# Yash-10/beta-sgp

Measured on AMD Instinct MI355X. Metric: SGP iterations/sec (fp64) on batched 256x256 images, higher is better.
Workload: dtype f64; 1 GPU; C3: 1024 independent 256x256 stamps per GPU, 25x25 PSF, linear A, beta-SGP (beta=1.05), proj_type=1, MAXIT=100, stop_criterion=1; images_per_gpu=1024, images_total=1024, maxit=100, parallelism=1 independent shards, one process per GPU (no collective on the data path), ls_spec=2, streams=1, team=1, proj_cache=1, gn_compact=1, storage=f64, persistent=1, stop_criterion=1

## Files before the change

### beta-sgp_amd/_bsgp.py

```python
import ctypes
import os
import threading

import numpy as np

try:
    import torch
except ImportError:
    torch = None

_HERE = os.path.dirname(os.path.abspath(__file__))
LIB_PATH = os.environ.get("BSGP_LIB", os.path.join(_HERE, "libbsgp.so"))

BSGP_CONV_CIRCULAR = 0
BSGP_CONV_LINEAR_FILL = 1
BSGP_VARIANT_KL = 0
BSGP_VARIANT_BETA = 1
BSGP_STORAGE_F64 = 0
BSGP_STORAGE_F32 = 1
ABI_VERSION = 3
BSGP_ERR_ARG = -1
BSGP_ERR_HIP = -2
BSGP_ERR_UNSUPPORTED = -3
BSGP_ERR_PSF = -4
# ... 35 lines not shown

class Inputs(ctypes.Structure):
    _fields_ = [("gn", _P), ("bkg", _P), ("flux", _P), ("x0", _P), ("beta0", _P), ("obj", _P)]


class Outputs(ctypes.Structure):
    _fields_ = [("x", _P), ("iters", _P), ("discr", _P), ("times", _P), ("crit", _P),
                ("flags", _P), ("beta_final", _P), ("counters", _P), ("err", _P),
                ("x_iter", _P)]


class PsfModel(ctypes.Structure):
    _fields_ = [("hw", ctypes.c_int32), ("ngauss", ctypes.c_int32), ("ldeg", ctypes.c_int32),
                ("sdeg", ctypes.c_int32), ("cos", ctypes.c_double), ("sin", ctypes.c_double),
                ("ax", ctypes.c_double), ("ay", ctypes.c_double), ("sigma_inc", ctypes.c_double),
                ("x_orig", ctypes.c_double), ("y_orig", ctypes.c_double), ("coeffs", _P),
                ("ncoef", ctypes.c_int32)]


BSGP_STATE_MAGIC = 0x53475342
BSGP_STATE_VERSION = 1
BSGP_STATE_HEADER_BYTES = 1024


class StateHeader(ctypes.Structure):
    _fields_ = [
        ("magic", ctypes.c_uint32), ("version", ctypes.c_uint32),
        ("H", ctypes.c_int32), ("W", ctypes.c_int32), ("storage", ctypes.c_int32),
        ("conv_mode", ctypes.c_int32), ("hist_cap", ctypes.c_int32), ("T", ctypes.c_int32),
        ("iters_done", ctypes.c_int32), ("stopped", ctypes.c_int32), ("Xones", ctypes.c_int32),
        ("epoch", ctypes.c_int32), ("g32", ctypes.c_int32), ("beta0_given", ctypes.c_int32),
        ("record_bytes", ctypes.c_int64), ("counters", ctypes.c_int64 * 7),
        ("scaling", ctypes.c_double), ("flux", ctypes.c_double), ("bkg_scalar", ctypes.c_double),
        ("x_low", ctypes.c_double), ("x_upp", ctypes.c_double), ("Dcoeff", ctypes.c_double),
        ("tol", ctypes.c_double), ("elapsed", ctypes.c_double), ("fv", ctypes.c_double),
        ("alpha", ctypes.c_double), ("tau", ctypes.c_double), ("lr", ctypes.c_double),
        ("init_lr", ctypes.c_double), ("beta", ctypes.c_double), ("lam_p", ctypes.c_double),
        ("lam_ratio", ctypes.c_double), ("kappa", ctypes.c_double), ("konst", ctypes.c_double),
        ("gfill", ctypes.c_double), ("Valpha", ctypes.c_double * 32),
        ("Fold", ctypes.c_double * 32), ("prm", Params),
    ]


assert ctypes.sizeof(StateHeader) <= BSGP_STATE_HEADER_BYTES
STATE_HEADER_DTYPE = np.dtype(StateHeader)
STATE_SECTIONS = ("discr", "crit", "times", "flags", "x", "g", "x_tf", "pw", "gn", "bkg")

_lib = None
_lib_lock = threading.Lock()


def lib():
    global _lib
    if _lib is not None:
        return _lib
    with _lib_lock:
        if _lib is None:
            if not os.path.exists(LIB_PATH):
                raise BsgpError(-3, f"{LIB_PATH} not built — run __graft_entry__.build()")
            L = ctypes.CDLL(LIB_PATH)
            i32, i64, dbl, vp = ctypes.c_int32, ctypes.c_int64, ctypes.c_double, ctypes.c_void_p
            L.bsgp_last_error.restype = ctypes.c_char_p
            L.bsgp_abi_version.restype = i32
            L.bsgp_plan_create.argtypes = [i32, i32, vp, i32, i32, i32, i32, i32,
                                           ctypes.POINTER(vp)]
            L.bsgp_plan_create_checked.argtypes = [i32, i32, vp, i32, i32, i32, i32, i32, i32,
                                                   ctypes.POINTER(vp)]
            L.bsgp_plan_destroy.argtypes = [vp]
            L.bsgp_plan_info.argtypes = [vp, vp, vp, vp, vp]
            L.bsgp_solve_device.argtypes = [vp, i32, vp, vp, vp, vp]
            L.bsgp_solve_host.argtypes = [vp, i32, vp, vp, vp]
            L.bsgp_solve_profiled.argtypes = [vp, i32, vp, vp, vp, vp, vp, vp]
            L.bsgp_apply_operator.argtypes = [vp, i32, i32, vp, vp, vp]
            L.bsgp_project_df.argtypes = [i64, dbl, vp, vp, dbl, i32, dbl, dbl, dbl, dbl, i32,
                                          i32, i32, vp, vp, vp]
            L.bsgp_beta_div.argtypes = [i64, vp, vp, dbl, vp, vp]
            L.bsgp_beta_div_deriv.argtypes = [i64, vp, vp, dbl, vp, vp]
            L.bsgp_beta_div_grad_parts.argtypes = [i64, vp, vp, dbl, vp, vp, vp]
            L.bsgp_extract_tiles.argtypes = [vp, i32, i32, vp, i32, i32, i32, vp, vp]
            L.bsgp_coadd_tiles.argtypes = [vp, i32, i32, i32, vp, i32, i32, vp, vp, vp]
            L.bsgp_fits_to_f64.argtypes = [vp, i64, i32, dbl, dbl, vp, vp]
            L.bsgp_psf_stamps.argtypes = [ctypes.POINTER(PsfModel), vp, i32, i32, i32, vp, vp]
            L.bsgp_plan_set_psfs.argtypes = [vp, vp, i32, vp]
            L.bsgp_state_layout.argtypes = [i32, i32, i32, i32, i32, vp]
            L.bsgp_state_bytes.argtypes = [vp, i32, i32, ctypes.POINTER(i64)]
            L.bsgp_state_save.argtypes = [vp, i32, vp, i64, vp]
            L.bsgp_solve_resume.argtypes = [vp, i32, vp, vp, i32, i64, vp, vp, vp]
            L.bsgp_background2d.argtypes = [vp, i32, i32, i32, i32, i32, i32, i32, i32, dbl, i32,
                                            dbl, i32, vp, vp, vp, vp, vp, vp, vp, vp]
            L.bsgp_convolve2d.argtypes = [vp, i32, i32, i32, i32, vp, i32, i32, vp, vp]
            L.bsgp_detect_sources.argtypes = [vp, i32, i32, i32, i32, vp, dbl, i32, i32, vp, vp,
                                              vp, vp]
            L.bsgp_segment_catalog.argtypes = [vp, vp, vp, i32, i32, i32, i32, vp, vp, vp, vp, vp]
            for name in ["bsgp_plan_create", "bsgp_plan_create_checked", "bsgp_plan_destroy", "bsgp_plan_info",
                         "bsgp_solve_device", "bsgp_solve_host", "bsgp_solve_profiled",
                         "bsgp_apply_operator",
                         "bsgp_project_df", "bsgp_beta_div", "bsgp_beta_div_deriv",
                         "bsgp_beta_div_grad_parts", "bsgp_device_synchronize",
                         "bsgp_extract_tiles", "bsgp_coadd_tiles", "bsgp_fits_to_f64",
                         "bsgp_psf_stamps", "bsgp_plan_set_psfs", "bsgp_state_layout",
                         "bsgp_state_bytes", "bsgp_state_save", "bsgp_solve_resume",
                         "bsgp_background2d", "bsgp_convolve2d", "bsgp_detect_sources",
                         "bsgp_segment_catalog"]:
                getattr(L, name).restype = ctypes.c_int
            if L.bsgp_abi_version() != ABI_VERSION:
                raise BsgpError(-3, f"{LIB_PATH} has ABI {L.bsgp_abi_version()}, this binding "
                                    f"needs {ABI_VERSION}: rebuild with __graft_entry__.build()")
            _lib = L
    return _lib


EXPORTED = ["bsgp_plan_create", "bsgp_plan_create_checked", "bsgp_plan_destroy", "bsgp_plan_info", "bsgp_solve_device",
            "bsgp_solve_host", "bsgp_solve_profiled", "bsgp_apply_operator", "bsgp_project_df", "bsgp_beta_div",
            "bsgp_beta_div_deriv", "bsgp_beta_div_grad_parts", "bsgp_device_synchronize",
            "bsgp_last_error", "bsgp_abi_version", "bsgp_extract_tiles", "bsgp_coadd_tiles",
            "bsgp_fits_to_f64", "bsgp_psf_stamps", "bsgp_plan_set_psfs", "bsgp_state_layout",
            "bsgp_state_bytes", "bsgp_state_save", "bsgp_solve_resume", "bsgp_background2d",
            "bsgp_convolve2d", "bsgp_detect_sources", "bsgp_segment_catalog"]


def check(rc):
    if rc != 0:
        raise BsgpError(rc, lib().bsgp_last_error().decode(errors="replace"))


def require_gpu():
    if torch is None or not torch.cuda.is_available():
        raise BsgpError(-2, "no HIP device visible: the beta-SGP engine has no CPU fallback")


def _ptr(t):
    return ctypes.c_void_p(t.data_ptr()) if t is not None else None


def current_stream():
    return ctypes.c_void_p(torch.cuda.current_stream().cuda_stream)


class Plan:

    _leased = False
    _done = None

    def __init__(self, H, W, psf, conv_mode, device=None, storage=BSGP_STORAGE_F64,
                 psf_checked=False):
        require_gpu()
        if device is None:
            device = torch.cuda.current_device()
        psf = np.ascontiguousarray(psf, dtype="<f8")
        self.H, self.W = int(H), int(W)
        self.kh, self.kw = psf.shape
        self.conv_mode = conv_mode
        self.device = device
        self.storage = storage
        h = ctypes.c_void_p()
        rc = lib().bsgp_plan_create_checked(self.H, self.W, psf.ctypes.data, self.kh, self.kw,
                                            conv_mode, storage, device, int(bool(psf_checked)),
                                            ctypes.byref(h))
        if rc != 0:
            raise BsgpError(rc, lib().bsgp_last_error().decode(errors="replace"))
        self.h = h
        P, Q, wave = ctypes.c_int32(), ctypes.c_int32(), ctypes.c_int32()
        sb = ctypes.c_int64()
        check(lib().bsgp_plan_info(h, ctypes.byref(P), ctypes.byref(Q), ctypes.byref(sb),
                                   ctypes.byref(wave)))
        self.P, self.Q, self.slot_bytes, self.fft_waves = P.value, Q.value, sb.value, wave.value

    def __del__(self):
        h = getattr(self, "h", None)
        if h is not None and _lib is not None:
            try:
                _lib.bsgp_plan_destroy(h)
            except Exception:
                pass
            self.h = None

    def set_psfs(self, psfs):
        psfs = psfs.to(dtype=torch.float64).contiguous()
        if psfs.dim() != 3 or tuple(psfs.shape[1:]) != (self.kh, self.kw):
            raise ValueError(f"psfs must be [n, {self.kh}, {self.kw}]")
        check(lib().bsgp_plan_set_psfs(self.h, _ptr(psfs), psfs.shape[0], current_stream()))
        self.n_psf = psfs.shape[0]
        return self

    def apply(self, x, transpose=False):
        x = x.contiguous()
        out = torch.empty_like(x)
        B = 1 if x.dim() == 2 else x.shape[0]
        check(lib().bsgp_apply_operator(self.h, B, int(transpose), _ptr(x), _ptr(out),
                                        current_stream()))
        return out

    def solve(self, gn, bkg, params, flux=None, x0=None, beta0=None, want_times=True, obj=None,
              want_iterates=False, profile=False):
        B = gn.shape[0]
        M1 = params.MAXIT + 1
        dev = gn.device
        f64 = dict(dtype=torch.float64, device=dev)
        if want_iterates:
            need = B * params.MAXIT * self.H * self.W * 8
            free = torch.cuda.mem_get_info(dev)[0]
            if need > 0.8 * free:
                raise BsgpError(
                    f"save=True keeps {params.MAXIT} iterates of {self.H}x{self.W} on the device "
                    f"({need / 2**30:.1f} GiB, {free / 2**30:.1f} GiB free): lower MAXIT")
        nd = B * M1 * (2 + bool(want_times) + (obj is not None)) + B
        d64 = torch.zeros(nd, **f64)
        i32 = torch.zeros(B * (M1 + 1) + 2 * 8 * B, dtype=torch.int32, device=dev)
        parts = iter(torch.split(d64, [B * M1] * (2 + bool(want_times) + (obj is not None)) + [B]))
        discr, crit = next(parts).view(B, M1), next(parts).view(B, M1)
        times = next(parts).view(B, M1) if want_times else None
        err = next(parts).view(B, M1) if obj is not None else None
        beta_final = next(parts)
        cnt, iters, flags = torch.split(i32, [2 * 8 * B, B, B * M1])
        out = {
            "x": torch.empty_like(gn),
            "iters": iters,
            "discr": discr,
            "times": times,
            "crit": crit,
            "flags": flags.view(B, M1),
            "beta_final": beta_final,
            "counters": cnt.view(torch.int64).view(B, 8),
            "err": err,
            "x_iter": (torch.zeros(B, params.MAXIT, self.H, self.W, **f64) if want_iterates
                       else None),
        }
        ins = Inputs(_ptr(gn), _ptr(bkg), _ptr(flux), _ptr(x0), _ptr(beta0), _ptr(obj))
        outs = Outputs(*[_ptr(out[k]) for k in ["x", "iters", "discr", "times", "crit", "flags",
                                                 "beta_final", "counters", "err", "x_iter"]])
        self._keep = (gn, bkg, flux, x0, beta0, obj)
        self._last = (B, int(params.MAXIT), int(params.bkg_is_map), out)
        if profile:
            kms = np.zeros(6, np.float64)
            nl = np.zeros(6, np.int64)
            check(lib().bsgp_solve_profiled(self.h, B, ctypes.byref(params), ctypes.byref(ins),
                                            ctypes.byref(outs), current_stream(),
                                            kms.ctypes.data, nl.ctypes.data))
            out["kernel_ms"], out["launches"] = kms, nl
            return out
        check(lib().bsgp_solve_device(self.h, B, ctypes.byref(params), ctypes.byref(ins),
                                      ctypes.byref(outs), current_stream()))
        return out

    def save_state(self, B):
        last = getattr(self, "_last", None)
        if last is None or last[0] != B:
            raise BsgpError(BSGP_ERR_ARG, "save_state: no solve of this batch size ran on the plan")
        _, maxit, bmap, _ = last
        nb = ctypes.c_int64()
        check(lib().bsgp_state_bytes(self.h, bmap, maxit, ctypes.byref(nb)))
        rec = torch.empty((B, nb.value), dtype=torch.uint8, device="cuda")
        check(lib().bsgp_state_save(self.h, B, _ptr(rec), nb.value, current_stream()))
        return rec

    def resume(self, state, params, index=None, want_times=True):
        n = state.shape[0]
        B = n if index is None else int(index.numel())
        M1 = params.MAXIT + 1
        dev = state.device
        f64 = dict(dtype=torch.float64, device=dev)
        d64 = torch.zeros(B * M1 * (2 + bool(want_times)) + B, **f64)
        i32 = torch.zeros(B * (M1 + 1) + 2 * 8 * B, dtype=torch.int32, device=dev)
        parts = iter(torch.split(d64, [B * M1] * (2 + bool(want_times)) + [B]))
        discr, crit = next(parts).view(B, M1), next(parts).view(B, M1)
        times = next(parts).view(B, M1) if want_times else None
# ... 427 lines not shown
```

### beta-sgp_amd/csrc/bsgp_api.hip

```cpp
#include <hip/hip_runtime.h>

#include <algorithm>
#include <atomic>
#include <cerrno>
#include <cstdlib>
#include <cmath>
#include <cstdio>
#include <cstring>
#include <string>
#include <vector>

#include "bsgp_internal.hpp"
#include "bsgp_psf.hpp"

using namespace bsgp;

namespace {

thread_local std::string g_err;

int fail(int code, const std::string& msg) {
  g_err = msg;
  return code;
}
// ... 71 lines not shown
  for (int h = 1; h <= maxh; ++h) {
    lev_off[h - 1] = (int)order.size();
    for (int k = 0; k < M; ++k)
      if (b.heights[k] == h) order.push_back(k);
  }
  lev_off[maxh] = (int)order.size();
  for (int i = 0; i < M; ++i) newid[order[i]] = L + i;
  auto val = [&](int t) { return t >= 0 ? t : newid[-t - 1]; };
  std::vector<int> prog(b.leaves);
  for (int i = 0; i < M; ++i) {
    prog.push_back(val(b.nodes_tmp[2 * order[i]]));
    prog.push_back(val(b.nodes_tmp[2 * order[i] + 1]));
  }
  for (int v : lev_off) prog.push_back(v);
  for (int t : root_tmp) prog.push_back(val(t));
  pp->nleaf = L;
  pp->nnode = M;
  pp->nlev = maxh;
  pp->nchunk = (int)root_tmp.size();
  return prog;
}

std::vector<cd> twiddles(int n) {
  std::vector<cd> t(n);
  const long double pi = 3.141592653589793238462643383279502884L;
  for (int k = 0; k < n; ++k) {
    const long double a = -2.0L * pi * (long double)k / (long double)n;
    t[k] = cmk((double)cosl(a), (double)sinl(a));
  }
  return t;
}

}

struct bsgp_plan_s {
  int device = 0;
  int conv_mode = 0;
  Geo g{};
  cd* tw = nullptr;
  cd* tf = nullptr;
  int n_tf = 1;
  int kh = 0, kw = 0;
  size_t lds_fft_bytes = 0;
  size_t lds_bytes = 0;
  int wg_per_cu = 1;
  int resident_per_cu = 1;
  int ncu = 256;
  double* ws = nullptr;
  size_t ws_slots = 0;
  size_t slot_stride = 0;
  size_t vec_stride = 0;
  size_t spec_off = 0;
  ImgState* st = nullptr;
  size_t st_n = 0;
  int* active = nullptr;
  int* active_h = nullptr;
  int* done_h = nullptr;
  int* done_d = nullptr;
  int seq = 0;
  static constexpr int kPollRing = 8;
  hipEvent_t ev_it[kPollRing] = {};
  static constexpr int kMaxStreams = 16;
  hipStream_t sub[kMaxStreams] = {};
  hipEvent_t ev_fork = nullptr;
  hipEvent_t ev_join[kMaxStreams] = {};
  int nsub = 0;
  double* tpart = nullptr;
  size_t tpart_n = 0;
  unsigned int* tctr = nullptr;
  size_t tctr_bytes = 0;
  double* plist = nullptr;
  size_t plist_n = 0;
  cd* opws = nullptr;
  size_t opws_slots = 0;
  int storage = BSGP_STORAGE_F64;
  int* pwprog = nullptr;
  PwProg pw{};
  unsigned* pq = nullptr;
  size_t pq_n = 0;
  bool last_valid = false;
  bsgp_params last_prm{};
  bsgp_outputs last_out{};
  int last_B = 0, last_T = 0, last_beta0 = 0;
};

static int proj_list_cap(const Geo& g, int T) {
  const long npair = ((long)g.H * g.W + 1) / 2;
  const int nb = plan_block(g);
  if (T == 1) return (int)(2 * ((npair + nb - 1) / nb));
  const long cp = (long)g.nfw * g.W;
  const long nch = (npair + cp - 1) / cp;
  return (int)(2 * ((nch + T - 1) / T) * ((cp + nb - 1) / nb));
}

static int ensure_plist(bsgp_plan p, size_t n) {
  if (n > p->plist_n) {
    if (p->plist) HIP_TRY(hipFree(p->plist));
    p->plist = nullptr;
    p->plist_n = 0;
    HIP_TRY(hipMalloc(&p->plist, n * sizeof(double)));
    p->plist_n = n;
  }
  return BSGP_OK;
}

static int ensure_ws(bsgp_plan p, size_t slots) {
  if (slots > p->ws_slots) {
    if (p->ws) HIP_TRY(hipFree(p->ws));
    p->ws = nullptr;
    p->ws_slots = 0;
    HIP_TRY(hipMalloc(&p->ws, slots * p->slot_stride * sizeof(double)));
    p->ws_slots = slots;
  }
  if (slots > p->st_n) {
    if (p->st) HIP_TRY(hipFree(p->st));
    p->st = nullptr;
    p->st_n = 0;
    HIP_TRY(hipMalloc(&p->st, slots * sizeof(ImgState)));
    p->st_n = slots;
  }
  return BSGP_OK;
}

static std::atomic<int> g_solve_seq{0};

static int choose_team(const bsgp_plan_s* p, int B, int req) {
  if (req == 1) return 1;
  const Geo& g = p->g;
  const int rows2 = (g.H + 1) / 2;
  int tgeo = rows2 / g.nfw;
  if (g.Qh / g.nfw < tgeo) tgeo = g.Qh / g.nfw;
  const int res = p->ncu * p->resident_per_cu / B;
  int T = std::min(p->ncu / B, tgeo);
  if (req > 1) T = std::min(req, tgeo);
  T = std::min(T, res);
  T = std::min(T, kMaxTeam);
  return T < 1 ? 1 : T;
}

static int ensure_team(bsgp_plan p, size_t B, int T) {
  const size_t np = B * kPartBufs * (size_t)(T + 8) * kMaxRed;
  if (T > 1 && np > p->tpart_n) {
    if (p->tpart) HIP_TRY(hipFree(p->tpart));
    p->tpart = nullptr;
    p->tpart_n = 0;
    HIP_TRY(hipMalloc(&p->tpart, np * sizeof(double)));
    p->tpart_n = np;
  }
  const size_t cb = round_up((B * kTeamWords + kTeamLine) * sizeof(unsigned int), 128);
  if (cb > p->tctr_bytes) {
    if (p->tctr) HIP_TRY(hipFree(p->tctr));
    p->tctr = nullptr;
    p->tctr_bytes = 0;
    HIP_TRY(hipMalloc(&p->tctr, cb));
    p->tctr_bytes = cb;
  }
  return BSGP_OK;
}

extern "C" {

int32_t bsgp_abi_version(void) { return 3; }

int bsgp_phase_prof(uint64_t* out, int32_t n, int32_t reset) {
  hipError_t e = phase_prof(reinterpret_cast<unsigned long long*>(out), n, reset);
  if (e == hipErrorNotSupported) return fail(BSGP_ERR_UNSUPPORTED, "built without BSGP_PHASE_PROF");
// ... 291 lines not shown
    if (p->sub[i]) (void)hipStreamDestroy(p->sub[i]);
    if (p->ev_join[i]) (void)hipEventDestroy(p->ev_join[i]);
  }
  if (p->ev_fork) (void)hipEventDestroy(p->ev_fork);
  if (p->st) (void)hipFree(p->st);
  if (p->active) (void)hipFree(p->active);
  if (p->active_h) (void)hipHostFree(p->active_h);
  if (p->done_h) (void)hipHostFree(p->done_h);
  for (hipEvent_t e : p->ev_it)
    if (e) (void)hipEventDestroy(e);
  if (p->opws) (void)hipFree(p->opws);
  if (p->tpart) (void)hipFree(p->tpart);
  if (p->tctr) (void)hipFree(p->tctr);
  if (p->plist) (void)hipFree(p->plist);
  if (p->pwprog) (void)hipFree(p->pwprog);
  if (p->pq) (void)hipFree(p->pq);
  delete p;
  return BSGP_OK;
}

int bsgp_plan_set_psfs(bsgp_plan p, const double* psfs, int32_t n, void* stream) {
  if (!p || !psfs || n < 1) return fail(BSGP_ERR_ARG, "bad arguments");
  Geo& g = p->g;
  const bool circ = p->conv_mode == BSGP_CONV_CIRCULAR;
  if (!circ && (p->kh > g.P || p->kw > g.Q || p->kw > g.P || p->kh > g.Q))
    return fail(BSGP_ERR_ARG, "per-image PSFs need a kernel no larger than the FFT grid");
  DEVICE_SCOPE(p->device);
  hipStream_t s = (hipStream_t)stream;
  const size_t PQ = (size_t)g.P * g.Q, tfn = (size_t)g.Qh * g.P, specn = (size_t)g.P * g.Qh;
  const size_t per = 2 * PQ * sizeof(double) + specn * sizeof(cd);
  const int chunk = (int)std::max<size_t>(1, std::min<size_t>((size_t)n, (256u << 20) / per));
  cd* tf = nullptr;
  double* kc = nullptr;
  cd* spec = nullptr;
  double* sums = nullptr;
  int rc = BSGP_OK;
  if (hipMalloc(&tf, (size_t)n * 2 * tfn * sizeof(cd)) != hipSuccess ||
      hipMalloc(&kc, (size_t)chunk * 2 * PQ * sizeof(double)) != hipSuccess ||
      hipMalloc(&spec, (size_t)chunk * specn * sizeof(cd)) != hipSuccess ||
      hipMalloc(&sums, (size_t)n * sizeof(double)) != hipSuccess)
    rc = fail(BSGP_ERR_HIP, "per-image PSF allocation failed");
  const double scale = 1.0 / ((double)g.P * (double)g.Q);
  Geo gb = g;
  gb.tf_stride = 0;
  for (int c0 = 0; rc == BSGP_OK && c0 < n; c0 += chunk) {
    const int m = std::min(chunk, n - c0);
    cd* t = tf + (size_t)c0 * 2 * tfn;
    if (hipMemsetAsync(kc, 0, (size_t)m * 2 * PQ * sizeof(double), s) != hipSuccess ||
        launch_place_psfs(gb, m, psfs + (size_t)c0 * p->kh * p->kw, p->kh, p->kw, circ ? 1 : 0,
                          kc, sums + c0, s) != hipSuccess ||
        launch_build_tfs(gb, m, kc, 2 * PQ, spec, specn, t, 2 * tfn, scale, 0, p->lds_bytes,
                         s) != hipSuccess ||
        launch_build_tfs(gb, m, circ ? kc : kc + PQ, 2 * PQ, spec, specn, t + tfn, 2 * tfn,
                         scale, circ ? 1 : 0, p->lds_bytes, s) != hipSuccess)
      rc = fail(BSGP_ERR_HIP, "per-image TF launch failed");
  }
  std::vector<double> hs(n);
  if (rc == BSGP_OK && (hipMemcpyAsync(hs.data(), sums, (size_t)n * sizeof(double),
                                       hipMemcpyDeviceToHost, s) != hipSuccess ||
                        hipStreamSynchronize(s) != hipSuccess))
    rc = fail(BSGP_ERR_HIP, "per-image TF build failed");
  for (int i = 0; rc == BSGP_OK && i < n; ++i)
    if (!(std::fabs(hs[i] - 1.0) <= 1e4 * 2.220446049250313e-16)) {
      char b[160];
      snprintf(b, sizeof b, "PSF %d is not normalized! sum(psf) - 1. = %.17g", i, hs[i] - 1.0);
      rc = fail(BSGP_ERR_PSF, b);
    }
  if (kc) (void)hipFree(kc);
  if (spec) (void)hipFree(spec);
  if (sums) (void)hipFree(sums);
  if (rc != BSGP_OK) {
    if (tf) (void)hipFree(tf);
    return rc;
  }
  if (p->tf) (void)hipFree(p->tf);
  p->tf = tf;
  p->n_tf = n;
  g.tfA = tf;
  g.tfAT = tf + tfn;
  g.tf_stride = n > 1 ? 2 * tfn : 0;
  return BSGP_OK;
}

int bsgp_plan_info(bsgp_plan p, int32_t* P, int32_t* Q, int64_t* slot_bytes,
                   int32_t* fft_waves) {
  if (!p) return fail(BSGP_ERR_ARG, "plan is NULL");
  if (P) *P = p->g.P;
  if (Q) *Q = p->g.Q;
  if (slot_bytes) *slot_bytes = (int64_t)(p->slot_stride * sizeof(double));
  if (fft_waves) *fft_waves = p->g.nfw;
  return BSGP_OK;
}

static int check_params(const bsgp_params* q) {
  if (!q) return fail(BSGP_ERR_ARG, "params is NULL");
  if (q->variant != BSGP_VARIANT_KL && q->variant != BSGP_VARIANT_BETA)
    return fail(BSGP_ERR_ARG, "bad variant");
  if (q->MAXIT < 1) return fail(BSGP_ERR_ARG, "MAXIT must be >= 1");
  if (q->M_alpha < 1 || q->M_alpha > 32) return fail(BSGP_ERR_ARG, "M_alpha must be in [1, 32]");
  if (q->M < 1 || q->M > 32) return fail(BSGP_ERR_ARG, "M must be in [1, 32]");
  if (q->ls_spec < 1 || q->ls_spec > 8) return fail(BSGP_ERR_ARG, "ls_spec must be in [1, 8]");
  if (q->init_recon < 0 || q->init_recon > 3) return fail(BSGP_ERR_ARG, "bad init_recon");
  if (q->proj_type != 0 && q->proj_type != 1) return fail(BSGP_ERR_ARG, "bad proj_type");
  if (q->scale_data < 0 || q->scale_data > 2) return fail(BSGP_ERR_ARG, "bad scale_data");
  if (q->flux_f32 && !(q->gn_f32 && q->scale_data != 2))
    return fail(BSGP_ERR_ARG, "flux_f32 needs gn_f32 with scale_data 0 or 1");
  return BSGP_OK;
}

struct SolveProf {
  std::vector<hipEvent_t> ev;
  double* kernel_ms;
  int64_t* launches;
};

struct ResumeCtx {
  StateArgs sa;
  int T;
  int it0;
  bool uniform;
  int done_it;
  int beta0_given;
};

static int solve_impl(bsgp_plan p, int32_t B, const bsgp_params* prm, const bsgp_inputs* in,
                      const bsgp_outputs* out, void* stream, SolveProf* prof,
                      const ResumeCtx* rs = nullptr);

int bsgp_solve_device(bsgp_plan p, int32_t B, const bsgp_params* prm, const bsgp_inputs* in,
                      const bsgp_outputs* out, void* stream) {
  return solve_impl(p, B, prm, in, out, stream, nullptr);
}

int bsgp_solve_profiled(bsgp_plan p, int32_t B, const bsgp_params* prm, const bsgp_inputs* in,
                        const bsgp_outputs* out, void* stream, double* kernel_ms,
                        int64_t* launches) {
  if (!kernel_ms || !launches) return fail(BSGP_ERR_ARG, "kernel_ms / launches missing");
  if (!prm) return fail(BSGP_ERR_ARG, "params is NULL");
  if (!p) return fail(BSGP_ERR_ARG, "plan is NULL");
  DEVICE_SCOPE(p->device);
  SolveProf prof;
  prof.kernel_ms = kernel_ms;
  prof.launches = launches;
  const size_t nev = 6 * (size_t)(prm->MAXIT > 0 ? prm->MAXIT : 0) + 2;
  prof.ev.resize(nev, nullptr);
  int rc = BSGP_OK;
  for (size_t i = 0; i < nev && rc == BSGP_OK; ++i)
    if (hipEventCreate(&prof.ev[i]) != hipSuccess) rc = fail(BSGP_ERR_HIP, "event create failed");
  if (rc == BSGP_OK) {
    bsgp_params q = *prm;
    q.streams = 1;
    rc = solve_impl(p, B, &q, in, out, stream, &prof);
  }
  for (hipEvent_t e : prof.ev)
    if (e) (void)hipEventDestroy(e);
  return rc;
}

static int solve_impl(bsgp_plan p, int32_t B, const bsgp_params* prm, const bsgp_inputs* in,
                      const bsgp_outputs* out, void* stream, SolveProf* prof,
                      const ResumeCtx* rs) {
  if (!p) return fail(BSGP_ERR_ARG, "plan is NULL");
  int rc = check_params(prm);
  if (rc) return rc;
  if (B < 1) return fail(BSGP_ERR_ARG, "B must be >= 1");
  if (!rs) {
    if (!in || !in->gn || !in->bkg) return fail(BSGP_ERR_ARG, "inputs gn/bkg missing");
    if ((prm->init_recon == 1 || prm->scale_data == 2) && !in->x0)
      return fail(BSGP_ERR_ARG, "init_recon=1 and scale_data=2 need x0");
  }
  if (!out || !out->x || !out->iters || !out->discr) return fail(BSGP_ERR_ARG, "outputs missing");
  if (out->err && (!in || !in->obj)) return fail(BSGP_ERR_ARG, "err needs the ground truth obj");
  if (p->n_tf > 1 && B != p->n_tf)
    return fail(BSGP_ERR_ARG, "the plan holds one PSF per image: B must equal its PSF count");
  DEVICE_SCOPE(p->device);
  rc = ensure_ws(p, (size_t)B);
  if (rc) return rc;
  const int T = rs ? rs->T : choose_team(p, B, prm->team);
  rc = ensure_team(p, (size_t)B, T);
  if (rc) return rc;
  SolveArgs a;
  a.g = p->g;
  a.prm = *prm;
  if (rs) {
    a.in = bsgp_inputs{};
    if (rs->beta0_given) a.in.beta0 = reinterpret_cast<const double*>(p->st);
  } else {
    a.in = *in;
  }
  a.out = *out;
  a.B = B;
  a.img0 = 0;
  a.nimg = B;
  a.st = p->st;
  a.active = p->active;
  a.ws = p->ws;
  a.slot_stride = p->slot_stride;
  a.vec_stride = p->vec_stride;
  a.lds_fft_bytes = p->lds_fft_bytes;
  a.T = T;
  a.Tc = T;
  if (T > 1) {
    const int ncol = (p->g.coop && p->g.nfc == 1 && p->g.Q % 2 == 0)
                         ? p->g.Qh - 1
                         : p->g.Qh;
    const int nc = (ncol + p->g.nfc - 1) / p->g.nfc;
    const int want = 4 * p->ncu / B;
    a.Tc = std::max(T, std::min(nc, want));
  }
  a.fuse_col = T == 1 ? 2 : 0;
  a.tpart = T > 1 ? p->tpart : nullptr;
  a.tctr = p->tctr;
  a.tfail = reinterpret_cast<int*>(p->tctr + (size_t)B * kTeamWords);
  a.plist = nullptr;
  a.plist_stride = 0;
  a.lcap = 0;
  a.list_lds = 0;
  a.pw = p->pw;
  a.storage = p->storage;
  a.spec_off = p->spec_off;
  a.spin_limit = (unsigned)env_knob("BSGP_SPIN_LIMIT", 1ll << 26, 0, 0xffffffffll);
  a.ls_predict = (int)env_knob("BSGP_LS_PREDICT", 1, 0, 5);
  a.ls_cap = (prm->beta > 0.0 && prm->beta < 1.0)
                 ? (int)std::ceil(std::log(1e-12) / std::log(prm->beta)) + 2
                 : 4096;
  if (prm->proj_cache && prm->proj_type == 1) {
    a.lcap = proj_list_cap(p->g, T);
    const size_t half = round_up((size_t)a.lcap * T * plan_block(p->g), 32);
    a.plist_stride = 2 * half;
    rc = ensure_plist(p, (size_t)B * a.plist_stride);
    if (rc) return rc;
    a.plist = p->plist;
    if (T > 1) {
      const size_t fit = p->lds_fft_bytes / ((size_t)plan_block(p->g) * 2 * sizeof(double));
      a.list_lds = (int)std::min<size_t>((size_t)a.lcap, fit);
    }
  }
  hipStream_t s = (hipStream_t)stream;
  const int K = (prm->adapt_beta && prm->variant == BSGP_VARIANT_BETA)
                    ? 1
                    : (prm->ls_spec <= 1 ? 1 : prm->ls_spec <= 2 ? 2 : prm->ls_spec <= 4 ? 4 : 8);
  int S = prm->streams < 1 ? 1 : prm->streams;
  if (S > bsgp_plan_s::kMaxStreams) S = bsgp_plan_s::kMaxStreams;
  if (S > B) S = B;
  const bool track = out->err != nullptr || out->x_iter != nullptr;
  const bool ring_rule = prm->stop_criterion >= 2 && prm->stop_criterion <= 4;
  const bool persist =
      prm->persistent && T == 1 && !track && (!rs || ring_rule || rs->uniform);
  if (persist) S = 1;
  const bool ring = prm->stop_criterion >= 2 && prm->stop_criterion <= 4;
  a.fold_setup = (persist && !ring && !rs && env_knob("BSGP_FOLD_SETUP", 1, 0, 1)) ? 1 : 0;
  if (S > 1 && p->nsub < S) {
    if (!p->ev_fork) HIP_TRY(hipEventCreateWithFlags(&p->ev_fork, hipEventDisableTiming));
    for (int i = (p->nsub > 1 ? p->nsub : 1); i < S; ++i) {
      HIP_TRY(hipStreamCreateWithFlags(&p->sub[i], hipStreamNonBlocking));
      HIP_TRY(hipEventCreateWithFlags(&p->ev_join[i], hipEventDisableTiming));
    }
    p->nsub = S;
  }
  HIP_TRY(hipMemsetD32Async((hipDeviceptr_t)p->active, rs ? 0 : B, 1, s));
  a.seq = g_solve_seq.fetch_add(1, std::memory_order_relaxed) + 1;
  p->seq = a.seq;
  a.done_host = p->done_d;
  HIP_TRY(hipMemsetAsync(p->tctr, 0, p->tctr_bytes, s));
  if (T > 1 && (T <= kTeamFlags || T >= 8))
    HIP_TRY(hipMemsetD32Async((hipDeviceptr_t)p->tpart, kPartEmptyWord,
                              B * kPartBufs * (size_t)(T + 8) * kMaxRed * 2, s));
  p->last_valid = true;
  p->last_prm = *prm;
  p->last_out = *out;
  p->last_B = B;
  p->last_T = T;
  p->last_beta0 = a.in.beta0 != nullptr;
  StateArgs ld{};
  if (rs) {
    ld = rs->sa;
    ld.ws = p->ws;
    ld.slot_stride = p->slot_stride;
    ld.vec_stride = p->vec_stride;
    ld.st = p->st;
    ld.T = T;
    ld.M1 = prm->MAXIT + 1;
    ld.out = *out;
    ld.prm = *prm;
    ld.active = p->active;
    HIP_TRY(launch_state_load(ld, B, s));
    if (!(persist && !ring))
      HIP_TRY(launch_state_post(ld, B, nullptr, nullptr, 0, p->done_d, a.seq, s));
  }
  hipStream_t ss[bsgp_plan_s::kMaxStreams];
  SolveArgs sa[bsgp_plan_s::kMaxStreams];
  if (S > 1) HIP_TRY(hipEventRecord(p->ev_fork, s));
  for (int j = 0; j < S; ++j) {
    ss[j] = j > 0 ? p->sub[j] : s;
    if (j > 0) HIP_TRY(hipStreamWaitEvent(ss[j], p->ev_fork, 0));
    sa[j] = a;
    sa[j].img0 = (int)((int64_t)B * j / S);
    sa[j].nimg = (int)((int64_t)B * (j + 1) / S) - sa[j].img0;
    if (prof) HIP_TRY(hipEventRecord(prof->ev[0], ss[j]));
    if (!a.fold_setup && !rs) HIP_TRY(launch_setup(sa[j], p->lds_bytes, ss[j]));
    if (prof) HIP_TRY(hipEventRecord(prof->ev[1], ss[j]));
    if (track) HIP_TRY(launch_track(sa[j], 0, ss[j]));
  }
  if (persist) {
    const size_t need = (size_t)2 * B + 4;
    if (need > p->pq_n) {
      if (p->pq) HIP_TRY(hipFree(p->pq));
      p->pq = nullptr;
      p->pq_n = 0;
      HIP_TRY(hipMalloc(&p->pq, need * sizeof(unsigned)));
      p->pq_n = need;
    }
    HIP_TRY(hipMemsetAsync(p->pq, 0, need * sizeof(unsigned), s));
    if (rs && !ring)
      HIP_TRY(launch_state_post(ld, B, p->pq, p->pq + 1, rs->done_it, p->done_d, a.seq, s));
    int per_cu = 0;
    HIP_TRY(persist_resident_per_cu(sa[0], K, p->lds_bytes, &per_cu));
    if (per_cu < 1) return fail(BSGP_ERR_HIP, "persistent solver does not fit a CU");
    const int grid = (int)std::min<long>(B, (long)p->ncu * per_cu);
    if (prof) HIP_TRY(hipEventRecord(prof->ev[2], s));
    HIP_TRY(launch_persist(sa[0], K, p->lds_bytes, s, p->pq, p->pq + 1, grid));
    if (prof) {
      HIP_TRY(hipEventRecord(prof->ev[3], s));
      HIP_TRY(hipStreamSynchronize(s));
      for (int k = 0; k < 6; ++k) {
        prof->kernel_ms[k] = 0.0;
        prof->launches[k] = 0;
      }
      float ms = 0.f;
      HIP_TRY(hipEventElapsedTime(&ms, prof->ev[0], prof->ev[1]));
      prof->kernel_ms[0] = a.fold_setup ? 0.0 : ms;
      prof->launches[0] = a.fold_setup ? 0 : 1;
// ... 118 lines not shown
  }
  auto d2h = [&](void* h, const void* d, size_t bytes) {
    return !h || hipMemcpy(h, d, bytes, hipMemcpyDeviceToHost) == hipSuccess;
  };
  ok = hipDeviceSynchronize() == hipSuccess && d2h(out->x, dout.x, B * N * 8) &&
       d2h(out->iters, dout.iters, B * 4) && d2h(out->discr, dout.discr, B * M1 * 8) &&
       (!out->times || d2h(out->times, dout.times, B * M1 * 8)) &&
       (!out->crit || d2h(out->crit, dout.crit, B * M1 * 8)) &&
       (!out->flags || d2h(out->flags, dout.flags, B * M1 * 4)) &&
       (!out->beta_final || d2h(out->beta_final, dout.beta_final, B * 8)) &&
       (!out->counters || d2h(out->counters, dout.counters, B * 64)) &&
       (!out->err || d2h(out->err, dout.err, B * M1 * 8)) &&
       (!out->x_iter || d2h(out->x_iter, dout.x_iter, B * (M1 - 1) * N * 8));
  cleanup();
  if (!ok) return fail(BSGP_ERR_HIP, "solve or device to host copy failed");
  return BSGP_OK;
}


int bsgp_state_layout(int32_t H, int32_t W, int32_t storage, int32_t bkg_is_map,
                      int32_t hist_cap, int64_t* offs) {
  if (!offs) return fail(BSGP_ERR_ARG, "offs is NULL");
  if (H < 1 || W < 1 || hist_cap < 1) return fail(BSGP_ERR_ARG, "bad shape or hist_cap");
  if (storage != BSGP_STORAGE_F64 && storage != BSGP_STORAGE_F32)
    return fail(BSGP_ERR_ARG, "bad storage");
  const StateLayout L = state_layout((size_t)H * W, storage, bkg_is_map != 0, hist_cap);
  const size_t v[11] = {L.bytes, L.discr, L.crit, L.times, L.flags, L.x,
                        L.g,     L.xtf,   L.pw,   L.gn,    L.bkg};
  for (int i = 0; i < 11; ++i) offs[i] = (int64_t)v[i];
  return BSGP_OK;
}

int bsgp_state_bytes(bsgp_plan p, int32_t bkg_is_map, int32_t MAXIT_done_max,
                     int64_t* bytes_per_image) {
  if (!p) return fail(BSGP_ERR_ARG, "plan is NULL");
  if (!bytes_per_image || MAXIT_done_max < 0) return fail(BSGP_ERR_ARG, "bad arguments");
  *bytes_per_image = (int64_t)state_layout((size_t)p->g.H * p->g.W, p->storage, bkg_is_map != 0,
                                           MAXIT_done_max + 1)
                         .bytes;
  return BSGP_OK;
}

int bsgp_state_save(bsgp_plan p, int32_t B, void* state_dev, int64_t bytes_per_image,
                    void* stream) {
  if (!p) return fail(BSGP_ERR_ARG, "plan is NULL");
  if (!state_dev) return fail(BSGP_ERR_ARG, "state_dev is NULL");
  if (!p->last_valid) return fail(BSGP_ERR_ARG, "no solve has run on this plan");
  if (B != p->last_B || B > 65535)
    return fail(BSGP_ERR_ARG, "B must be the last solve's batch size (at most 65535)");
  const bsgp_params& q = p->last_prm;
  if (q.stop_criterion == 2 && !p->last_out.crit)
    return fail(BSGP_ERR_ARG, "saving a stop_criterion 2 solve needs its out->crit");
  StateArgs a{};
  a.N = p->g.H * p->g.W;
  a.H = p->g.H;
  a.W = p->g.W;
  a.storage = p->storage;
  a.conv_mode = p->conv_mode;
  a.bmap = q.bkg_is_map != 0;
  a.hist_cap = q.MAXIT + 1;
  a.L = state_layout((size_t)a.N, a.storage, a.bmap != 0, a.hist_cap);
  if ((int64_t)a.L.bytes != bytes_per_image)
    return fail(BSGP_ERR_ARG, "bytes_per_image is not bsgp_state_bytes(plan, bkg_is_map, MAXIT)");
  a.rec = static_cast<unsigned char*>(state_dev);
  a.rec_bytes = a.L.bytes;
  a.ws = p->ws;
  a.slot_stride = p->slot_stride;
  a.vec_stride = p->vec_stride;
  a.st = p->st;
  a.T = p->last_T;
  a.beta0_given = p->last_beta0;
  a.M1 = q.MAXIT + 1;
  a.out = p->last_out;
  a.prm = q;
  DEVICE_SCOPE(p->device);
  HIP_TRY(launch_state_save(a, B, (hipStream_t)stream));
  return BSGP_OK;
}

int bsgp_solve_resume(bsgp_plan p, int32_t B, const bsgp_params* prm, const void* state_dev,
                      int32_t n_state, int64_t bytes_per_image, const int32_t* index,
                      const bsgp_outputs* out, void* stream) {
  if (!p) return fail(BSGP_ERR_ARG, "plan is NULL");
  int rc = check_params(prm);
  if (rc) return rc;
  if (!state_dev || n_state < 1) return fail(BSGP_ERR_ARG, "state_dev missing");
  if (B < 1 || B > 65535 || (!index && B > n_state))
    return fail(BSGP_ERR_ARG, "B must be in [1, 65535] and, without an index, at most n_state");
  if (!out || !out->x || !out->iters || !out->discr) return fail(BSGP_ERR_ARG, "outputs missing");
  if (out->err || out->x_iter)
    return fail(BSGP_ERR_UNSUPPORTED, "err / x_iter are not available on a resumed solve");
  if (p->n_tf > 1 && B != p->n_tf)
    return fail(BSGP_ERR_ARG, "the plan holds one PSF per image: B must equal its PSF count");
  if (bytes_per_image < BSGP_STATE_HEADER_BYTES || bytes_per_image % 16)
    return fail(BSGP_ERR_ARG, "bad bytes_per_image");
  DEVICE_SCOPE(p->device);
  hipStream_t s = (hipStream_t)stream;
  std::vector<bsgp_state_header> hs((size_t)n_state);
  std::vector<int32_t> idx((size_t)B);
  HIP_TRY(hipMemcpy2DAsync(hs.data(), sizeof(bsgp_state_header), state_dev,
                           (size_t)bytes_per_image, sizeof(bsgp_state_header), (size_t)n_state,
                           hipMemcpyDeviceToHost, s));
  if (index)
    HIP_TRY(hipMemcpyAsync(idx.data(), index, (size_t)B * sizeof(int32_t), hipMemcpyDeviceToHost,
                           s));
  HIP_TRY(hipStreamSynchronize(s));
  if (!index)
    for (int i = 0; i < B; ++i) idx[i] = i;
  const size_t N = (size_t)p->g.H * p->g.W;
  ResumeCtx rs{};
  int min_done = -1, max_done = -1;
  char msg[200];
  for (int i = 0; i < B; ++i) {
    if (idx[i] < 0 || idx[i] >= n_state) {
      snprintf(msg, sizeof msg, "index[%d] = %d is outside the %d records", i, idx[i], n_state);
      return fail(BSGP_ERR_ARG, msg);
    }
    const bsgp_state_header& h = hs[(size_t)idx[i]];
    const bsgp_params& q = h.prm;
    const char* bad = nullptr;
    auto same = [](const void* a, const void* b, size_t n) { return memcmp(a, b, n) == 0; };
#define BSGP_SAME(f) \
  if (!bad && !same(&q.f, &prm->f, sizeof q.f)) bad = #f
    if (h.magic != BSGP_STATE_MAGIC) bad = "magic";
    if (!bad && h.version != BSGP_STATE_VERSION) bad = "version";
    if (!bad && (h.H != p->g.H || h.W != p->g.W)) bad = "shape (H, W)";
    if (!bad && h.storage != p->storage) bad = "storage";
    if (!bad && h.conv_mode != p->conv_mode) bad = "conv_mode";
    BSGP_SAME(variant);
    BSGP_SAME(init_recon);
    BSGP_SAME(proj_type);
    BSGP_SAME(stop_criterion);
    BSGP_SAME(M_alpha);
    BSGP_SAME(M);
    BSGP_SAME(max_projs);
    BSGP_SAME(gamma);
    BSGP_SAME(beta);
    BSGP_SAME(alpha);
    BSGP_SAME(alpha_min);
    BSGP_SAME(alpha_max);
    BSGP_SAME(tau);
    BSGP_SAME(ccd_sat_level);
    BSGP_SAME(betaParam);
    BSGP_SAME(lr);
    BSGP_SAME(lr_exp_param);
    BSGP_SAME(tol_convergence);
    BSGP_SAME(prescaled_scaling);
    BSGP_SAME(prescaled_tol4);
    BSGP_SAME(has_sat);
    BSGP_SAME(scale_data);
    BSGP_SAME(verbose);
    BSGP_SAME(adapt_beta);
    BSGP_SAME(schedule_lr);
    BSGP_SAME(bkg_is_map);
    BSGP_SAME(ls_series);
    BSGP_SAME(gn_compact);
    BSGP_SAME(gn_f32);
    BSGP_SAME(beta0_general);
    BSGP_SAME(flux_f32);
#undef BSGP_SAME
    if (!bad && (h.hist_cap < 1 || h.iters_done < 0 || h.iters_done >= h.hist_cap ||
                 h.record_bytes != bytes_per_image ||
                 (int64_t)state_layout(N, p->storage, q.bkg_is_map != 0, h.hist_cap).bytes !=
                     bytes_per_image))
      bad = "record_bytes / hist_cap";
    if (!bad && i > 0 && (h.hist_cap != rs.sa.hist_cap || h.T != rs.T ||
// ... 315 lines not shown
```

### beta-sgp_amd/csrc/bsgp_device.hpp

```cpp
#pragma once

#include <hip/hip_runtime.h>
#include <stdint.h>

#include <type_traits>

#include "bsgp_fft.hpp"
#include "bsgp_lanesplit.hpp"
#include "bsgp_math.hpp"

namespace bsgp {

#ifndef BSGP_BLOCK
#define BSGP_BLOCK 256
#endif
constexpr int kBlock = BSGP_BLOCK;
constexpr int kWaves = kBlock / 64;
constexpr int kMaxRed = 24;

constexpr int kTeamFlags = 64;
constexpr int kPartBufs = 3;
constexpr unsigned long long kPartEmpty = 0xFFF75EE0FFF75EE0ull;
constexpr unsigned int kPartEmptyWord = 0xFFF75EE0u;
constexpr int kSharedBytes = 512;

constexpr int kPhaseSlots = 40;
#ifdef BSGP_PHASE_PROF
static __device__ unsigned long long g_phase[kPhaseSlots];
#define PH_T(v) const unsigned long long v = __builtin_amdgcn_s_memtime()
#define PH_ADD(slot, t0)                                                                 \
  do {                                                                                   \
    if (threadIdx.x == 0) atomicAdd(&g_phase[slot], __builtin_amdgcn_s_memtime() - (t0)); \
  } while (0)
#define PH_SUB(slot, t)                                                                 \
  do {                                                                                  \
    if (PHS >= 0) {                                                                     \
      const unsigned long long t_ = __builtin_amdgcn_s_memtime();                        \
      if (threadIdx.x == 0) atomicAdd(&g_phase[(slot) < 0 ? 0 : (slot)], t_ - (t));       \
      t = t_;                                                                           \
    }                                                                                   \
  } while (0)
#define PH_SUB_T(v) unsigned long long v = __builtin_amdgcn_s_memtime()
#else
#define PH_T(v)
#define PH_ADD(slot, t0)
#define PH_SUB(slot, t)
#define PH_SUB_T(v)
#endif

struct Geo {
  int H, W;
  int P, Q;
  int Qh;
  int nfw;
  int nfc;
  int coop;
  int lpad;
  int sld;
  int tw2;
  int twmix;
  FftPlan fp;
  FftPlan fq;
  const cd* tfA;
  const cd* tfAT;
  size_t tf_stride;
};

__device__ __forceinline__ const cd* tf_of(const Geo& G, int img, int transpose) {
  return (transpose ? G.tfAT : G.tfA) + (size_t)img * G.tf_stride;
}

__device__ __forceinline__ void copy_tw(const FftPlan& f) {
  if (f.lds_tw < 0) return;
  extern __shared__ __attribute__((aligned(16))) char bsgp_dyn_lds[];
  cd* d = reinterpret_cast<cd*>(bsgp_dyn_lds + f.lds_tw);
  for (int i = threadIdx.x; i < f.n; i += kBlock) d[i] = f.tw[i];
}
__device__ __forceinline__ void copy_tw2(const FftPlan& f) {
  if (f.lds_tw2 < 0) return;
  extern __shared__ __attribute__((aligned(16))) char bsgp_dyn_lds[];
  cd* d = reinterpret_cast<cd*>(bsgp_dyn_lds + f.lds_tw2);
  const int m = 64 + f.n / 64;
  for (int i = threadIdx.x; i < m; i += blockDim.x) d[i] = f.tw[i < 64 ? i : 64 * (i - 64)];
}
__device__ __forceinline__ void load_tw_lds(const Geo& G) {
  if (G.twmix >= 0) {
    extern __shared__ __attribute__((aligned(16))) char bsgp_dyn_lds[];
    cd* d = reinterpret_cast<cd*>(bsgp_dyn_lds + G.twmix);
    for (int i = threadIdx.x; i < 64 + 512; i += blockDim.x)
      d[i] = G.fp.tw[i < 64 ? 32 * i : 4 * (i - 64)];
  }
  copy_tw(G.fp);
  if (G.fq.lds_tw != G.fp.lds_tw) copy_tw(G.fq);
  copy_tw2(G.fp);
  if (G.fq.lds_tw2 != G.fp.lds_tw2) copy_tw2(G.fq);
  __syncthreads();
}

__device__ __forceinline__ void wave_sync() {
  __builtin_amdgcn_fence(__ATOMIC_RELEASE, "wavefront");
  __builtin_amdgcn_s_waitcnt(0xC07F);
  __builtin_amdgcn_wave_barrier();
  __builtin_amdgcn_fence(__ATOMIC_ACQUIRE, "wavefront");
}

struct WaveSync {
  __device__ __forceinline__ void operator()() const { wave_sync(); }
};

template <int O>
__device__ __forceinline__ double xor_lanes(double v) {
  if constexpr (O == 1 || O == 2) {
    constexpr int ctrl = O == 1 ? 0xB1 : 0x4E;
    const int lo = __builtin_amdgcn_update_dpp(0, __double2loint(v), ctrl, 0xF, 0xF, false);
    const int hi = __builtin_amdgcn_update_dpp(0, __double2hiint(v), ctrl, 0xF, 0xF, false);
    return __hiloint2double(hi, lo);
  } else if constexpr (O < 32) {
    constexpr int pat = (O << 10) | 0x1F;
    const int lo = __builtin_amdgcn_ds_swizzle(__double2loint(v), pat);
    const int hi = __builtin_amdgcn_ds_swizzle(__double2hiint(v), pat);
    return __hiloint2double(hi, lo);
  } else {
    return __shfl_xor(v, O, 64);
  }
}
__device__ __forceinline__ double wave_sum(double v) {
  v += xor_lanes<32>(v);
  v += xor_lanes<16>(v);
  v += xor_lanes<8>(v);
  v += xor_lanes<4>(v);
  v += xor_lanes<2>(v);
  v += xor_lanes<1>(v);
  return v;
}
template <bool MAX>
__device__ __forceinline__ double wave_ext_step(double v, double u) {
  return MAX ? ((u > v || u != u) ? u : v) : ((u < v || u != u) ? u : v);
}
template <bool MAX>
__device__ __forceinline__ double wave_ext(double v) {
  v = wave_ext_step<MAX>(v, xor_lanes<32>(v));
  v = wave_ext_step<MAX>(v, xor_lanes<16>(v));
  v = wave_ext_step<MAX>(v, xor_lanes<8>(v));
  v = wave_ext_step<MAX>(v, xor_lanes<4>(v));
  v = wave_ext_step<MAX>(v, xor_lanes<2>(v));
  v = wave_ext_step<MAX>(v, xor_lanes<1>(v));
  return v;
}
__device__ __forceinline__ double wave_max(double v) { return wave_ext<true>(v); }
__device__ __forceinline__ double wave_min(double v) { return wave_ext<false>(v); }

template <int NV>
// ... 600 lines not shown
    typename Rep::val r[sizeof(T) / B];
#pragma unroll
    for (int n = 0; n < (int)(sizeof(T) / B); ++n)
      r[n] = __builtin_nontemporal_load(reinterpret_cast<const R*>(p) + n);
    T v;
    __builtin_memcpy(&v, r, sizeof(T));
    return v;
  }
}
template <bool NT, class T, int ALIGN = (alignof(T) < 16 ? (int)alignof(T) : 16)>
__device__ __forceinline__ void stp(T* p, const T& v) {
  if constexpr (!NT) {
    *p = v;
  } else {
    constexpr int B = sizeof(T) <= 16 ? (int)sizeof(T) : 16;
    static_assert(sizeof(T) % B == 0, "4, 8 or whole 16-byte pieces");
    typedef NtRep<B, (B < ALIGN ? B : ALIGN)> Rep;
    typedef typename Rep::ptr R;
    typename Rep::val r[sizeof(T) / B];
    __builtin_memcpy(r, &v, sizeof(T));
#pragma unroll
    for (int n = 0; n < (int)(sizeof(T) / B); ++n)
      __builtin_nontemporal_store(r[n], reinterpret_cast<R*>(p) + n);
  }
}

struct alignas(32) CPair {
  cd a, b;
};

template <unsigned POL = 0>
__device__ __forceinline__ void store_pair(cd* col, bool two, bool pair_ok, cd ak, cd bk) {
  constexpr bool NT = (POL & kNtSR) != 0;
  if (two && pair_ok) {
    CPair v;
    v.a = ak;
    v.b = bk;
    stp<NT>(reinterpret_cast<CPair*>(col), v);
  } else {
    stp<NT>(col, ak);
    if (two) stp<NT>(col + 1, bk);
  }
}

constexpr int kJCH = 4;
constexpr int kGCH = 3;
constexpr int kPCH = 5;

template <int JCH, class LD, class V>
__device__ __forceinline__ void load_rows(LD& ld, int r, bool two, int j0, int lane, int ncols,
                                          V (&v0)[JCH], V (&v1)[JCH]) {
  const int r1 = two ? r + 1 : r;
#pragma unroll
  for (int u = 0; u < JCH; ++u) {
    const int j = min(j0 + lane + 64 * u, ncols - 1);
    v0[u] = ld(r, j);
    v1[u] = ld(r1, j);
  }
}

template <class V>
struct Two {
  V a, b;
};
struct NoWide {};

template <class T>
__device__ __forceinline__ void half_swap(T& a, T& b) {
  static_assert(sizeof(T) % 4 == 0, "whole dwords");
  constexpr int N = sizeof(T) / 4;
  unsigned int x[N], y[N];
  __builtin_memcpy(x, &a, sizeof(T));
  __builtin_memcpy(y, &b, sizeof(T));
#pragma unroll
  for (int n = 0; n < N; ++n) {
    const auto s = __builtin_amdgcn_permlane32_swap(x[n], y[n], false, false);
    x[n] = s[0];
    y[n] = s[1];
  }
  __builtin_memcpy(&a, x, sizeof(T));
  __builtin_memcpy(&b, y, sizeof(T));
}

template <bool COOP>
__device__ __forceinline__ bool row_wide(const Geo& G) {
  return !COOP && (G.W & 1) == 0;
}

__device__ __forceinline__ double split_undo(double v) {
  return __shfl(v, split_lane((int)(threadIdx.x & 63u)), 64);
}

template <int JCH, class LD2, class V>
__device__ __forceinline__ void load_rows2(LD2& ld2, int r, bool two, int j0, int lane, int ncols,
                                           V (&v0)[JCH], V (&v1)[JCH]) {
  const int rr = (two && split_half(lane)) ? r + 1 : r;
#pragma unroll
  for (int u = 0; u < JCH; ++u) {
    const Two<V> q = ld2(rr, split_pair_clamped(j0 + 64 * u, lane, ncols));
    v0[u] = q.a;
    v1[u] = q.b;
  }
}

struct BlockSync {
  __device__ __forceinline__ void operator()() const { __syncthreads(); }
};
constexpr int kCCH = 4;


template <class LD, class MK>
__device__ __forceinline__ void coop_row_fwd_1(const Geo& G, const Part& D, int nrows, int ncols,
                                             int ldim, cd* spec, cd* lds, LD& ld, MK& mk) {
  using V = decltype(ld(0, 0));
  const int t = threadIdx.x;
  const bool pair_ok = (ldim & 1) == 0;
  cd* a = lds;
  cd* b = lds + G.lpad;
  for (int r = 2 * D.gw0; r < nrows; r += 2 * D.gws) {
    const bool two = (r + 1) < nrows;
    for (int j0 = 0; j0 < G.Q; j0 += kBlock * kCCH) {
      V v0[kCCH], v1[kCCH];
#pragma unroll
      for (int u = 0; u < kCCH; ++u) {
        const int j = min(j0 + t + kBlock * u, ncols - 1);
        v0[u] = ld(r, j);
        v1[u] = ld(two ? r + 1 : r, j);
      }
#pragma unroll
      for (int u = 0; u < kCCH; ++u) {
        const int j = j0 + t + kBlock * u;
        if (j < G.Q) {
          double va = 0.0, vb = 0.0;
          if (j < ncols) {
            va = mk(r, j, v0[u]);
            if (two) vb = mk(r + 1, j, v1[u]);
          }
          a[j] = cmk(va, vb);
        }
      }
    }
    __syncthreads();
    cd* Z = fft_wide(a, b, G.fq, false, t, kBlock, BlockSync());
    for (int k = t; k < G.Qh; k += kBlock) {
      cd ak, bk;
      r2c_split(Z, G.Q, k, &ak, &bk);
      store_pair(spec + (size_t)k * ldim + r, two, pair_ok, ak, bk);
    }
    __syncthreads();
  }
}

__device__ __forceinline__ void coop_gather_1(const Geo& G, const cd* spec, int r, bool two, cd* a) {
  const int t = threadIdx.x;
  for (int k0 = 0; k0 < G.Qh; k0 += kBlock * kCCH) {
    cd A[kCCH], B[kCCH];
#pragma unroll
    for (int u = 0; u < kCCH; ++u) {
      const int k = min(k0 + t + kBlock * u, G.Qh - 1);
      const cd* col = spec + (size_t)k * G.sld + r;
      A[u] = col[0];
      const cd b = col[two ? 1 : 0];
      B[u] = two ? b : cmk(0.0, 0.0);
    }
#pragma unroll
    for (int u = 0; u < kCCH; ++u) {
      const int k = k0 + t + kBlock * u;
      if (k < G.Qh) {
// ... 346 lines not shown
  const CGrp c = coop_grp(D.nf);
  const int t = c.t;
  cd* a = lds + c.g * 2 * G.lpad;
  cd* b = a + G.lpad;
  for (int k0 = D.gw0; k0 < G.Qh; k0 += D.gws) {
    const int k = k0 + c.g;
    const bool act = k < G.Qh;
    cd* col = spec + (size_t)k * G.sld;
    const cd* tk = tf + (size_t)k * G.P;
    PH_T(tq0);
    if (act) {
      for (int p0 = 0; p0 < G.P; p0 += c.nt * kCCH) {
        cd cv[kCCH];
#pragma unroll
        for (int u = 0; u < kCCH; ++u) {
          const int p = p0 + t + c.nt * u;
          const cd v = col[min(p, G.H - 1)];
          cv[u] = (p < G.H) ? v : cmk(0.0, 0.0);
        }
#pragma unroll
        for (int u = 0; u < kCCH; ++u) {
          const int p = p0 + t + c.nt * u;
          if (p < G.P) a[p] = cv[u];
        }
      }
    }
    __syncthreads();
    PH_ADD(29, tq0);
    PH_T(tq1);
    cd* Z = fft_wide<false>(a, b, G.fp, false, t, c.nt, BlockSync());
    if (act) {
      for (int p0 = 0; p0 < G.P; p0 += c.nt * kCCH) {
        cd tv[kCCH];
#pragma unroll
        for (int u = 0; u < kCCH; ++u) tv[u] = tk[min(p0 + t + c.nt * u, G.P - 1)];
#pragma unroll
        for (int u = 0; u < kCCH; ++u) {
          const int p = p0 + t + c.nt * u;
          if (p < G.P) Z[p] = cmul(Z[p], tv[u]);
        }
      }
    }
    __syncthreads();
    cd* Y = fft_wide<false>(Z, (Z == a) ? b : a, G.fp, true, t, c.nt, BlockSync());
    if (act)
      for (int p = t; p < G.H; p += c.nt) col[p] = Y[p];
    __syncthreads();
    PH_ADD(30, tq1);
  }
}

template <class LD, class MK>
__device__ __forceinline__ void coop_row_fwd(const Geo& G, const Part& D, int nrows, int ncols,
                                             int ldim, cd* spec, cd* lds, LD& ld, MK& mk) {
  if (D.nf == 1)
    coop_row_fwd_1(G, D, nrows, ncols, ldim, spec, lds, ld, mk);
  else
    coop_row_fwd_g(G, D, nrows, ncols, ldim, spec, lds, ld, mk);
}
template <class LD, class USE>
__device__ __forceinline__ void coop_row_inv(const Geo& G, const Part& D, const cd* spec, cd* lds,
                                             LD& ld, USE& use) {
  if (D.nf == 1)
    coop_row_inv_1(G, D, spec, lds, ld, use);
  else
    coop_row_inv_g(G, D, spec, lds, ld, use);
}
template <class CP>
__device__ __forceinline__ void coop_row_inv_fwd(const Geo& G, const Part& D, cd* spec, cd* lds,
                                                 CP& cp) {
  if (D.nf == 1)
    coop_row_inv_fwd_1(G, D, spec, lds, cp);
  else
    coop_row_inv_fwd_g(G, D, spec, lds, cp);
}
__device__ __forceinline__ void coop_col_conv(const Geo& G, const Part& D, cd* spec, const cd* tf,
                                              cd* lds) {
  if (D.nf == 1)
    coop_col_conv_1(G, D, spec, tf, lds);
  else
    coop_col_conv_g(G, D, spec, tf, lds);
}

template <int JCH = kJCH, bool PF = false, bool COMP = true, bool COOP = false,
          bool PIPE = false, int PHS = -1, unsigned POL = 0, class LD, class MK,
          class LD2 = NoWide>
__device__ __forceinline__ void row_fwd2(const Geo& G, const Part& D, int nrows, int ncols,
                                         int ldim, cd* spec, cd* lds, LD&& ld, MK&& mk,
                                         LD2&& ld2 = LD2{}) {
  if constexpr (COOP) {
    coop_row_fwd(G, D, nrows, ncols, ldim, spec, lds, ld, mk);
    return;
  }
  using V = decltype(ld(0, 0));
  const int w = threadIdx.x >> 6, lane = threadIdx.x & 63;
  const bool pair_ok = (ldim & 1) == 0;
  constexpr bool kHasWide =
      !std::is_same<typename std::decay<LD2>::type, NoWide>::value;
  if (w < G.nfw) {
    auto run = [&](auto wide_c, auto& ldw) __attribute__((always_inline)) {
    constexpr bool WIDE = decltype(wide_c)::value;
    auto load = [&](int rr, bool two_r, int j0, V (&w0)[JCH], V (&w1)[JCH]) __attribute__((always_inline)) {
      if constexpr (WIDE)
        load_rows2<JCH>(ldw, rr, two_r, j0, lane, ncols, w0, w1);
      else
        load_rows<JCH>(ld, rr, two_r, j0, lane, ncols, w0, w1);
    };
    cd* a = lds + w * 2 * G.lpad;
    cd* b = a + G.lpad;
    int r = 2 * (D.gw0 + w);
    V v0[JCH], v1[JCH];
    if (PF && r < nrows) load(r, (r + 1) < nrows, 0, v0, v1);
    PH_SUB_T(tph);
    for (; r < nrows; r += 2 * D.gws) {
      const bool two = (r + 1) < nrows;
      auto put = [&](int j0, const V (&w0)[JCH], const V (&w1)[JCH]) __attribute__((always_inline)) {
#pragma unroll
        for (int u = 0; u < JCH; ++u) {
          V q0 = w0[u], q1 = w1[u];
          if constexpr (WIDE) half_swap(q0, q1);
          const int j = j0 + 64 * u + (WIDE ? split_col(lane) : lane);
          if (j < G.Q) {
            double va = 0.0, vb = 0.0;
            if (j < ncols) {
              va = mk(r, j, q0);
              if (two) vb = mk(r + 1, j, q1);
            }
            a[j] = cmk(va, vb);
          }
        }
      };
      if constexpr (PIPE) {
        constexpr int S = 64 * JCH;
        V u0[JCH], u1[JCH];
        if (!PF) load(r, two, 0, v0, v1);
        for (int j0 = 0; j0 < G.Q; j0 += 2 * S) {
          if (j0 + S < ncols) load(r, two, j0 + S, u0, u1);
          put(j0, v0, v1);
          if (j0 + S < G.Q) {
            if (j0 + 2 * S < ncols) load(r, two, j0 + 2 * S, v0, v1);
            put(j0 + S, u0, u1);
          }
        }
      } else {
        for (int j0 = 0; j0 < G.Q; j0 += 64 * JCH) {
          if ((!PF || j0 > 0) && j0 < ncols) load(r, two, j0, v0, v1);
          put(j0, v0, v1);
        }
      }
      const int rn = r + 2 * D.gws;
      if (PF && rn < nrows) load(rn, (rn + 1) < nrows, 0, v0, v1);
      wave_sync();
      PH_SUB(PHS, tph);
      cd* Z = fft_any<COMP>(a, b, G.fq, false, lane, 64, WaveSync());
      PH_SUB(PHS + 1, tph);
      for (int k = lane; k < G.Qh; k += 64) {
        cd ak, bk;
        r2c_split(Z, G.Q, k, &ak, &bk);
        store_pair<POL>(spec + (size_t)k * ldim + r, two, pair_ok, ak, bk);
      }
      wave_sync();
      PH_SUB(PHS + 2, tph);
    }
    };
    if constexpr (kHasWide) {
      if ((ncols & 1) == 0)
        run(std::true_type{}, ld2);
      else
        run(std::false_type{}, ld2);
    } else {
      run(std::false_type{}, ld2);
    }
  }
}

template <bool COOP = false, class Prod>
__device__ __forceinline__ void row_fwd(const Geo& G, const Part& D, int nrows, int ncols, int ldim,
                                        cd* spec, cd* lds, Prod&& prod) {
  row_fwd2<kJCH, false, true, COOP>(G, D, nrows, ncols, ldim, spec, lds, prod,
                                                  [](int, int, double v) { return v; });
}

template <unsigned POL = 0>
__device__ __forceinline__ void gather_pair(const Geo& G, const cd* spec, int ld, int r, bool two,
                                            cd* a, int lane) {
  constexpr bool NT = (POL & kNtSR) != 0;
  for (int k0 = lane; k0 < G.Qh; k0 += 64 * kGCH) {
    cd A[kGCH], B[kGCH];
#pragma unroll
    for (int u = 0; u < kGCH; ++u) {
      const int k = min(k0 + 64 * u, G.Qh - 1);
      const cd* col = spec + (size_t)k * ld + r;
      A[u] = ldp<NT>(col);
      const cd bk = ldp<NT>(col + (two ? 1 : 0));
      B[u] = two ? bk : cmk(0.0, 0.0);
    }
#pragma unroll
    for (int u = 0; u < kGCH; ++u) {
      const int k = k0 + 64 * u;
      if (k < G.Qh) {
        a[k] = cmk(A[u].x - B[u].y, A[u].y + B[u].x);
        if (k > 0 && G.Q - k >= G.Qh) a[G.Q - k] = cmk(A[u].x + B[u].y, B[u].x - A[u].y);
      }
    }
  }
}

typedef __attribute__((address_space(3))) void lds_void_t;
typedef __attribute__((address_space(1))) void gbl_void_t;
template <unsigned POL = 0>
__device__ __forceinline__ void stage_pair(const Geo& G, const cd* spec, int ld, int r, bool two,
                                           cd* F, int lane) {
  constexpr int kAux = (POL & kNtSR) ? 2 : 0;
  for (int k0 = 0; k0 < G.Qh; k0 += 32) {
    const int k = k0 + (lane >> 1);
    if (k < G.Qh) {
      const cd* col = spec + (size_t)k * ld + r + (two ? (lane & 1) : 0);
      __builtin_amdgcn_global_load_lds((gbl_void_t*)col, (lds_void_t*)(F + 2 * k0), 16, 0, kAux);
    }
  }
}
__device__ __forceinline__ void unpack_pair(const Geo& G, const cd* F, bool two, cd* a, int lane) {
  for (int k = lane; k < G.Qh; k += 64) {
    const cd A = F[2 * k];
    const cd B = two ? F[2 * k + 1] : cmk(0.0, 0.0);
    a[k] = cmk(A.x - B.y, A.y + B.x);
    if (k > 0 && G.Q - k >= G.Qh) a[G.Q - k] = cmk(A.x + B.y, B.x - A.y);
  }
}

template <bool PRE, int JCH = kJCH, bool COMP = true, bool COOP = false,
          bool PIPE = false, int PHS = -1, unsigned POL = 0, class LD, class USE,
          class LD2 = NoWide>
__device__ __forceinline__ void row_inv2(const Geo& G, const Part& D, const cd* spec, cd* lds,
                                         LD&& ld, USE&& use, LD2&& ld2 = LD2{}) {
  if constexpr (COOP) {
    coop_row_inv(G, D, spec, lds, ld, use);
    return;
  }
  using V = decltype(ld(0, 0));
  const int w = threadIdx.x >> 6, lane = threadIdx.x & 63;
  constexpr bool kHasWide =
      !std::is_same<typename std::decay<LD2>::type, NoWide>::value;
  if (w < G.nfw) {
    auto run = [&](auto wide_c, auto& ldw) __attribute__((always_inline)) {
    constexpr bool WIDE = decltype(wide_c)::value;
    auto load = [&](int rr, bool two_r, int j0, V (&w0)[JCH], V (&w1)[JCH]) __attribute__((always_inline)) {
      if constexpr (WIDE)
        load_rows2<JCH>(ldw, rr, two_r, j0, lane, G.W, w0, w1);
      else
        load_rows<JCH>(ld, rr, two_r, j0, lane, G.W, w0, w1);
    };
    cd* in = lds + w * 2 * G.lpad;
    cd* other = in + G.lpad;
    int r = 2 * (D.gw0 + w);
    PH_SUB_T(tph);
    if (r < G.H) gather_pair<POL>(G, spec, G.sld, r, (r + 1) < G.H, in, lane);
    for (; r < G.H; r += 2 * D.gws) {
      const bool two = (r + 1) < G.H;
      V v0[JCH], v1[JCH];
      if (PRE) load(r, two, 0, v0, v1);
      wave_sync();
      PH_SUB(PHS + 2, tph);
      cd* Z = fft_any<COMP>(in, other, G.fq, true, lane, 64, WaveSync());
      PH_SUB(PHS + 1, tph);
      cd* F = (Z == in) ? other : in;
      const int rn = r + 2 * D.gws;
      const bool next = rn < G.H, two_n = (rn + 1) < G.H;
      if (next) stage_pair<POL>(G, spec, G.sld, rn, two_n, F, lane);
      auto eat = [&](int j0, const V (&w0)[JCH], const V (&w1)[JCH]) __attribute__((always_inline)) {
#pragma unroll
        for (int u = 0; u < JCH; ++u) {
          V q0 = w0[u], q1 = w1[u];
          if constexpr (WIDE) half_swap(q0, q1);
          const int j = j0 + 64 * u + (WIDE ? split_col(lane) : lane);
          if (j < G.W) {
            const cd z = Z[j];
            use(r, j, z.x, q0);
            if (two) use(r + 1, j, z.y, q1);
          }
        }
      };
      if constexpr (PIPE) {
        constexpr int S = 64 * JCH;
        V u0[JCH], u1[JCH];
        if (!PRE) load(r, two, 0, v0, v1);
        for (int j0 = 0; j0 < G.W; j0 += 2 * S) {
          load(r, two, j0 + S, u0, u1);
          eat(j0, v0, v1);
          if (j0 + S < G.W) {
            load(r, two, j0 + 2 * S, v0, v1);
            eat(j0 + S, u0, u1);
          }
        }
      } else {
        for (int j0 = 0; j0 < G.W; j0 += 64 * JCH) {
          if (!PRE || j0 > 0) load(r, two, j0, v0, v1);
          eat(j0, v0, v1);
        }
      }
      PH_SUB(PHS, tph);
      if (next) {
        asm volatile("s_waitcnt vmcnt(0)" ::: "memory");
        wave_sync();
        unpack_pair(G, F, two_n, Z, lane);
        in = Z;
        other = F;
      }
    }
    wave_sync();
    };
    if constexpr (kHasWide) {
      if ((G.W & 1) == 0)
        run(std::true_type{}, ld2);
      else
        run(std::false_type{}, ld2);
    } else {
      run(std::false_type{}, ld2);
    }
  }
}

template <bool COOP = false, class Cons>
__device__ __forceinline__ void row_inv(const Geo& G, const Part& D, const cd* spec, cd* lds,
                                        Cons&& cons) {
  row_inv2<false, kJCH, true, COOP>(
      G, D, spec, lds, [](int, int) { return 0; },
      [&](int r, int j, double v, int) { cons(r, j, v); });
}

template <bool COOP = false, class CP>
__device__ __forceinline__ void row_inv_fwd(const Geo& G, const Part& D, cd* spec, cd* lds,
                                            CP&& cp) {
  if constexpr (COOP) {
    coop_row_inv_fwd(G, D, spec, lds, cp);
    return;
  }
  const int w = threadIdx.x >> 6, lane = threadIdx.x & 63;
  const bool pair_ok = (G.sld & 1) == 0;
  if (w < G.nfw) {
    cd* a = lds + w * 2 * G.lpad;
    cd* b = a + G.lpad;
    for (int r = 2 * (D.gw0 + w); r < G.H; r += 2 * D.gws) {
      const bool two = (r + 1) < G.H;
      gather_pair(G, spec, G.sld, r, two, a, lane);
      wave_sync();
      cd* Z = fft_any(a, b, G.fq, true, lane, 64, WaveSync());
      cd* in2 = (Z == a) ? b : a;
      for (int j = lane; j < G.Q; j += 64) {
        double va = 0.0, vb = 0.0;
        if (j < G.W) {
          const cd z = Z[j];
          va = cp(r, j, z.x);
          if (two) vb = cp(r + 1, j, z.y);
        }
        in2[j] = cmk(va, vb);
      }
      wave_sync();
      cd* Y = fft_any(in2, Z, G.fq, false, lane, 64, WaveSync());
      for (int k = lane; k < G.Qh; k += 64) {
        cd ak, bk;
        r2c_split(Y, G.Q, k, &ak, &bk);
        store_pair(spec + (size_t)k * G.sld + r, two, pair_ok, ak, bk);
      }
      wave_sync();
    }
  }
}

template <int JCH = kJCH, bool COMP = true, unsigned POL = 0, class LD, class CP>
__device__ __forceinline__ void row_inv_fwd2(const Geo& G, const Part& D, cd* spec, cd* lds,
                                             LD&& ld, CP&& cp) {
  using V = decltype(ld(0, 0));
  const int w = threadIdx.x >> 6, lane = threadIdx.x & 63;
  const bool pair_ok = (G.sld & 1) == 0;
  if (w < G.nfw) {
    cd* a = lds + w * 2 * G.lpad;
    cd* b = a + G.lpad;
    for (int r = 2 * (D.gw0 + w); r < G.H; r += 2 * D.gws) {
      const bool two = (r + 1) < G.H;
      gather_pair<POL>(G, spec, G.sld, r, two, a, lane);
      V v0[JCH], v1[JCH];
      load_rows<JCH>(ld, r, two, 0, lane, G.W, v0, v1);
      wave_sync();
      cd* Z = fft_any<COMP>(a, b, G.fq, true, lane, 64, WaveSync());
      cd* in2 = (Z == a) ? b : a;
      for (int j0 = 0; j0 < G.Q; j0 += 64 * JCH) {
        if (j0 > 0 && j0 < G.W) load_rows<JCH>(ld, r, two, j0, lane, G.W, v0, v1);
#pragma unroll
        for (int u = 0; u < JCH; ++u) {
          const int j = j0 + 64 * u + lane;
          if (j < G.Q) {
            double va = 0.0, vb = 0.0;
            if (j < G.W) {
              const cd z = Z[j];
              va = cp(r, j, z.x, v0[u]);
              if (two) vb = cp(r + 1, j, z.y, v1[u]);
            }
            in2[j] = cmk(va, vb);
          }
        }
      }
      wave_sync();
      cd* Y = fft_any<COMP>(in2, Z, G.fq, false, lane, 64, WaveSync());
      for (int k = lane; k < G.Qh; k += 64) {
        cd ak, bk;
        r2c_split(Y, G.Q, k, &ak, &bk);
        store_pair<POL>(spec + (size_t)k * G.sld + r, two, pair_ok, ak, bk);
      }
      wave_sync();
    }
  }
}

template <bool COOP = false, unsigned POL = 0>
__device__ __forceinline__ void col_conv(const Geo& G, const Part& D, cd* spec, const cd* tf,
                                         cd* lds) {
  constexpr bool NT = (POL & kNtSC) != 0;
  if constexpr (COOP) {
    coop_col_conv(G, D, spec, tf, lds);
    return;
  }
  const int w = threadIdx.x >> 6, lane = threadIdx.x & 63;
  if (w < G.nfw) {
    cd* a = lds + w * 2 * G.lpad;
    cd* b = a + G.lpad;
    for (int k = D.gw0 + w; k < G.Qh; k += D.gws) {
      cd* col = spec + (size_t)k * G.sld;
#ifdef BSGP_TF_ONECOL
      const cd* t = tf;
#else
      const cd* t = tf + (size_t)k * G.P;
#endif
      for (int p0 = 0; p0 < G.P; p0 += 64 * kPCH) {
        cd cv[kPCH];
#pragma unroll
        for (int u = 0; u < kPCH; ++u) {
          const int p = p0 + lane + 64 * u;
          const cd c = ldp<NT>(col + min(p, G.H - 1));
          cv[u] = p < G.H ? c : cmk(0.0, 0.0);
        }
#pragma unroll
        for (int u = 0; u < kPCH; ++u) {
          const int p = p0 + lane + 64 * u;
          if (p < G.P) a[p] = cv[u];
        }
      }
      wave_sync();
      cd* Z = fft_any(a, b, G.fp, false, lane, 64, WaveSync());
      if (G.P <= 64 * kPCH) {
        cd tv[kPCH];
#pragma unroll
        for (int u = 0; u < kPCH; ++u) tv[u] = t[min(lane + 64 * u, G.P - 1)];
#pragma unroll
        for (int u = 0; u < kPCH; ++u) {
          const int p = lane + 64 * u;
          if (p < G.P) Z[p] = cmul(Z[p], tv[u]);
        }
      } else {
        for (int p = lane; p < G.P; p += 64) Z[p] = cmul(Z[p], t[p]);
      }
      wave_sync();
      cd* Y = fft_any(Z, (Z == a) ? b : a, G.fp, true, lane, 64, WaveSync());
      for (int p = lane; p < G.H; p += 64) stp<NT>(col + p, Y[p]);
      wave_sync();
    }
  }
  __syncthreads();
}

struct ProjOut {
  double lam;
  int evals;
  int biter;
  int siter;
};

struct ProjClip {
  bool has_sat;
  double satv;
  __device__ __forceinline__ double operator()(double c, double dia, double lam) const {
    double v = (c + lam) / dia;
    v = (0.0 > v) ? 0.0 : v;
    if (has_sat) v = (satv < v) ? satv : v;
    return v;
  }
};

template <class CDF>
__device__ __forceinline__ double proj_sum(int N, CDF& cdf, const ProjClip& clip, double lam, double* red) {
  double s[1] = {0.0};
  for (int i = threadIdx.x; i < N; i += kBlock) {
    double c, dia;
    cdf(i, c, dia);
    s[0] += clip(c, dia, lam);
  }
  block_sum<1>(s, red);
  return s[0];
}
// ... 277 lines not shown
```

### beta-sgp_amd/csrc/bsgp_internal.hpp

```cpp
#pragma once

#include <hip/hip_runtime.h>

#include <vector>

#include "../../include/bsgp.h"
#include "bsgp_device.hpp"

namespace bsgp {

struct ImgState {
  int par, Xones, stop, iter, epoch;
  int bar_base;
  int64_t E_p, E_ls, ls_passes, status, ls_series;
  int64_t proj_passes, proj_list;
  double sc, flux, bks_scalar, lo, hi, Dcoeff, tol, t0;
  double fv, alpha, tau, lr, init_lr, beta, lam_p, gd, lam;
  double lam_ratio, kappa;
  double konst;
  int g32;
  int par_tf;
  double gfill;
  double Valpha[32];
  double Fold[32];
};


struct PwProg {
  const int* prog;
  int nleaf, nnode, nlev, nchunk;
};

struct SolveArgs {
  Geo g;
  bsgp_params prm;
  bsgp_inputs in;
  bsgp_outputs out;
  int B;
  int img0, nimg;
  ImgState* st;
  int* active;
  int* done_host;
  int seq;
  double* ws;
  size_t slot_stride;
  size_t vec_stride;
  size_t lds_fft_bytes;
  int T;
  int Tc;
  int fuse_col;
  double* tpart;
  unsigned int* tctr;
  int* tfail;
  double* plist;
  size_t plist_stride;
  int lcap;
  int list_lds;
  PwProg pw;
  int storage;
  size_t spec_off;
  int ls_cap;
  unsigned spin_limit;
  int fold_setup;
  int ls_predict;
};

hipError_t launch_setup(const SolveArgs& a, size_t lds, hipStream_t s);
hipError_t launch_iteration(const SolveArgs& a, int K, size_t lds, hipStream_t s,
                            hipEvent_t* ev = nullptr);
hipError_t launch_track(const SolveArgs& a, int it, hipStream_t s);
hipError_t launch_build_tf(const Geo& g, const double* kc, cd* spec, cd* tf, double scale,
                           int conj, size_t lds, hipStream_t s);
hipError_t launch_build_tfs(const Geo& g, int n, const double* kc, size_t kc_stride, cd* spec,
                            size_t spec_stride, cd* tf, size_t tf_stride, double scale, int conj,
                            size_t lds, hipStream_t s);
hipError_t launch_place_psfs(const Geo& g, int n, const double* psfs, int kh, int kw, int circ,
                             double* kc, double* sums, hipStream_t s);
hipError_t launch_apply_op(const Geo& g, int B, int transpose, const double* x, double* out,
                           cd* specws, size_t spec_stride, int grid, size_t lds, hipStream_t s);
hipError_t launch_apply_op_split(const Geo& g, int B, int transpose, const double* x,
                                 double* out, cd* specws, size_t spec_stride, int per, size_t lds,
                                 hipStream_t s);
hipError_t launch_project_df(int n, double b, const double* c, const double* dia, ProjClip clip,
                             double lam0, double dlam0, double tol_lam, int biter, int siter,
                             int max_projs, double* x, double* info, hipStream_t s);
hipError_t launch_beta_div(int n, const double* y, const double* x, double beta, double* out,
                           hipStream_t s);
hipError_t launch_beta_div_deriv(int64_t n, const double* y, const double* x, double beta,
                                 double* out, hipStream_t s);
hipError_t launch_grad_parts(int64_t n, const double* den, const double* gn, double beta,
                             double* pow1, double* w, hipStream_t s);
hipError_t set_solver_lds_limit(size_t bytes);
hipError_t team_resident_per_cu(bool coop, int storage, size_t lds, int* per_cu);
hipError_t launch_extract_tiles(const double* img, int W, const int* boxes, int n, int th, int tw,
                                double* out, hipStream_t s);
hipError_t launch_coadd_tiles(const double* tiles, int n, int th, int tw, const int* boxes, int H,
                              int W, double* mean, double* footprint, hipStream_t s);
hipError_t launch_fits_to_f64(const void* raw, int64_t n, int bitpix, double bscale, double bzero,
                              double* out, hipStream_t s);
constexpr int kBkgMaxBox = 4096;
constexpr int kBkgMaxCells = 4096;
constexpr int kBkgMaxFilter = 7;
constexpr int kBkgZoomLine = 520;
struct BkgArgs {
  const void* data;
  const unsigned char* mask;
  int B, H, W, bh, bw, fh, fw, ny, nx, maxiters, clip;
  double sigma;
  double excl_count;
  double* ws;
  size_t ws_stride;
  int* wsi;
  double *bkg, *rms, *mesh, *rms_mesh, *medians;
  int* status;
};
hipError_t launch_bkg_boxstats(const BkgArgs& a, int f32, hipStream_t s);
hipError_t launch_bkg_mesh(const BkgArgs& a, hipStream_t s);
hipError_t launch_bkg_zoom(const BkgArgs& a, hipStream_t s);
constexpr int kSegMaxKernel = 7;
constexpr int kSegChunk = 2048;
struct SegConvArgs {
  const void* data;
  const double* kernel;
  double* out;
  int B, H, W, kh, kw;
};
struct SegArgs {
  const void* data;
  const double* thr_map;
  const unsigned char* mask;
  double thr;
  int B, H, W, npixels, conn, nblk;
  int* lab;
  int* area;
  int* blk;
  int* labels_out;
  int* nlabels_out;
};
struct SegCatArgs {
  const double* data;
  const double* conv;
  const int* labels;
  const int* nlabels;
  int B, H, W, cap;
  int* icols;
  double* fcols;
  int* status;
};
hipError_t launch_seg_convolve(const SegConvArgs& a, int f32, hipStream_t s);
hipError_t launch_seg_detect(const SegArgs& a, int f32, hipStream_t s);
hipError_t launch_seg_catalog(const SegCatArgs& a, hipStream_t s);
struct PsfModel;
hipError_t launch_psf_stamps(const PsfModel& m, const double* xy, int n, int spatial,
                             int normalize, double* out, hipStream_t s);
hipError_t phase_prof(unsigned long long* out, int n, int reset);
hipError_t launch_persist(const SolveArgs& a, int K, size_t lds, hipStream_t s, unsigned* queue,
                          unsigned* done, int grid);
hipError_t persist_resident_per_cu(const SolveArgs& a, int K, size_t lds, int* per_cu);
hipError_t persist_phase_prof(unsigned long long* out, int n, int reset);
void persist_kernels_all(std::vector<const void*>& f);

static_assert(sizeof(bsgp_state_header) <= BSGP_STATE_HEADER_BYTES, "state header overflows");

struct StateLayout {
  size_t bytes, discr, crit, times, flags, x, g, xtf, pw, gn, bkg;
};
inline size_t state_pad16(size_t v) { return (v + 15) / 16 * 16; }
inline StateLayout state_layout(size_t N, int storage, bool bmap, int hist_cap) {
  const size_t vb = storage == BSGP_STORAGE_F32 ? 4 : 8;
  StateLayout L{};
  size_t o = BSGP_STATE_HEADER_BYTES;
  auto take = [&](size_t n) {
    const size_t at = o;
    o += state_pad16(n);
    return at;
  };
  L.discr = take((size_t)hist_cap * 8);
  L.crit = take((size_t)hist_cap * 8);
  L.times = take((size_t)hist_cap * 8);
  L.flags = take((size_t)hist_cap * 4);
  L.x = take(N * vb);
  L.g = take(N * vb);
  L.xtf = take(N * vb);
  L.pw = take(N * vb);
  L.gn = take(N * 8);
  L.bkg = bmap ? take(N * 8) : 0;
  L.bytes = o;
  return L;
}

struct StateArgs {
  unsigned char* rec;
  size_t rec_bytes;
  const int* index;
  StateLayout L;
  double* ws;
  size_t slot_stride, vec_stride;
  ImgState* st;
  int N, storage, bmap, hist_cap, T, conv_mode, H, W, beta0_given;
  int M1;
  bsgp_outputs out;
  bsgp_params prm;
  int* active;
};
hipError_t launch_state_save(const StateArgs& a, int B, hipStream_t s);
hipError_t launch_state_load(const StateArgs& a, int B, hipStream_t s);
hipError_t launch_state_post(const StateArgs& a, int B, unsigned* queue, unsigned* done,
                             int done_it, int* done_host, int seq, hipStream_t s);

constexpr int kCoopGroups = 4;
constexpr int kCoopBlock = 512;
__host__ __device__ inline int plan_block(const Geo& g) { return g.coop ? kCoopBlock : kBlock; }
inline bool app_static_plan(const Geo& g, int storage) {
  const bool app_n = g.fp.n == 400 || g.fp.n == 480 || g.fq.n == 400 || g.fq.n == 480;
  return !g.coop && storage == BSGP_STORAGE_F64 && app_n;
}

}

extern "C" {
size_t bsgp_c512_args_size(void);
int bsgp_c512_block(void);
int bsgp_c512_waves(void);
hipError_t bsgp_c512_launch_setup(const void* a, size_t lds, hipStream_t s);
hipError_t bsgp_c512_launch_iteration(const void* a, int K, size_t lds, hipStream_t s,
                                      hipEvent_t* ev);
hipError_t bsgp_c512_team_resident(int storage, size_t lds, int* per_cu);
hipError_t bsgp_c512_set_lds_limit(size_t bytes);
hipError_t bsgp_c512_launch_persist(const void* a, int K, size_t lds, hipStream_t s,
                                    unsigned* queue, unsigned* done, int grid);
hipError_t bsgp_c512_persist_resident(const void* a, int K, size_t lds, int* per_cu);
hipError_t bsgp_c512_persist_set_lds_limit(size_t bytes);
size_t bsgp_app_args_size(void);
hipError_t bsgp_app_launch_persist(const void* a, int K, size_t lds, hipStream_t s,
                                   unsigned* queue, unsigned* done, int grid);
hipError_t bsgp_app_persist_resident(const void* a, int K, size_t lds, int* per_cu);
hipError_t bsgp_app_persist_set_lds_limit(size_t bytes);
hipError_t bsgp_app_phase_prof(unsigned long long* out, int n, int reset);
hipError_t bsgp_c512_phase_prof(unsigned long long* out, int n, int reset);
}
```

### beta-sgp_amd/csrc/bsgp_kernels.hpp

```cpp
#pragma once

#include <hip/hip_runtime.h>

#include <type_traits>
#include <vector>

#include "bsgp_device.hpp"
#include "bsgp_internal.hpp"

namespace bsgp {


#ifndef BSGP_LS1_PRE
#define BSGP_LS1_PRE false
#endif
constexpr int kLs1Jch = 1;
#ifndef BSGP_COL_ATTR
#define BSGP_COL_ATTR
#endif
#ifndef BSGP_LS_ATTR
#define BSGP_LS_ATTR __attribute__((amdgpu_waves_per_eu(COOP ? 1 : ((K <= 2 && !ADAPT) ? 3 : 2))))
#endif
#ifndef BSGP_LS1_K2
#define BSGP_LS1_K2 0
#endif
#ifndef BSGP_STREAM_NT
#define BSGP_STREAM_NT 0
#endif
constexpr int kLsLanes = 32;
#ifndef BSGP_ACC_SERIES
#define BSGP_ACC_SERIES 0
#endif
constexpr int kLsAccJch = 1;
constexpr bool kLsAccPf = true;
#ifndef BSGP_LS1_PIPE
#define BSGP_LS1_PIPE false
#endif
#ifndef BSGP_LSACC_PIPE
#define BSGP_LSACC_PIPE false
#endif
#ifndef BSGP_BB_PIPE
#define BSGP_BB_PIPE false
#endif
constexpr int kProjU = 4;
constexpr int kDirJch = 4;
constexpr bool kDirPf = true;
constexpr bool kDirComp = true;
constexpr bool kLsComp = false;
constexpr bool kBbComp = false;
#ifndef BSGP_BB_PRE
#define BSGP_BB_PRE false
#endif
constexpr int kBbJch = 1;

__device__ __forceinline__ double clipX(double x, double lo, double hi) {
  double X = (x < lo) ? lo : x;
  return (X > hi) ? hi : X;
}

__device__ __forceinline__ double realtime_s() {
  return (double)__builtin_amdgcn_s_memrealtime() * 1e-8;
}

template <int U, class LD, class CP>
__device__ __forceinline__ void stream_range(int p0, int p1, LD&& ld, CP&& cp) {
  using T = decltype(ld(0));
  for (int b = p0 + threadIdx.x; b < p1; b += kBlock * U) {
    T v[U];
#pragma unroll
    for (int u = 0; u < U; ++u) v[u] = ld(min(b + u * kBlock, p1 - 1));
#pragma unroll
    for (int u = 0; u < U; ++u) {
      const int p = b + u * kBlock;
      if (p < p1) cp(p, v[u]);
    }
  }
}
template <int U, class LD, class CP>
__device__ __forceinline__ void stream2(const Part& D, int npair, LD&& ld, CP&& cp) {
  if (D.T == 1) {
    stream_range<U>(0, npair, ld, cp);
    return;
  }
  for (int p0 = D.m * D.cp; p0 < npair; p0 += D.T * D.cp)
    stream_range<U>(p0, p0 + D.cp < npair ? p0 + D.cp : npair, ld, cp);
}

template <bool NT = false>
__device__ __forceinline__ double2 ld2(const double* a, int p) {
  return ldp<NT>(reinterpret_cast<const double2*>(a) + p);
}
template <bool NT = false>
__device__ __forceinline__ double2 ld2(const float* a, int p) {
  const float2 f = ldp<NT>(reinterpret_cast<const float2*>(a) + p);
  return double2{(double)f.x, (double)f.y};
}

template <bool NT = false, class T>
__device__ __forceinline__ double opt_ld(bool on, const T* a, int i, double off) {
  const double v = (double)ldp<NT>(a + (on ? i : 0));
  return on ? v : off;
}
template <bool NT = false, class T>
__device__ __forceinline__ double2 opt_ld2(bool on, const T* a, int p, double off) {
  const double2 v = ld2<NT>(a, on ? p : 0);
  return on ? v : double2{off, off};
}
template <bool NT = false>
__device__ __forceinline__ double g_raw(bool g32, const double* gns, int i) {
  const unsigned int* w = reinterpret_cast<const unsigned int*>(gns) + (g32 ? i : 2 * i);
// ... 51 lines not shown
  double alpha, lo, hi, lam_p;
  ProjClip clip;
  __device__ __forceinline__ void cd_of(double x, double g, double& c, double& dia) const {
    const double X = Xones ? 1.0 : clipX(x, lo, hi);
    const double D = 1 / X;
    const double y = x - alpha * (X * g);
    c = y * D;
    dia = D;
  }
  __device__ __forceinline__ void yx(double x, double g, double& y, double& X) const {
    X = Xones ? 1.0 : clipX(x, lo, hi);
    y = x - alpha * (X * g);
  }
  __device__ __forceinline__ double pv(double y, double X, double lam) const {
    double v = fma(lam, X, y);
    v = (0.0 > v) ? 0.0 : v;
    if (clip.has_sat) v = (clip.satv < v) ? clip.satv : v;
    return v;
  }
  __device__ __forceinline__ double d(double x, double g) const {
    double y;
    if (proj) {
      double c, dia;
      cd_of(x, g, c, dia);
      y = clip(c, dia, lam_p);
    } else {
      const double X = Xones ? 1.0 : clipX(x, lo, hi);
      y = x - alpha * (X * g);
      if (y < 0) y = 0;
    }
    return y - x;
  }
};

__device__ __forceinline__ Dir make_dir(const SolveArgs& A, const ImgState& st) {
  Dir D;
  D.Xones = st.Xones != 0;
  D.proj = A.prm.proj_type == 1;
  D.alpha = st.alpha;
  D.lo = st.lo;
  D.hi = st.hi;
  D.lam_p = st.lam_p;
  D.clip = ProjClip{A.prm.has_sat != 0, A.prm.ccd_sat_level / st.sc - 2.220446049250313e-16};
  if (A.prm.gn_f32 && A.prm.proj_type == 0 && st.iter == 1) {
    D.lo = (double)(float)st.lo;
    D.hi = (double)(float)st.hi;
  }
  return D;
}

__device__ __forceinline__ Objective make_obj(const SolveArgs& A, double beta) {
  Objective o;
  o.variant = A.prm.variant;
  o.f32g = A.prm.gn_f32 != 0;
  o.set_beta(beta);
  return o;
}

__device__ __forceinline__ Team make_team(const SolveArgs& A, int img, const ImgState& st) {
  Team t;
  t.T = A.T;
  t.m = A.T == 1 ? 0 : (int)(blockIdx.x % (unsigned)A.T);
  t.part = A.tpart ? A.tpart + (size_t)img * kPartBufs * (A.T + 8) * kMaxRed : nullptr;
  t.flags = A.T <= 1 ? 0 : A.T <= kTeamFlags ? 1 : A.T >= 8 ? 2 : 0;
  t.ctr = A.tctr ? A.tctr + (size_t)img * kTeamWords : nullptr;
  t.base = (unsigned int)st.bar_base;
  t.nb = 0;
  t.fail = A.tfail;
  t.grp = (int)(blockIdx.x & 7u);
  const unsigned first = blockIdx.x - (unsigned)t.m;
  const int r = (int)(((unsigned)t.grp - (first & 7u)) & 7u);
  t.ng = t.T / 8 + (r < (t.T & 7) ? 1 : 0);
  t.G = t.T < 8 ? t.T : 8;
  return t;
}
__device__ __forceinline__ int team_img(const SolveArgs& A) {
  return A.img0 + (A.T == 1 ? (int)blockIdx.x : (int)(blockIdx.x / (unsigned)A.T));
}
__device__ __forceinline__ void team_end(ImgState& st, const Team& t) {
  if (t.T > 1 && t.m == 0 && threadIdx.x == 0 && t.nb > 0)
    st.bar_base = (int)(t.base + (unsigned int)t.nb);
}
__device__ __forceinline__ bool leader(const Team& t) { return t.m == 0 && threadIdx.x == 0; }

#define BSGP_LDS_VIEWS(A)                                                           \
  extern __shared__ __attribute__((aligned(16))) char smem[];                      \
  cd* lds = reinterpret_cast<cd*>(smem + (A).g.tw2);                               \
  double* red = reinterpret_cast<double*>(smem + (A).g.tw2 + (A).lds_fft_bytes)

template <class TERM>
__device__ __forceinline__ float np_f32_sum(const PwProg& pw, TERM&& term, float* vals, const Part& D, Team& tm) {
  const int* lv = pw.prog;
  const int* nd = lv + 2 * pw.nleaf;
  const int* off = nd + 2 * pw.nnode;
  const int* roots = off + pw.nlev + 1;
  const int q = D.gt0 + (int)threadIdx.x;
  const int j = q & 7;
  const int lstride = D.gts >> 3;
  const int nrounds = (pw.nleaf + lstride - 1) / lstride;
  for (int it = 0; it < nrounds; ++it) {
    const int l = (q >> 3) + it * lstride;
    const bool act = l < pw.nleaf;
    const int s0 = act ? lv[2 * l] : 0, n = act ? lv[2 * l + 1] : 0;
    float r = 0.0f;
    if (n >= 8) {
      const int m8 = n - (n % 8);
      r = term(s0 + j);
      for (int i = 8 + j; i < m8; i += 8) r += term(s0 + i);
    }
    float s = r + __shfl_xor(r, 1);
    s = s + __shfl_xor(s, 2);
    s = s + __shfl_xor(s, 4);
    if (act && j == 0) {
      float res;
      int i;
      if (n < 8) {
        res = 0.0f;
        i = 0;
      } else {
        res = s;
        i = n - (n % 8);
      }
      for (; i < n; ++i) res += term(s0 + i);
      vals[l] = res;
    }
  }
  team_sync(tm);
  for (int h = 0; h < pw.nlev; ++h) {
    for (int k = off[h] + D.gt0 + (int)threadIdx.x; k < off[h + 1]; k += D.gts)
      vals[pw.nleaf + k] = vals[nd[2 * k]] + vals[nd[2 * k + 1]];
    team_sync(tm);
  }
  float res = 0.0f;
  for (int c = 0; c < pw.nchunk; ++c) res = res + vals[roots[c]];
  return res;
}

__device__ __forceinline__ void write_counters(const SolveArgs& A, const ImgState& st, int img,
                                               int T) {
  if (!A.out.counters) return;
  int64_t* c = A.out.counters + (size_t)img * 8;
  c[0] = st.E_p;
  c[1] = st.E_ls;
  c[2] = st.ls_passes;
  c[3] = st.status |
         ((A.tfail && __hip_atomic_load(A.tfail, __ATOMIC_RELAXED, __HIP_MEMORY_SCOPE_AGENT)) ? 4
                                                                                              : 0);
  c[4] = st.ls_series;
  c[5] = T;
  c[6] = st.proj_passes;
  c[7] = st.proj_list;
}

__device__ __forceinline__ void count_stopped(const SolveArgs& A) {
  if (atomicSub(A.active, 1) == 1 && A.done_host)
    __hip_atomic_store(A.done_host, A.seq, __ATOMIC_RELAXED, __HIP_MEMORY_SCOPE_SYSTEM);
}

template <bool COOP, class V>
__device__ __forceinline__ void setup_phase(const SolveArgs& A, int img) {
  BSGP_LDS_VIEWS(A);
  const Geo& G = A.g;
  const bsgp_params& P = A.prm;
  const int N = G.H * G.W;
  const int tid = threadIdx.x;
  const bool bmap = P.bkg_is_map != 0;
// ... 344 lines not shown
      const int kl = cnt < nl ? cnt : nl;
      for (; k < kl; ++k) t[0] += D.pv(qy[k * kBlock + tl], qX[k * kBlock + tl], lam);
    }
    for (; k + 4 <= cnt; k += 4) {
      double yv[4], Xv[4];
#pragma unroll
      for (int u = 0; u < 4; ++u) {
        yv[u] = ly[(size_t)(k + u) * LS + gt];
        Xv[u] = lX[(size_t)(k + u) * LS + gt];
      }
#pragma unroll
      for (int u = 0; u < 4; ++u) t[0] += D.pv(yv[u], Xv[u], lam);
    }
    for (; k < cnt; ++k) t[0] += D.pv(ly[(size_t)k * LS + gt], lX[(size_t)k * LS + gt], lam);
    team_sum<1>(t, red, tm);
    PH_ADD(11, tl0);
    const double lin = SA + lam * SB;
    return (hs ? lin + nsat * satv : lin) + t[0];
  };
  auto sumf = [&](double lam) {
    double S;
    if (calls == 0) {
      const double lams[3] = {lam, lam - 1.0, lam + 1.0};
      double Sv[3];
      const bool wide = tm.T > 1 && (long)N <= (long)kProjWidePx * LS;
      bool guess = wide || (isfinite(lam_prev) && lam_prev != 0.0);
      const double w = kProjGuessW * fabs(lam_prev);
      double gL = wide ? lams[1] : lam_prev - w, gU = wide ? lams[2] : lam_prev + w;
      const double lh = D.alpha * lam_ratio;
      if (!wide && isfinite(lh) && lh != 0.0) {
        gL = lh - kProjW1 * fabs(lh);
        gU = lh + kProjW1 * fabs(lh);
        const double pk = kappa * lh;
        if (isfinite(pk) && pk != 0.0) {
          gL = fmin(gL, pk - kProjW2 * fabs(pk));
          gU = fmax(gU, pk + kProjW2 * fabs(pk));
        }
        guess = true;
      }
      const double slope = pass(std::integral_constant<int, 3>{}, lams, Sv, guess, gL, gU);
      S = Sv[0];
      xl0 = lams[1];
      xs0 = Sv[1];
      xl1 = lams[2];
      xs1 = Sv[2];
      note(lams[1], Sv[1]);
      note(lams[2], Sv[2]);
      lamN = slope > 0.0 ? lam - (S - flux) / slope : NAN;
    } else if (lam == xl0) {
      S = xs0;
    } else if (lam == xl1) {
      S = xs1;
    } else {
      if (!isfinite(first_lam)) first_lam = lam;
      if (have && lam >= cL && lam <= cU) {
        S = leval(lam);
        list_reads += (int64_t)nstr;
      } else {
        bool split = false;
        double qL = 0.0, qU = 0.0;
        if (first_miss && isfinite(lamN)) {
          qL = fmin(lam, lamN);
          qU = fmax(lam, lamN);
          split = true;
        } else if (isfinite(Lk) && isfinite(Uk)) {
          qL = fmin(Lk, Uk);
          qU = fmax(Lk, Uk);
          split = true;
        }
        first_miss = false;
        const double lams[1] = {lam};
        double Sv[1];
        (void)pass(std::integral_constant<int, 1>{}, lams, Sv, split, qL, qU);
        S = Sv[0];
      }
    }
    ++calls;
    note(lam, S);
    return S;
  };
  return project_df_fn(sumf, flux, 0.0, 1.0, 1e-11, 0, 0, A.prm.max_projs);
}

template <bool COOP, class V, bool LL = true, unsigned POL = 0>
__device__ __forceinline__ void dir_phase(const SolveArgs& A, int img) {
  constexpr bool kO16 = (POL & kNtO16) != 0, kO8 = (POL & kNtO8) != 0;
  BSGP_LDS_VIEWS(A);
  ImgState& st = A.st[img];
  PH_T(tk0);
  Team tm = make_team(A, img, st);
  const Geo& G = A.g;
  const Part Pt = make_part(tm, G.nfw, G.W);
  const bsgp_params& P = A.prm;
  const int N = G.H * G.W;
  const int npair = (N + 1) / 2;
  const bool odd = (N & 1) != 0;
  Bufs<V> B = slot_bufs<V>(A, img, st.par, st.par_tf);
  Dir D = make_dir(A, st);
  const double flux = st.flux;
  int evals = 0;
  int64_t ppass = 0, plist_reads = 0;
  double lam_ratio = 0.0, kappa = 0.0;
  if (P.proj_type == 1 && A.plist != nullptr) {
    double first_lam = NAN;
    ProjOut po = cached_projection<V, LL, POL>(A, img, Pt, tm, D, B, red, lds, st.lam_p, flux, npair,
                                          odd, N, ppass, plist_reads, st.lam_ratio, st.kappa,
                                          first_lam);
    D.lam_p = po.lam;
    evals = po.evals;
    lam_ratio = D.alpha != 0.0 ? po.lam / D.alpha : 0.0;
    kappa = (isfinite(first_lam) && po.lam != 0.0) ? first_lam / po.lam : 0.0;
  } else if (P.proj_type == 1) {
    const V* xa = B.xa;
    const V* ga = B.ga;
    auto psum = [&](double lam) {
      double s[1] = {0.0};
      stream2<4>(
          Pt, npair,
          [&](int p) {
            struct Ld {
              double2 x, g;
            } v;
            v.x = ld2<(POL & kNtPJ) != 0>(xa, p);
            v.g = ld2<(POL & kNtPJ) != 0>(ga, p);
            return v;
          },
          [&](int p, const auto& v) {
            double c, d;
            D.cd_of(v.x.x, v.g.x, c, d);
            s[0] += D.clip(c, d, lam);
            if (!odd || 2 * p + 1 < N) {
              D.cd_of(v.x.y, v.g.y, c, d);
              s[0] += D.clip(c, d, lam);
            }
          });
      team_sum<1>(s, red, tm);
      return s[0];
    };
    ProjOut po = project_df_fn(psum, flux, 0.0, 1.0, 1e-11, 0, 0, P.max_projs);
    D.lam_p = po.lam;
    evals = po.evals;
    ppass = po.evals;
  }
  PH_ADD(0, tk0);
  PH_T(tk1);
  double gd[1] = {0.0};
  row_fwd2<kDirJch, kDirPf, kDirComp, COOP, false, 22, POL>(
      G, Pt, G.H, G.W, G.sld, B.spec, lds,
      [&](int r, int j) {
        const int i = r * G.W + j;
        return double2{(double)ldp<kO8>(B.xa + i), (double)ldp<kO8>(B.ga + i)};
      },
      [&](int, int, const double2& v) {
        const double d = D.d(v.x, v.y);
        gd[0] += d * v.y;
        return d;
      },
      [&](int r, int j) {
        const int p = (r * G.W + j) >> 1;
        const double2 x = ld2<kO16>(B.xa, p), g = ld2<kO16>(B.ga, p);
        return Two<double2>{double2{x.x, g.x}, double2{x.y, g.y}};
      });
  if (row_wide<COOP>(G)) gd[0] = split_undo(gd[0]);
  team_sum<1>(gd, red, tm);
  PH_ADD(1, tk1);
  PH_ADD(2, tk0);
  team_end(st, tm);
  if (leader(tm)) {
    for (int k = 0; k < P.M_alpha - 1; ++k) st.Valpha[k] = st.Valpha[k + 1];
    for (int k = 0; k < P.M - 1; ++k) st.Fold[k] = st.Fold[k + 1];
    st.Fold[P.M - 1] = st.fv;
    st.epoch += 1;
    st.lam_p = D.lam_p;
    st.lam_ratio = isfinite(lam_ratio) ? lam_ratio : 0.0;
    st.kappa = isfinite(kappa) ? kappa : 0.0;
    st.E_p += evals;
    st.proj_passes += ppass;
    st.proj_list += plist_reads;
    st.gd = gd[0];
  }
}

template <bool COOP, class V>
__global__ void __launch_bounds__(kBlock) k_dir(SolveArgs A) {
  const int img = team_img(A);
  if (A.st[img].stop) return;
  load_tw_lds(A.g);
  dir_phase<COOP, V>(A, img);
}

template <bool COOP>
__global__ void __launch_bounds__(kBlock) BSGP_COL_ATTR k_col(SolveArgs A, int transpose) {
  BSGP_LDS_VIEWS(A);
  const int img = A.img0 + (A.Tc == 1 ? (int)blockIdx.x : (int)(blockIdx.x / (unsigned)A.Tc));
  const ImgState& st = A.st[img];
  if (st.stop) return;
  PH_T(tc0);
  Team tm{};
  tm.T = A.Tc;
  tm.m = A.Tc == 1 ? 0 : (int)(blockIdx.x % (unsigned)A.Tc);
  const Bufs<double> B = slot_bufs<double>(A, img, 0);
  load_tw_lds(A.g);
  col_conv<COOP>(A.g, make_part(tm, A.g.nfc, A.g.W), B.spec, tf_of(A.g, img, transpose), lds);
  PH_ADD(3, tc0);
}

template <int K, int MODE, bool ADAPT, bool COOP, class V, bool SB = false, bool PRED = false,
          unsigned POL = 0>
__device__ __forceinline__ void ls_phase(const SolveArgs& A, int img) {
  constexpr bool kO8 = (POL & kNtO8) != 0, kW = (POL & kNtW) != 0;
  BSGP_LDS_VIEWS(A);
  ImgState& st = A.st[img];
  PH_T(tk0);
  Team tm = make_team(A, img, st);
  const Geo& G = A.g;
  const Part Pt = make_part(tm, G.nfw, G.W);
  const bsgp_params& P = A.prm;
  const int N = G.H * G.W;
  const int npair = (N + 1) / 2;
  const bool odd = (N & 1) != 0;
  const bool bmap = SB ? false : P.bkg_is_map != 0;
  const double lr_st = st.lr;
  constexpr bool adapt = ADAPT;
  Bufs<V> B = slot_bufs<V>(A, img, st.par, st.par_tf);
  const double bks_scalar = st.bks_scalar;
  const double flux = st.flux;
  const double gd = st.gd;
  const int g32 = st.g32;
  const double gsc = st.sc, grc = 1.0 / st.sc, gfill = st.gfill;
  auto gdec1 = [&](float v) __attribute__((always_inline)) {
    const double g = v;
    return g > 0 ? (g32 == 2 ? div_rn(g, gsc, grc) : g) : gfill;
  };
  auto gdec = [&](double r) __attribute__((always_inline)) {
    return g32 ? gdec1(__int_as_float(__double2loint(r))) : r;
  };
  double fr = st.Fold[0];
  for (int k = 1; k < P.M; ++k) fr = py_max2(fr, st.Fold[k]);
  const int ls_cap = A.ls_cap;
  Objective obj = make_obj(A, st.beta);
  double lam = 1.0;
  double f_acc = 0.0;
  int nls = 0, passes = 0, status = 0, series_evals = 0;
  bool accepted = false;
  bool acc_series = false;
  constexpr int NT = 2 * K + 2;
  double konst = st.konst;
  const bool k32 = ADAPT && P.gn_f32 != 0;
  float* const xbc =
      (k32 && tm.T == 1 && sizeof(V) == 8) ? reinterpret_cast<float*>(B.pw) + N : nullptr;
  auto konst32 = [&](double b) -> double {
    const float sf = (float)(1 / (b * (b - 1)));
    const float bf = (float)b;
    return (double)np_f32_sum(
        A.pw,
        [&](int i) {
          if (xbc) return sf * xbc[i];
          const double g = g32 ? gdec1(reinterpret_cast<const float*>(B.gns)[i]) : B.gns[i];
          return sf * libm_powf((float)g, bf);
        },
        reinterpret_cast<float*>(B.pw), Pt, tm);
  };
  auto bderiv = [&](double den, double g, double b, int i) __attribute__((always_inline)) {
    return k32 ? beta_deriv_px_f32(den, g, b, xbc ? xbc + i : nullptr) : beta_deriv_px(den, g, b);
  };
  constexpr int MS = 6;
  constexpr double kSeriesRho = 0.01;
  constexpr double kSeriesTail = 8.673617379884035e-19;
  const bool tail_bound = obj.beta >= 0.0 && obj.beta <= MS + 2;
  const bool series = (MODE == 3 || MODE == 4) && !adapt && P.ls_series != 0;
  double* ser = red + kWaves * kMaxRed + kMaxRed + 8;
  double rho = INFINITY;
  constexpr bool kPredBuild = PRED && BSGP_LS1_K2 && !COOP && !ADAPT &&
                              (MODE == 3 || MODE == 4) && sizeof(V) == 8;
  constexpr double kLsStagLam = 1e-4;
  int pred = 0;
  if constexpr (kPredBuild) {
    if (series && tm.T == 1 && A.ls_predict != 0) {
      const double ll = st.lam;
      const int lp = A.ls_predict;
      pred = lp == 2 ? 1 : lp == 3 ? 2 : ll == 1.0 ? (lp == 5 ? 0 : 1) : ll < kLsStagLam ? (lp >= 4 ? 2 : 0) : 0;
    }
  }
  const bool k2 = BSGP_LS1_K2 && !COOP && series && pred == 0;
  const double lam2 = lam * P.beta;
  double f2 = NAN;
  bool have2 = false;
  constexpr int O2 = 4 + 2 * (MS + 1);
  constexpr int N1 = O2 + ((BSGP_LS1_K2 && !COOP) ? 2 : 0);
  auto ls_replay = [&](bool with_mom) __attribute__((always_inline)) {
    if constexpr (kPredBuild) {
      PH_T(tr0);
      double t1[N1];
#pragma unroll
      for (int k = 0; k < N1; ++k) t1[k] = 0.0;
      double umax = 0.0;
      const int w = threadIdx.x >> 6, lane = threadIdx.x & 63;
      if (w < G.nfw) {
// ... 63 lines not shown
            return q;
          },
          [&](int r, int j, double v, const SpIn& q) {
            const int i = r * G.W + j;
            stp<kW>(B.dtf + i, (V)v);
            const double g = gdec(q.g);
            const double xt = q.x0 + lam * v;
            const double den = xt + q.bkv;
            const double p = fpow(den, bm1s);
            ts[0] += obj.c1 * (den * p);
            ts[1] += (MODE == 4 ? (double)(obj.c2f * (float)g) : obj.c2 * g) * p;
            stp<kW>(xs + i, (V)xt);
            stp<kW>(ps + i, (V)p);
            return g * (p / den);
          });
      team_sum<2>(ts, red, tm);
      PH_ADD(37, tk0);
      ++passes;
      ++nls;
      const double f1 = obj.combine(konst, ts[0], ts[1], flux, (double)N);
      if (f1 <= fr + P.gamma * lam * gd || lam < 1e-12) {
        f_acc = f1;
        accepted = true;
        spec_acc = true;
      } else {
        lam = lam * P.beta;
      }
    }
  }
  if (pred != 1) {
    double t1[N1];
#pragma unroll
    for (int k = 0; k < N1; ++k) t1[k] = 0.0;
    double umax = 0.0;
    struct LsIn {
      double x0, g, p0, bkv;
    };
    row_inv2<BSGP_LS1_PRE, kLs1Jch, kLsComp, COOP, BSGP_LS1_PIPE, 13, POL>(
        G, Pt, B.spec, lds,
        [&](int r, int j) {
          const int i = r * G.W + j;
          LsIn q;
          q.x0 = ldp<kO8>(B.xtf + i);
          q.g = g_raw<kO8>(g32, B.gns, i);
          q.p0 = opt_ld<kO8>(series, B.pw, i, 0.0);
          q.bkv = opt_ld<kO8>(bmap, B.bks, i, bks_scalar);
          return q;
        },
        [&](int r, int j, double v, const LsIn& q) {
      const int i = r * G.W + j;
      stp<kW>(B.dtf + i, (V)v);
      const double g = gdec(q.g);
      const double x0 = q.x0;
      const double bkv = q.bkv;
      const double xt = x0 + lam * v;
      obj.template terms_m<MODE>(xt, xt + bkv, g, &t1[0]);
      if constexpr (adapt) {
        if (!k32) t1[2] += obj.konst(g);
        t1[3] += bderiv(xt + bkv, g, obj.beta, i);
      }
      if (series) {
        const double a = x0 + bkv;
        const double u = v / a;
        const double p0 = q.p0;
        const double A0 = a * p0, B0 = (MODE == 4 ? (double)(obj.c2f * (float)g) : g) * p0;
        double um = 1.0;
#pragma unroll
        for (int m = 0; m <= MS; ++m) {
          t1[4 + m] += A0 * um;
          t1[4 + MS + 1 + m] += B0 * um;
          um *= u;
        }
        const double au = fabs(u);
        umax = (au > umax || au != au || !(a > 0)) ? (a > 0 ? au : INFINITY) : umax;
        if constexpr (BSGP_LS1_K2 && !COOP) {
          if (k2) {
            const double x2 = x0 + lam2 * v;
            obj.template terms_m<MODE>(x2, x2 + bkv, g, &t1[O2]);
          }
        }
      }
    });
    if (series) {
      team_sum_max<N1>(t1, umax, red, tm, 25);
      rho = umax;
    } else {
      team_sum<N1>(t1, red, tm);
    }
    PH_ADD(4, tk0);
    if (series && threadIdx.x == 0) {
      for (int m = 0; m <= MS; ++m) {
        ser[m] = t1[4 + m];
        ser[MS + 1 + m] = t1[4 + MS + 1 + m];
      }
    }
    if (adapt) konst = k32 ? konst32(obj.beta) : t1[2];
    ++passes;
    ++nls;
    const double f1 = obj.combine(konst, t1[0], t1[1], flux, (double)N);
    if (f1 <= fr + P.gamma * lam * gd || lam < 1e-12) {
      f_acc = f1;
      accepted = true;
    } else {
      lam = lam * P.beta;
      if (adapt) {
        const double bgrad = (obj.beta == 0.0 || obj.beta == 1.0) ? 0.0 : t1[3] / N;
        obj.set_beta(obj.beta - lr_st * bgrad);
      }
      if constexpr (BSGP_LS1_K2 && !COOP) {
        if (k2) {
          f2 = obj.combine(konst, t1[O2], t1[O2 + 1], flux, (double)N);
          have2 = true;
        }
      }
    }
  }
#ifdef BSGP_PHASE_PROF
  if (threadIdx.x == 0 && pred) atomicAdd(&g_phase[pred == 1 ? 32 : 33], 1ull);
#endif
  if (pred == 1 && !accepted) {
    ls_replay(true);
#ifdef BSGP_PHASE_PROF
    if (threadIdx.x == 0) atomicAdd(&g_phase[35], 1ull);
#endif
  }
  const bool have_mom = !spec_acc;
  if (series && have_mom && threadIdx.x == 0) {
    double c0 = 1.0, c1 = 1.0;
    ser[2 * (MS + 1)] = 1.0;
    ser[3 * (MS + 1)] = 1.0;
    for (int m = 1; m <= MS; ++m) {
      c0 = c0 * (obj.beta - (m - 1)) / m;
      c1 = c1 * (obj.beta - 1 - (m - 1)) / m;
      ser[2 * (MS + 1) + m] = c0;
      ser[3 * (MS + 1) + m] = c1;
    }
    const double c7p = fabs(c0 * (obj.beta - MS) / (MS + 1));
    const double c7q = fabs(c1 * (obj.beta - 1 - MS) / (MS + 1));
    const double tp = c7p * ser[MS] / ser[0], tq = c7q * ser[2 * MS + 1] / ser[MS + 1];
    ser[4 * (MS + 1)] = (ser[0] > 0 && ser[MS + 1] > 0 && tp == tp && tq == tq)
                            ? (tp > tq ? tp : tq)
                            : INFINITY;
  }
  __syncthreads();
  const double tail_c = (series && tail_bound) ? ser[4 * (MS + 1)] : INFINITY;
  auto series_ok = [&](double l) __attribute__((always_inline)) {
    const double lu = l * rho;
    if (lu <= kSeriesRho) return true;
    if (!(lu <= 0.5)) return false;
    double l7 = l;
#pragma unroll
    for (int m = 1; m <= MS; ++m) l7 *= l;
    return l7 * rho * tail_c / (1.0 - lu) <= kSeriesTail;
  };
  PH_T(tk1);
  if (pred == 2 && !accepted && !series_ok(lam)) {
    ls_replay(false);
#ifdef BSGP_PHASE_PROF
    if (threadIdx.x == 0) atomicAdd(&g_phase[36], 1ull);
#endif
  }
  while (!accepted) {
    if (have2 && !series_ok(lam)) {
      have2 = false;
      ++nls;
      if (f2 <= fr + P.gamma * lam * gd || lam < 1e-12) {
        f_acc = f2;
// ... 121 lines not shown
      obj.set_beta(obj.beta - lr_st * bgrad);
    }
    if (nls > ls_cap) {
      status = 1;
      break;
    }
  }
  PH_ADD(5, tk1);
  PH_T(tk2);
  const double lam_acc = lam;
  const bool pw_series = BSGP_ACC_SERIES && acc_series && MODE >= 3;
  const double bm1 = obj.beta - 1;
  struct AcIn {
    double x, d, g, bkv, p0;
  };
  if (!spec_acc) {
    row_fwd2<kLsAccJch, kLsAccPf, kLsComp, COOP, BSGP_LSACC_PIPE, 16, POL>(
        G, Pt, G.H, G.W, G.sld, B.spec, lds,
        [&](int r, int j) {
          const int i = r * G.W + j;
          AcIn q;
          q.x = ldp<kO8>(B.xtf + i);
          q.d = ldp<kO8>(B.dtf + i);
          q.g = g_raw<kO8>(g32, B.gns, i);
          q.bkv = opt_ld<kO8>(bmap, B.bks, i, bks_scalar);
          q.p0 = opt_ld<kO8>(pw_series, B.pw, i, 0.0);
          return q;
        },
        [&](int r, int j, const AcIn& q) {
          const int i = r * G.W + j;
          const double xt = q.x + lam_acc * q.d;
          stp<kW>(B.xtf + i, (V)xt);
          const double den = xt + q.bkv;
          const double g = gdec(q.g);
          if (P.variant != BSGP_VARIANT_BETA) return g / den;
          double p;
          if (pw_series) {
            const double t = lam_acc * (q.d / (q.x + q.bkv));
            double h = 1.0;
  #pragma unroll
            for (int m = MS; m >= 1; --m) h = fma(fma(obj.beta, 1.0 / m, -1.0) * t, h, 1.0);
            p = q.p0 * h;
          } else {
            p = fpow(den, bm1);
          }
          stp<kW>(B.pw + i, (V)p);
          return g * (p / den);
        });
  }
  PH_ADD(6, tk2);
  if (A.fuse_col & 2) {
    PH_T(tc0);
    team_sync(tm);
    col_conv<COOP, POL>(G, Pt, B.spec, tf_of(G, img, 1), lds);
    PH_ADD(3, tc0);
  }
  PH_ADD(7, tk0);
  team_end(st, tm);
  if (leader(tm)) {
    if (A.out.flags)
      A.out.flags[(size_t)img * (P.MAXIT + 1) + st.iter] =
          ((f_acc >= fr) ? 1 : 0) | ((nls < 0xffff ? nls : 0xffff) << 8);
    st.fv = f_acc;
    st.beta = obj.beta;
    st.konst = konst;
    st.lam = lam_acc;
    if (spec_acc) st.par_tf ^= 1;
    st.E_ls += nls;
    st.ls_passes += passes;
    st.ls_series += series_evals;
    st.status |= status;
  }
}

template <int K, int MODE, bool ADAPT, bool COOP, class V>
__global__ void __launch_bounds__(kBlock) BSGP_LS_ATTR k_ls(SolveArgs A) {
  const int img = team_img(A);
  if (A.st[img].stop) return;
  load_tw_lds(A.g);
  ls_phase<K, MODE, ADAPT, COOP, V>(A, img);
}


template <bool COOP, class V, unsigned POL = 0>
__device__ __forceinline__ void bb_phase(const SolveArgs& A, int img) {
  constexpr bool kO16 = (POL & kNtO16) != 0, kO8 = (POL & kNtO8) != 0, kW = (POL & kNtW) != 0;
  BSGP_LDS_VIEWS(A);
  ImgState& st = A.st[img];
  PH_T(tk0);
  Team tm = make_team(A, img, st);
  const Geo& G = A.g;
  const Part Pt = make_part(tm, G.nfw, G.W);
  const bsgp_params& P = A.prm;
  const int N = G.H * G.W;
  const int tid = threadIdx.x;
  const bool beta_obj = P.variant == BSGP_VARIANT_BETA;
  Bufs<V> B = slot_bufs<V>(A, img, st.par, st.par_tf);
  Dir D = make_dir(A, st);
  const double lam = st.lam;
  const double lo = st.lo, hi = st.hi;
  const double alpha = st.alpha;
  double vmin_ring = INFINITY;
  for (int k = 0; k < P.M_alpha - 1; ++k) vmin_ring = k ? py_min2(vmin_ring, st.Valpha[k]) : st.Valpha[0];
  const int iter = st.iter;
  const double tau0 = st.tau, init_lr = st.init_lr, lr0 = st.lr;
  const int epoch = st.epoch;
  const double fv = st.fv, Dcoeff = st.Dcoeff, tol = st.tol, fold_last = st.Fold[P.M - 1];
  const double sc = st.sc;
  double bb[6] = {0, 0, 0, 0, 0, 0};
  struct BbIn {
    double p, x, g;
  };
  row_inv2<BSGP_BB_PRE, kBbJch, kBbComp, COOP, BSGP_BB_PIPE, 19, POL>(
      G, Pt, B.spec, lds,
      [&](int r, int j) {
        const int i = r * G.W + j;
        BbIn q;
        q.p = opt_ld<kO8>(beta_obj, B.pw, i, 1.0);
        q.x = ldp<kO8>(B.xa + i);
        q.g = ldp<kO8>(B.ga + i);
        return q;
      },
      [&](int r, int j, double at, const BbIn& q) {
    const int i = r * G.W + j;
    const double gnew = q.p - at;
    const double x = q.x, g = q.g;
    const double d = D.d(x, g);
    const double sk = lam * d;
    const double xn = x + lam * d;
    const double yk = gnew - g;
    const double X = clipX(xn, lo, hi);
    const double Dd = 1 / X;
    const double sk2 = sk * Dd;
    const double yk2 = yk * X;
    bb[0] += sk2 * yk;
    bb[1] += yk2 * sk;
    bb[2] += sk2 * sk2;
    bb[3] += yk2 * yk2;
    bb[4] += sk * sk;
    bb[5] += xn * xn;
    stp<kW>(B.xb + i, (V)xn);
    stp<kW>(B.gb + i, (V)gnew);
  },
      [&](int r, int j) {
        const int p = (r * G.W + j) >> 1;
        const double2 pw = opt_ld2<kO16>(beta_obj, B.pw, p, 1.0), x = ld2<kO16>(B.xa, p),
                      g = ld2<kO16>(B.ga, p);
        return Two<BbIn>{BbIn{pw.x, x.x, g.x}, BbIn{pw.y, x.y, g.y}};
      });
  if (row_wide<COOP>(G)) {
#pragma unroll
    for (int k = 0; k < 6; ++k) bb[k] = split_undo(bb[k]);
  }
  team_sum<6>(bb, red, tm);
  PH_ADD(8, tk0);
  double alpha1, alpha2;
  if (bb[0] <= 0) {
    alpha1 = py_min2(10 * alpha, P.alpha_max);
  } else {
    alpha1 = py_min2(P.alpha_max, py_max2(P.alpha_min, bb[2] / bb[0]));
  }
  if (bb[1] <= 0) {
    alpha2 = py_min2(10 * alpha, P.alpha_max);
  } else {
    alpha2 = py_min2(P.alpha_max, py_max2(P.alpha_min, bb[1] / bb[3]));
  }
  const double vmin = P.M_alpha > 1 ? py_min2(vmin_ring, alpha2) : alpha2;
  double tau = tau0, anew;
  if (iter <= 20) {
    anew = vmin;
  } else if (alpha2 / alpha1 < tau) {
    anew = vmin;
    tau = tau * 0.9;
  } else {
// ... 12 lines not shown
    loop = crit > tol;
  } else if (P.stop_criterion == 3) {
    crit = (fold_last - fv) / fv;
    loop = crit > tol && crit >= 0;
  } else if (P.stop_criterion == 4) {
    crit = dk;
    loop = dk > tol;
  }
  if (it2 > P.MAXIT) loop = false;
  if (!loop) {
    double* xo = A.out.x + (size_t)img * N;
    for (int i = Pt.gt0 + tid; i < N; i += Pt.gts) xo[i] = B.xa[i] * sc;
  }
  team_end(st, tm);
  if (leader(tm)) {
    const size_t M1 = (size_t)P.MAXIT + 1;
    A.out.discr[img * M1 + it2 - 1] = dk;
    if (A.out.times) A.out.times[img * M1 + it2 - 1] = realtime_s() - st.t0;
    if (A.out.crit) A.out.crit[img * M1 + it2 - 1] = crit;
    st.Valpha[P.M_alpha - 1] = alpha2;
    st.alpha = anew;
    st.tau = tau;
    st.lr = lr;
    st.iter = it2;
    if (loop) {
      st.par ^= 1;
      st.Xones = 0;
    } else {
      st.stop = 1;
      A.out.iters[img] = it2 - 1;
      if (A.out.beta_final) A.out.beta_final[img] = st.beta;
      write_counters(A, st, img, tm.T);
      count_stopped(A);
    }
  }
}

template <bool COOP, class V>
__global__ void __launch_bounds__(kBlock) k_bb(SolveArgs A) {
  const int img = team_img(A);
  if (A.st[img].stop) return;
  load_tw_lds(A.g);
  bb_phase<COOP, V>(A, img);
}

static __global__ void k_ring_init(unsigned* queue, int nimg, int img0) {
  unsigned long long* ring = reinterpret_cast<unsigned long long*>(queue + 4);
  const int i = blockIdx.x * blockDim.x + threadIdx.x;
  if (i == 0) {
    queue[0] = 0;
    queue[1] = (unsigned)nimg;
  }
  if (i < nimg) ring[i] = ((unsigned long long)i << 32) | (unsigned)(img0 + i);
}

#ifndef BSGP_PERSIST_ATTR
#define BSGP_PERSIST_ATTR __attribute__((amdgpu_waves_per_eu(COOP ? 2 : 3)))
#endif

__device__ __forceinline__ unsigned long long ld_sc1_u64(const unsigned long long* p) {
  return __hip_atomic_load((gu64*)p, __ATOMIC_RELAXED, __HIP_MEMORY_SCOPE_AGENT);
}

struct ArgRef {
  unsigned lo, hi;
};
__device__ __forceinline__ ArgRef kernarg_ref() {
  const unsigned long long a = (unsigned long long)__builtin_amdgcn_kernarg_segment_ptr();
  return ArgRef{(unsigned)a, (unsigned)(a >> 32)};
}
__device__ __forceinline__ const SolveArgs& args_of(ArgRef r) {
  typedef const __attribute__((address_space(4))) SolveArgs* KP;
  const unsigned lo = (unsigned)__builtin_amdgcn_readfirstlane((int)r.lo);
  const unsigned hi = (unsigned)__builtin_amdgcn_readfirstlane((int)r.hi);
  const unsigned long long a = ((unsigned long long)hi << 32) | (unsigned long long)lo;
  KP p = (KP)a;
  asm volatile("" : "+s"(p));
  return *(const SolveArgs*)p;
}
template <bool COOP, class V>
__device__ __attribute__((noinline)) void persist_setup(ArgRef r, int img) {
  setup_phase<COOP, V>(args_of(r), __builtin_amdgcn_readfirstlane(img));
}
template <bool COOP, class V, unsigned POL>
__device__ __attribute__((noinline)) void persist_dir(ArgRef r, int img) {
  dir_phase<COOP, V, false, POL>(args_of(r), __builtin_amdgcn_readfirstlane(img));
}
template <bool COOP, unsigned POL>
__device__ __attribute__((noinline)) void persist_col_a(ArgRef r, int img) {
  const SolveArgs& A = args_of(r);
  img = __builtin_amdgcn_readfirstlane(img);
  BSGP_LDS_VIEWS(A);
  (void)red;
  Team tm{};
  tm.T = 1;
  const Bufs<double> Bd = slot_bufs<double>(A, img, 0);
  PH_T(tc0);
  col_conv<COOP, POL>(A.g, make_part(tm, COOP ? A.g.nfc : A.g.nfw, A.g.W), Bd.spec,
                      tf_of(A.g, img, 0), lds);
  PH_ADD(3, tc0);
}
template <int K, int MODE, bool ADAPT, bool COOP, class V, bool SB, unsigned POL>
__device__ __attribute__((noinline)) void persist_ls(ArgRef r, int img) {
  ls_phase<K, MODE, ADAPT, COOP, V, SB, true, POL>(args_of(r),
                                                   __builtin_amdgcn_readfirstlane(img));
}
template <bool COOP, class V, unsigned POL>
__device__ __attribute__((noinline)) void persist_bb(ArgRef r, int img) {
  bb_phase<COOP, V, POL>(args_of(r), __builtin_amdgcn_readfirstlane(img));
}

constexpr unsigned kDoneStop = 0x40000000u;
__device__ __forceinline__ unsigned ld_sc1_u32(const unsigned* p) {
  return __hip_atomic_load((gu32*)p, __ATOMIC_RELAXED, __HIP_MEMORY_SCOPE_AGENT);
}

template <bool COOP, int K, int MODE, bool ADAPT, class V, bool SB = false>
__global__ void __launch_bounds__(kBlock) BSGP_PERSIST_ATTR k_persist(SolveArgs A,
                                                                        unsigned* queue,
                                                                        unsigned* done) {
  BSGP_LDS_VIEWS(A);
  (void)red;
  __shared__ int s_img;
  __shared__ unsigned s_k;
  constexpr unsigned kPol = ADAPT ? 0u : (unsigned)(BSGP_STREAM_NT);
  const int tid = threadIdx.x;
  const Geo& G = A.g;
  load_tw_lds(G);
  const unsigned nimg = (unsigned)A.nimg;
  const unsigned fs = A.fold_setup ? 1u : 0u;
  const unsigned total = ((unsigned)A.prm.MAXIT + fs) * nimg;
  const bool use_ring = A.prm.stop_criterion >= 2 && A.prm.stop_criterion <= 4;
  unsigned long long* ring = reinterpret_cast<unsigned long long*>(queue + 4);
  for (;;) {
    PH_T(tq);
    if (tid == 0) {
      int img = -1;
      unsigned k = 0;
      if (use_ring) {
        const unsigned h = atomicAdd(queue, 1u);
        unsigned long long e = ld_sc1_u64(ring + h % nimg);
        unsigned spins = 0;
        while ((unsigned)(e >> 32) != h) {
          __builtin_amdgcn_s_sleep(2);
          if ((++spins & 63u) == 0) {
            if (__hip_atomic_load((gi32*)A.active, __ATOMIC_RELAXED, __HIP_MEMORY_SCOPE_AGENT) <=
                0)
              break;
            if (__hip_atomic_load((gi32*)A.tfail, __ATOMIC_RELAXED, __HIP_MEMORY_SCOPE_AGENT) ||
                spins > A.spin_limit) {
              __hip_atomic_store((gi32*)A.tfail, 1, __ATOMIC_RELAXED, __HIP_MEMORY_SCOPE_AGENT);
              break;
            }
          }
          e = ld_sc1_u64(ring + h % nimg);
        }
        if ((unsigned)(e >> 32) == h) {
          img = (int)(unsigned)e;
          __builtin_amdgcn_fence(__ATOMIC_ACQUIRE, "agent");
          asm volatile("s_waitcnt vmcnt(0)" ::: "memory");
          if (A.st[img].stop) img = -2;
        }
      } else {
        unsigned t = atomicAdd(queue, 1u);
        if (t < total && __hip_atomic_load((gi32*)A.active, __ATOMIC_RELAXED,
                                           __HIP_MEMORY_SCOPE_AGENT) <= 0)
          t = total;
        if (t < total) {
          img = A.img0 + (int)(t % nimg);
          const unsigned need = t / nimg;
          k = need + 1;
          unsigned d = ld_sc1_u32(done + img), spins = 0;
          while (d < need) {
            __builtin_amdgcn_s_sleep(2);
            d = ld_sc1_u32(done + img);
            if (((++spins & 1023u) == 0 || spins > A.spin_limit) &&
                (__hip_atomic_load((gi32*)A.tfail, __ATOMIC_RELAXED, __HIP_MEMORY_SCOPE_AGENT) ||
                 spins > A.spin_limit)) {
              __hip_atomic_store((gi32*)A.tfail, 1, __ATOMIC_RELAXED, __HIP_MEMORY_SCOPE_AGENT);
              img = -1;
              break;
            }
          }
          if (img >= 0) {
            if (d & kDoneStop) {
              img = -2;
            } else {
              __builtin_amdgcn_fence(__ATOMIC_ACQUIRE, "agent");
              asm volatile("s_waitcnt vmcnt(0)" ::: "memory");
              if (!fs && need == 0 && A.st[img].stop) {
                __hip_atomic_store((gu32*)(done + img), kDoneStop, __ATOMIC_RELAXED,
                                   __HIP_MEMORY_SCOPE_AGENT);
                img = -2;
              }
            }
          }
        }
      }
      s_img = img;
      s_k = k;
    }
    __syncthreads();
    const int img = s_img;
    const unsigned k = s_k;
    __syncthreads();
    PH_ADD(31, tq);
    if (img == -1) break;
    if (img < 0) continue;
    const ArgRef ar = kernarg_ref();
    if (fs && k == 1) {
      persist_setup<COOP, V>(ar, img);
    } else {
      persist_dir<COOP, V, kPol>(ar, img);
      __syncthreads();
      persist_col_a<COOP, kPol>(ar, img);
      persist_ls<K, MODE, ADAPT, COOP, V, SB, kPol>(ar, img);
      __syncthreads();
      persist_bb<COOP, V, kPol>(ar, img);
    }
    asm volatile("s_waitcnt vmcnt(0)" ::: "memory");
    __syncthreads();
    if (tid == 0) {
      const bool stopped = A.st[img].stop != 0;
      if (use_ring) {
        if (!stopped) {
          __builtin_amdgcn_fence(__ATOMIC_RELEASE, "agent");
          asm volatile("s_waitcnt vmcnt(0)" ::: "memory");
          const unsigned t = atomicAdd(queue + 1, 1u);
          __hip_atomic_store((gu64*)(ring + t % nimg),
                             ((unsigned long long)t << 32) | (unsigned)img, __ATOMIC_RELAXED,
                             __HIP_MEMORY_SCOPE_AGENT);
        }
      } else {
        __builtin_amdgcn_fence(__ATOMIC_RELEASE, "agent");
        asm volatile("s_waitcnt vmcnt(0)" ::: "memory");
        __hip_atomic_store((gu32*)(done + img), stopped ? (kDoneStop | k) : k, __ATOMIC_RELAXED,
                           __HIP_MEMORY_SCOPE_AGENT);
      }
    }
  }
}

template <class V>
__global__ void __launch_bounds__(kBlock) k_persist_finalize(SolveArgs A) {
  const int img = A.img0 + (int)blockIdx.x;
  ImgState& st = A.st[img];
  if (st.stop) return;
  const int N = A.g.H * A.g.W;
  const Bufs<V> B = slot_bufs<V>(A, img, st.par, st.par_tf);
  double* xo = A.out.x + (size_t)img * N;
  for (int i = threadIdx.x; i < N; i += kBlock) xo[i] = (double)B.xa[i] * st.sc;
  __syncthreads();
  if (threadIdx.x == 0) {
    st.status |= 4;
    st.stop = 1;
    A.out.iters[img] = st.iter - 1;
    if (A.out.beta_final) A.out.beta_final[img] = st.beta;
    write_counters(A, st, img, 1);
  }
}

inline int ls_mode(const SolveArgs& a, bool* adapt) {
  const bsgp_params& P = a.prm;
  *adapt = P.adapt_beta && P.variant == BSGP_VARIANT_BETA;
  const bool special = a.in.beta0 ? !P.beta0_general : (P.betaParam == 0.0 || P.betaParam == 1.0);
  return P.variant == BSGP_VARIANT_KL ? 0 : special ? -1 : P.gn_f32 ? 4 : 3;
}

template <class V, bool COOP = false>
inline const void* persist_kernel(int K, int mode, bool adapt, bool scalar_bkg = false) {
  if (!COOP && scalar_bkg && !adapt && mode == 3 && K >= 2)
    return (const void*)k_persist<COOP, 2, 3, false, V, true>;
  if (adapt) return (const void*)k_persist<COOP, 1, -1, true, V>;
  if (K > 2) K = 2;
  if (mode == -1) return (const void*)k_persist<COOP, 2, -1, false, V>;
  if (mode == 0) return K == 1 ? (const void*)k_persist<COOP, 1, 0, false, V>
                               : (const void*)k_persist<COOP, 2, 0, false, V>;
  if (mode == 4) return K == 1 ? (const void*)k_persist<COOP, 1, 4, false, V>
                               : (const void*)k_persist<COOP, 2, 4, false, V>;
  return K == 1 ? (const void*)k_persist<COOP, 1, 3, false, V>
                : (const void*)k_persist<COOP, 2, 3, false, V>;
}
template <class V, bool COOP = false>
inline void persist_kernels(std::vector<const void*>& f) {
  for (int adapt = 0; adapt < 2; ++adapt)
    for (int mode : {-1, 0, 3, 4})
      for (int K : {1, 2}) f.push_back(persist_kernel<V, COOP>(K, mode, adapt != 0));
  if (!COOP) f.push_back(persist_kernel<V, COOP>(2, 3, false, true));
}
template <class V, bool COOP = false>
inline hipError_t launch_persist_t(const SolveArgs& a, int K, size_t lds, hipStream_t s,
                                   unsigned* queue, unsigned* done, int grid) {
  if (a.prm.stop_criterion >= 2 && a.prm.stop_criterion <= 4)
    hipLaunchKernelGGL(k_ring_init, dim3((a.nimg + 255) / 256), dim3(256), 0, s, queue, a.nimg,
// ... 133 lines not shown
```

### beta-sgp_amd/csrc/bsgp_persist.hip

```cpp
#include <hip/hip_runtime.h>

#include <vector>

#ifndef BSGP_LS1_K2
#define BSGP_LS1_K2 1
#endif
#ifndef BSGP_STREAM_NT
#define BSGP_STREAM_NT 21
#endif
#include "bsgp_kernels.hpp"

namespace bsgp {

hipError_t launch_persist_f32(const SolveArgs& a, int K, size_t lds, hipStream_t s,
                              unsigned* queue, unsigned* done, int grid);
const void* persist_kernel_f32(int K, int mode, bool adapt, bool scalar_bkg);
void persist_kernels_f32(std::vector<const void*>& f);

hipError_t launch_persist(const SolveArgs& a, int K, size_t lds, hipStream_t s, unsigned* queue,
                          unsigned* done, int grid) {
  if (a.g.coop) return bsgp_c512_launch_persist(&a, K, lds, s, queue, done, grid);
  if (app_static_plan(a.g, a.storage))
    return bsgp_app_launch_persist(&a, K, lds, s, queue, done, grid);
  if (a.storage == BSGP_STORAGE_F32) return launch_persist_f32(a, K, lds, s, queue, done, grid);
  return launch_persist_t<double>(a, K, lds, s, queue, done, grid);
}

hipError_t persist_resident_per_cu(const SolveArgs& a, int K, size_t lds, int* per_cu) {
  if (a.g.coop) return bsgp_c512_persist_resident(&a, K, lds, per_cu);
  if (app_static_plan(a.g, a.storage)) return bsgp_app_persist_resident(&a, K, lds, per_cu);
  bool adapt = false;
  const int mode = ls_mode(a, &adapt);
  const bool sb = !a.prm.bkg_is_map;
  const void* f = a.storage == BSGP_STORAGE_F32 ? persist_kernel_f32(K, mode, adapt, sb)
                                                : persist_kernel<double>(K, mode, adapt, sb);
  return hipOccupancyMaxActiveBlocksPerMultiprocessor(per_cu, f, kBlock, lds);
}

hipError_t persist_phase_prof_f32(unsigned long long* out, int n, int reset);
hipError_t persist_phase_prof(unsigned long long* out, int n, int reset) {
#ifdef BSGP_PHASE_PROF
  hipError_t e = hipMemcpyFromSymbol(out, HIP_SYMBOL(g_phase), n * sizeof(unsigned long long));
  if (e == hipSuccess && reset) {
    unsigned long long z[kPhaseSlots] = {};
    e = hipMemcpyToSymbol(HIP_SYMBOL(g_phase), z, sizeof z);
  }
  if (e == hipSuccess) {
    unsigned long long c[kPhaseSlots] = {};
    e = persist_phase_prof_f32(c, n, reset);
    for (int i = 0; i < n; ++i) out[i] += c[i];
  }
  if (e == hipSuccess) {
    unsigned long long c[kPhaseSlots] = {};
    e = bsgp_app_phase_prof(c, n, reset);
    for (int i = 0; i < n; ++i) out[i] += c[i];
  }
  return e;
#else
  for (int i = 0; i < n; ++i) out[i] = 0;
  (void)reset;
  return hipSuccess;
#endif
}

void persist_kernels_all(std::vector<const void*>& f) {
  persist_kernels<double>(f);
  persist_kernels_f32(f);
}

}
```

### beta-sgp_amd/sgp.py

```python
import errno
import logging
import math
import os

import numpy as np

import _bsgp as _B
import fits_io

DEFAULT_PARAMS = (1000, 1e-4, 0.4, 1e-5, 1e5, 1e1, 3, 0.5, 1)
DEFAULT_COLUMNS = ['label', 'xcentroid', 'ycentroid', 'sky_centroid',
                   'bbox_xmin', 'bbox_xmax', 'bbox_ymin', 'bbox_ymax',
                   'area', 'semimajor_sigma', 'semiminor_sigma',
                   'orientation', 'eccentricity', 'min_value', 'max_value',
                   'local_background', 'segment_flux', 'segment_fluxerr', 'ellipticity',
                   'fwhm']

LS_SPEC_DEFAULT = 2
LS_SERIES_DEFAULT = 1
def _hw_queues():
    try:
        return int(os.environ.get("GPU_MAX_HW_QUEUES", "4"))
    except ValueError:
        return 4


STREAMS_DEFAULT = 8 if _hw_queues() >= 8 else 4
TEAM_DEFAULT = 0
PROJ_CACHE_DEFAULT = 1
GN_COMPACT_DEFAULT = 1
PERSIST_DEFAULT = 1


def _check_psf(psf):
    total = np.sum(psf) if isinstance(psf, np.ndarray) and psf.flags.c_contiguous \
        else np.sum(psf.flatten())
    checkPSF = np.abs(total - 1.)
    tolCheckPSF = 1e4 * np.finfo(float).eps
    if checkPSF > tolCheckPSF:
        errmsg = f"\n\tsum(psf) - 1. = {checkPSF}, tolerance = {tolCheckPSF}"
        raise ValueError(f'PSF is not normalized! Provide a normalized PSF! {errmsg}')


def _bkg_kind(bkg, shape):
    b = np.asarray(bkg)
    if b.size == 1:
        return "scalar", b
    if b.size == int(np.prod(shape)):
        return "map", b.reshape(shape)
    raise ValueError(f"bkg of shape {b.shape} does not broadcast to the image shape {shape}")


def _scalar_dtype(v):
    if isinstance(v, (np.generic, np.ndarray)):
        return np.asarray(v).dtype
    return np.dtype(np.float64) if isinstance(v, float) else np.dtype(np.int64)


def _np1_scalar_div(a, b):
    rt = np.promote_types(_scalar_dtype(a), _scalar_dtype(b))
    if rt.kind != "f":
        rt = np.dtype(np.float64)
    return rt.type(np.asarray(a, dtype=rt) / np.asarray(b, dtype=rt))


def _prelude_host(gn, bkg, init_recon, flux, stop_criterion, scale_data):
    gn = np.asarray(gn)
    gn = gn.astype(gn.dtype.newbyteorder("="), copy=True)
    dt = gn.dtype
    bk = np.asarray(bkg)
    bk = bk.astype(bk.dtype.newbyteorder("="))
    if init_recon == 0:
        x = np.zeros_like(gn)
    elif init_recon == 1:
        np.random.seed(42)
        x = np.random.randn(*gn.shape)
    elif init_recon == 2:
        x = gn.copy()
    else:
        if flux is None:
            v = _np1_scalar_div(np.sum(gn - (bk.astype(dt) if bk.ndim == 0 else bk)), gn.size)
        else:
            v = _np1_scalar_div(flux, gn.size)
        x = np.full(gn.shape, v).astype(dt)
    gn = gn.flatten()
    x = x.flatten()
# ... 276 lines not shown
def sgp(gn, psf, bkg, init_recon=0, proj_type=0, stop_criterion=0, MAXIT=500, gamma=1e-4,
        beta=0.4, alpha=1.3, alpha_min=1e-5, alpha_max=1e5, M_alpha=3, tau=0.5, M=1,
        max_projs=1000, save=False, obj=None, verbose=True, flux=None, ccd_sat_level=None,
        scale_data=True, errflag=False, tol_convergence=1e-4, use_original_SGP_Afunction=True):
    x, it, discr, times, extra = _run(_B.BSGP_VARIANT_KL, gn, psf, bkg, init_recon, proj_type,
                                      stop_criterion, MAXIT, gamma, beta, alpha, alpha_min,
                                      alpha_max, M_alpha, tau, M, max_projs, save, obj, verbose,
                                      flux, ccd_sat_level, scale_data, errflag, tol_convergence,
                                      use_original_SGP_Afunction, {})
    return x, it, discr, times, extra["err"]


def sgp_betaDiv(gn, psf, bkg, init_recon=0, proj_type=0, stop_criterion=0, MAXIT=500,
                gamma=1e-4, beta=0.4, alpha=1.3, alpha_min=1e-5, alpha_max=1e5, M_alpha=3,
                tau=0.5, M=1, max_projs=1000, save=False, obj=None, verbose=True, flux=None,
                ccd_sat_level=None, scale_data=True, errflag=False, adapt_beta=True,
                betaParam=1.005, lr=1e-3, lr_exp_param=0.1, schedule_lr=False,
                tol_convergence=1e-4, use_original_SGP_Afunction=True):
    bkw = dict(adapt_beta=adapt_beta, betaParam=betaParam, lr=lr, lr_exp_param=lr_exp_param,
               schedule_lr=schedule_lr)
    x, it, discr, times, extra = _run(_B.BSGP_VARIANT_BETA, gn, psf, bkg, init_recon, proj_type,
                                      stop_criterion, MAXIT, gamma, beta, alpha, alpha_min,
                                      alpha_max, M_alpha, tau, M, max_projs, save, obj, verbose,
                                      flux, ccd_sat_level, scale_data, errflag, tol_convergence,
                                      use_original_SGP_Afunction, bkw)
    print(f'Beta parameter in beta-divergence (final value): {extra["beta"]}')
    print(f'No. of iterations: {it}')
    return x, it, discr, times, None


def _dev1(a):
    return _B.to_dev(np.asarray(a, dtype=np.float64).ravel())


def betaDiv(y, x, betaParam):
    _B.require_gpu()
    out = _B.beta_div_dev(_dev1(y), _dev1(x), float(betaParam))
    return np.float64(out.cpu().numpy()[0])


def betaDivDeriv(y, x, betaParam):
    if betaParam == 0 or betaParam == 1:
        return 0
    _B.require_gpu()
    shape = np.shape(y)
    out = _B.beta_div_deriv_dev(_dev1(y), _dev1(x), float(betaParam))
    return out.cpu().numpy().reshape(shape)


def betaDivDerivwrtY(AT, den_arg, gn_arg, betaParam):
    _B.require_gpu()
    shape = np.shape(den_arg)
    p1, w = _B.grad_parts_dev(_dev1(den_arg), _dev1(gn_arg), float(betaParam))
    return p1.cpu().numpy().reshape(shape) - AT(x=w.cpu().numpy().reshape(shape))


def lr_schedule(init_lr, k, epoch):
    return init_lr * math.exp(-k * epoch)


def _bkg_batch(bkgs, Bn, H, W):
    torch = _B.torch
    t = (bkgs.to(device="cuda", dtype=torch.float64) if torch.is_tensor(bkgs)
         else _B.to_dev(np.asarray(bkgs, dtype=np.float64)))
    shape = tuple(t.shape)
    if t.dim() == 0 or (t.dim() == 1 and shape[0] in (1, Bn)):
        return t.reshape(-1).expand(Bn).contiguous()
    if shape in ((H, W), (1, H, W)):
        return t.reshape(1, H, W).expand(Bn, H, W).contiguous()
    if shape == (Bn, H, W):
        return t.contiguous()
    raise ValueError(f"bkg of shape {shape} fits neither [B]={Bn} scalars nor [B, H, W] maps "
                     f"of {H}x{W} images")


def _solve_batch(variant, gns, psf, bkgs, betaParams=None, flux=None, init_recon=0, proj_type=0,
                 stop_criterion=0, MAXIT=500, gamma=1e-4, beta=0.4, alpha=1.3, alpha_min=1e-5,
                 alpha_max=1e5, M_alpha=3, tau=0.5, M=1, max_projs=1000, verbose=True,
                 ccd_sat_level=None, scale_data=True, tol_convergence=1e-4,
                 use_original_SGP_Afunction=True, adapt_beta=False, betaParam=1.005, lr=1e-3,
                 lr_exp_param=0.1, schedule_lr=False, ls_spec=None, ls_series=None,
                 streams=None, team=None, proj_cache=None, gn_compact=None,
                 device_out=False, profile=False, storage="f64", gn_f32=None, save=False,
                 errflag=False, obj=None, persistent=None, return_state=False):
    torch = _B.torch
    if save or errflag:
        raise ValueError("save / errflag are single-image options: use sgp / sgp_betaDiv")
    per_image = (psf.dim() if torch.is_tensor(psf) else np.ndim(psf)) == 3
    if return_state and per_image:
        raise ValueError("return_state=True needs one shared PSF: a solver state of per-image "
                         "PSFs is not supported")
    _B.require_gpu()
    if not per_image:
        psf = np.asarray(psf.cpu().numpy() if torch.is_tensor(psf) else psf)
        _B.check_psf_once(psf, _check_psf)
    if gn_f32 is None:
        gn_f32 = (gns.dtype == torch.float32) if torch.is_tensor(gns) else \
            np.asarray(gns).dtype.kind == "f" and np.asarray(gns).dtype.itemsize == 4
    if gn_f32:
        f64b = (bkgs.dtype == torch.float64) if torch.is_tensor(bkgs) else \
            (np.asarray(bkgs).dtype.kind == "f" and np.asarray(bkgs).dtype.itemsize == 8)
        bnd = bkgs.dim() if torch.is_tensor(bkgs) else np.ndim(bkgs)
        if not f64b or (init_recon == 3 and flux is None and bnd <= 1):
            raise ValueError("float32 images in a batch need float64 backgrounds, and a flux for "
                             "init_recon=3 with scalar backgrounds (numpy computes those parts "
                             "in float32 from the background; solve such images one at a time "
                             "with sgp_betaDiv / sgp)")
    if torch.is_tensor(gns):
        gns = gns.to(device="cuda", dtype=torch.float64).contiguous()
    else:
        gns = _B.to_dev(np.asarray(gns, dtype=np.float64))
    if gns.dim() != 3:
        raise ValueError("gns must be a batch [B, H, W]")
    Bn, H, W = gns.shape
    mode = _B.BSGP_CONV_CIRCULAR if use_original_SGP_Afunction else _B.BSGP_CONV_LINEAR_FILL
    bkgs = _bkg_batch(bkgs, Bn, H, W)
    bkg_is_map = bkgs.dim() == 3
    prm = _params(variant, init_recon, proj_type, stop_criterion, MAXIT, gamma, beta, alpha,
                  alpha_min, alpha_max, M_alpha, tau, M, max_projs, verbose, ccd_sat_level,
                  scale_data, tol_convergence, adapt_beta=adapt_beta, betaParam=betaParam, lr=lr,
                  lr_exp_param=lr_exp_param, schedule_lr=schedule_lr, bkg_is_map=bkg_is_map,
                  ls_spec=ls_spec, ls_series=ls_series, streams=streams,
                  team=team, proj_cache=proj_cache, gn_compact=gn_compact, betaParams=betaParams,
                  persistent=persistent)
    if gn_f32:
        prm.gn_f32 = 1
        prm.scale_data = 1 if scale_data else 0
        prm.flux_f32 = int(_flux_is_f32(flux) if not torch.is_tensor(flux)
                           else flux.dtype == torch.float32)
    x0 = None
    if init_recon == 1:
        np.random.seed(42)
        x0 = _B.to_dev(np.broadcast_to(np.random.randn(H, W), (Bn, H, W)))
    b0 = None if betaParams is None else _B.to_dev(np.broadcast_to(
        np.asarray(betaParams, dtype=np.float64), (Bn,)))
    if flux is None:
        fl = None
    elif torch.is_tensor(flux):
        fl = flux.to(device="cuda", dtype=torch.float64).reshape(-1).expand(Bn).contiguous()
    else:
        fl = _B.to_dev(np.broadcast_to(np.asarray(flux, dtype=np.float64), (Bn,)))
    state = None
    if per_image:
        if len(psf) != Bn:
            raise ValueError("one PSF per image: psf must be [B, kh, kw]")
        plan = _B.per_image_plan(H, W, psf, mode, storage=storage)
        out = plan.solve(gns, bkgs, prm, flux=fl, x0=x0, beta0=b0, profile=profile)
    else:
        with _B.lease_plan(H, W, psf, mode, storage=storage) as plan:
            out = plan.solve(gns, bkgs, prm, flux=fl, x0=x0, beta0=b0, profile=profile)
            state = _B.SolverState(plan.save_state(Bn), psf) if return_state else None
    return _finish_batch(out, state, device_out)


def _finish_batch(out, state, device_out):
    torch = _B.torch
    if device_out:
        if state is not None:
            out["state"] = state
        return out
    prof = {k: out.pop(k) for k in ("kernel_ms", "launches") if k in out}
    torch.cuda.current_stream().synchronize()
    _B.check_status(out["counters"])
    res = {k: (v.cpu().numpy() if v is not None else None) for k, v in out.items()}
    res.update(prof)
    if state is not None:
        res["state"] = state
    return res


SolverState = _B.SolverState


def state_params(variant, **kw):
    d = dict(init_recon=0, proj_type=0, stop_criterion=0, MAXIT=500, gamma=1e-4, beta=0.4,
             alpha=1.3, alpha_min=1e-5, alpha_max=1e5, M_alpha=3, tau=0.5, M=1, max_projs=1000,
             verbose=True, ccd_sat_level=None, scale_data=True, tol_convergence=1e-4)
    d.update({k: kw.pop(k) for k in list(kw) if k in d})
    code = {"kl": _B.BSGP_VARIANT_KL, "beta": _B.BSGP_VARIANT_BETA}[variant]
    return _params(code, **d, **kw)


_RESUME_TUNING =("streams", "persistent", "proj_cache", "ls_spec", "team")


def sgp_resume(state, MAXIT, images=None, device_out=False, return_state=False, **tuning):
    torch = _B.torch
    bad = sorted(set(tuning) - set(_RESUME_TUNING))
    if bad:
        raise ValueError(f"sgp_resume: {bad} cannot change on a resume (only "
                         f"{list(_RESUME_TUNING)} may be given)")
    state.validate()
    h = state.header
    prm = state.params()
    prm.MAXIT = int(MAXIT)
    prm.team = int(h["T"][0])
    for k, v in tuning.items():
        if v is not None:
            setattr(prm, k, int(v))
    if prm.variant == _B.BSGP_VARIANT_BETA and prm.adapt_beta:
        prm.ls_spec = 1
    _B.require_gpu()
    H, W = state.shape
    dev = state.to_device()
    index = None
    if images is not None:
        idx = np.atleast_1d(np.asarray(images)).astype(np.int64)
        if idx.size < 1 or idx.min() < -len(state) or idx.max() >= len(state):
            raise ValueError(f"images must index the {len(state)} saved images")
        index = torch.from_numpy((idx % len(state)).astype(np.int32)).to("cuda")
    storage = int(h["storage"][0])
    with _B.lease_plan(H, W, state.psf, int(h["conv_mode"][0]), storage=storage) as plan:
        out = plan.resume(dev.records, prm, index=index)
        new = (_B.SolverState(plan.save_state(out["iters"].numel()), state.psf)
               if return_state else None)
    return _finish_batch(out, new, device_out)


def on_devices(devices, n, work):
    import threading
    devices = list(devices)
    k = len(devices)
    if k == 0:
        raise ValueError("devices is empty")
    bounds = [(n * j // k, n * (j + 1) // k) for j in range(k)]
    res, errs = [None] * k, [None] * k

    def run(j):
        try:
            with _B.torch.cuda.device(devices[j]):
                res[j] = work(devices[j], *bounds[j])
                _B.torch.cuda.current_stream().synchronize()
        except BaseException as e:
            errs[j] = e

    threads = [threading.Thread(target=run, args=(j,)) for j in range(k)
               if bounds[j][1] > bounds[j][0]]
    for t in threads:
        t.start()
    for t in threads:
        t.join()
    for e in errs:
        if e is not None:
            raise e
    return [r for r, (lo, hi) in zip(res, bounds) if hi > lo]


def _shard(v, lo, hi, Bn):
    if v is None:
        return None
    shape = tuple(v.shape) if hasattr(v, "shape") else np.shape(v)
    if len(shape) in (1, 3) and shape[0] == Bn and Bn > 1:
        return v[lo:hi]
    return v


def _solve_sharded(variant, gns, psf, bkgs, devices, betaParams=None, flux=None, **kw):
    Bn = gns.shape[0]
    if kw.get("device_out"):
        raise ValueError("devices=... returns host arrays (device_out is per device)")
    if len(set(devices)) < len(list(devices)):
        kw["team"] = 1
    per_image_psf = (psf.dim() if _B.torch.is_tensor(psf) else np.ndim(psf)) == 3

    def work(dev, lo, hi):
        return _solve_batch(variant, gns[lo:hi], psf[lo:hi] if per_image_psf else psf,
                            _shard(bkgs, lo, hi, Bn),
                            betaParams=_shard(betaParams, lo, hi, Bn),
                            flux=_shard(flux, lo, hi, Bn), **kw)

    parts = on_devices(devices, Bn, work)
    return {k: (np.concatenate([p[k] for p in parts]) if parts[0][k] is not None else None)
            for k in parts[0]}


def _no_sharded_state(kw):
    if kw.get("return_state"):
        raise ValueError("return_state=True is not available with devices=[...]: a solver "
                         "state sharded over GPUs is not supported")


def sgp_batch(gns, psf, bkgs, devices=None, **kw):
    if devices is not None:
        _no_sharded_state(kw)
        return _solve_sharded(_B.BSGP_VARIANT_KL, gns, psf, bkgs, devices, **kw)
    return _solve_batch(_B.BSGP_VARIANT_KL, gns, psf, bkgs, **kw)


def sgp_betaDiv_batch(gns, psf, bkgs, betaParams=None, devices=None, **kw):
    if devices is not None:
        _no_sharded_state(kw)
        return _solve_sharded(_B.BSGP_VARIANT_BETA, gns, psf, bkgs, devices,
                              betaParams=betaParams, **kw)
    return _solve_batch(_B.BSGP_VARIANT_BETA, gns, psf, bkgs, betaParams=betaParams, **kw)


# ... 70 lines not shown
```

### include/bsgp.h

```cpp
#ifndef BSGP_H_
#define BSGP_H_

#include <stddef.h>
#include <stdint.h>

#ifdef __cplusplus
extern "C" {
#endif

#define BSGP_OK 0
#define BSGP_ERR_ARG (-1)
#define BSGP_ERR_HIP (-2)
#define BSGP_ERR_UNSUPPORTED (-3)
#define BSGP_ERR_PSF (-4)

#define BSGP_CONV_CIRCULAR 0
#define BSGP_CONV_LINEAR_FILL 1

#define BSGP_VARIANT_KL 0
#define BSGP_VARIANT_BETA 1

typedef struct bsgp_plan_s* bsgp_plan;

typedef struct {
// ... 101 lines not shown
#define BSGP_DTYPE_F32 0
#define BSGP_DTYPE_F64 1
int bsgp_background2d(const void* data, int32_t dtype, int32_t B, int32_t H, int32_t W, int32_t bh,
                      int32_t bw, int32_t fh, int32_t fw, double sigma, int32_t maxiters,
                      double exclude_percentile, int32_t clip, const uint8_t* mask, double* bkg_out,
                      double* rms_out, double* mesh_out, double* rms_mesh_out, double* medians_out,
                      int32_t* status_out, void* stream);

typedef struct {
  int32_t hw;
  int32_t ngauss;
  int32_t ldeg;
  int32_t sdeg;
  double cos, sin;
  double ax, ay;
  double sigma_inc;
  double x_orig, y_orig;
  const double* coeffs;
  int32_t ncoef;
} bsgp_psf_model;

int bsgp_psf_stamps(const bsgp_psf_model* model, const double* xy, int32_t n, int32_t spatial,
                    int32_t normalize, double* out, void* stream);

int bsgp_plan_set_psfs(bsgp_plan plan, const double* psfs_dev, int32_t n, void* stream);


#define BSGP_STATE_MAGIC 0x53475342u
#define BSGP_STATE_VERSION 1
#define BSGP_STATE_HEADER_BYTES 1024

typedef struct {
  uint32_t magic;
  uint32_t version;
  int32_t H, W;
  int32_t storage;
  int32_t conv_mode;
  int32_t hist_cap;
  int32_t T;
  int32_t iters_done;
  int32_t stopped;
  int32_t Xones;
  int32_t epoch;
  int32_t g32;
  int32_t beta0_given;
  int64_t record_bytes;
  int64_t counters[7];
  double scaling, flux, bkg_scalar;
  double x_low, x_upp;
  double Dcoeff, tol;
  double elapsed;
  double fv, alpha, tau, lr, init_lr, beta;
  double lam_p, lam_ratio, kappa;
  double konst;
  double gfill;
  double Valpha[32];
  double Fold[32];
  bsgp_params prm;
} bsgp_state_header;

int bsgp_state_layout(int32_t H, int32_t W, int32_t storage, int32_t bkg_is_map,
                      int32_t hist_cap, int64_t* offs );
int bsgp_state_bytes(bsgp_plan plan, int32_t bkg_is_map, int32_t MAXIT_done_max,
                     int64_t* bytes_per_image);
int bsgp_state_save(bsgp_plan plan, int32_t B, void* state_dev, int64_t bytes_per_image,
                    void* stream);
int bsgp_solve_resume(bsgp_plan plan, int32_t B, const bsgp_params* params,
                      const void* state_dev, int32_t n_state, int64_t bytes_per_image,
                      const int32_t* index, const bsgp_outputs* out, void* stream);

int bsgp_convolve2d(const void* data, int32_t dtype, int32_t B, int32_t H, int32_t W,
                    const double* kernel, int32_t kh, int32_t kw, double* out, void* stream);
int bsgp_detect_sources(const void* data, int32_t dtype, int32_t B, int32_t H, int32_t W,
                        const double* threshold_map, double threshold, int32_t npixels,
                        int32_t connectivity, const uint8_t* mask, int32_t* labels_out,
                        int32_t* nlabels_out, void* stream);
int bsgp_segment_catalog(const double* data, const double* conv, const int32_t* labels, int32_t B,
                         int32_t H, int32_t W, int32_t cap, const int32_t* nlabels,
                         int32_t* int_cols_out, double* f64_cols_out, int32_t* status_out,
                         void* stream);

int bsgp_device_synchronize(void);
const char* bsgp_last_error(void);
int32_t bsgp_abi_version(void);

#ifdef __cplusplus
}
#endif
#endif
```

Baseline: 302,700 image-iterations/s.

## Specialize persistent solver phases on compile-time 256x256 geometry

Adds a compile-time geometry type (SGeo256) and templates the row/column FFT convolution, line-search and BB phases on it. For 256x256 f64 persistent solves with the matching plan, the persistent kernel dispatches to these specialized instances, so sizes, strides, LDS offsets and twiddle offsets become constants and the odd-row tail checks disappear. The goal is to cut runtime address arithmetic, register pressure and branching in the hot loop. The cost is extra code size and compile time, plus a second code path that must stay consistent with the generic one; a runtime toggle and an environment knob are added.

```diff
diff --git a/beta-sgp_amd/_bsgp.py b/beta-sgp_amd/_bsgp.py
--- a/beta-sgp_amd/_bsgp.py
+++ b/beta-sgp_amd/_bsgp.py
@@ -141,6 +141,8 @@
             L.bsgp_fits_to_f64.argtypes = [vp, i64, i32, dbl, dbl, vp, vp]
             L.bsgp_psf_stamps.argtypes = [ctypes.POINTER(PsfModel), vp, i32, i32, i32, vp, vp]
             L.bsgp_plan_set_psfs.argtypes = [vp, vp, i32, vp]
+            L.bsgp_plan_set_static_geo.argtypes = [vp, i32]
+            L.bsgp_plan_static_geo.argtypes = [vp, vp]
             L.bsgp_state_layout.argtypes = [i32, i32, i32, i32, i32, vp]
             L.bsgp_state_bytes.argtypes = [vp, i32, i32, ctypes.POINTER(i64)]
             L.bsgp_state_save.argtypes = [vp, i32, vp, i64, vp]
@@ -160,7 +162,8 @@
                          "bsgp_psf_stamps", "bsgp_plan_set_psfs", "bsgp_state_layout",
                          "bsgp_state_bytes", "bsgp_state_save", "bsgp_solve_resume",
                          "bsgp_background2d", "bsgp_convolve2d", "bsgp_detect_sources",
-                         "bsgp_segment_catalog"]:
+                         "bsgp_segment_catalog", "bsgp_plan_set_static_geo",
+                         "bsgp_plan_static_geo"]:
                 getattr(L, name).restype = ctypes.c_int
             if L.bsgp_abi_version() != ABI_VERSION:
                 raise BsgpError(-3, f"{LIB_PATH} has ABI {L.bsgp_abi_version()}, this binding "
@@ -175,7 +178,8 @@
             "bsgp_last_error", "bsgp_abi_version", "bsgp_extract_tiles", "bsgp_coadd_tiles",
             "bsgp_fits_to_f64", "bsgp_psf_stamps", "bsgp_plan_set_psfs", "bsgp_state_layout",
             "bsgp_state_bytes", "bsgp_state_save", "bsgp_solve_resume", "bsgp_background2d",
-            "bsgp_convolve2d", "bsgp_detect_sources", "bsgp_segment_catalog"]
+            "bsgp_convolve2d", "bsgp_detect_sources", "bsgp_segment_catalog",
+            "bsgp_plan_set_static_geo", "bsgp_plan_static_geo"]
 
 
 def check(rc):
@@ -241,6 +245,15 @@
         check(lib().bsgp_plan_set_psfs(self.h, _ptr(psfs), psfs.shape[0], current_stream()))
         self.n_psf = psfs.shape[0]
         return self
+
+    def set_static_geo(self, mode):
+        check(lib().bsgp_plan_set_static_geo(self.h, -1 if mode is None else int(bool(mode))))
+        return self
+
+    def static_geo_used(self):
+        used = ctypes.c_int32()
+        check(lib().bsgp_plan_static_geo(self.h, ctypes.byref(used)))
+        return bool(used.value)
 
     def apply(self, x, transpose=False):
         x = x.contiguous()
diff --git a/beta-sgp_amd/csrc/bsgp_api.hip b/beta-sgp_amd/csrc/bsgp_api.hip
--- a/beta-sgp_amd/csrc/bsgp_api.hip
+++ b/beta-sgp_amd/csrc/bsgp_api.hip
@@ -177,6 +177,14 @@
   bsgp_params last_prm{};
   bsgp_outputs last_out{};
   int last_B = 0, last_T = 0, last_beta0 = 0;
+  int static_geo_next = -1;
+  int last_static_geo = 0;
+};
+
+struct StaticGeoCall {
+  bsgp_plan p;
+  explicit StaticGeoCall(bsgp_plan q) : p(q) { p->last_static_geo = 0; }
+  ~StaticGeoCall() { p->static_geo_next = -1; }
 };
 
 static int proj_list_cap(const Geo& g, int T) {
@@ -634,6 +642,19 @@
   return BSGP_OK;
 }
 
+int bsgp_plan_set_static_geo(bsgp_plan p, int32_t mode) {
+  if (!p) return fail(BSGP_ERR_ARG, "plan is NULL");
+  if (mode < -1 || mode > 1) return fail(BSGP_ERR_ARG, "static_geo must be -1, 0 or 1");
+  p->static_geo_next = mode;
+  return BSGP_OK;
+}
+
+int bsgp_plan_static_geo(bsgp_plan p, int32_t* used) {
+  if (!p || !used) return fail(BSGP_ERR_ARG, "plan or used is NULL");
+  *used = p->last_static_geo;
+  return BSGP_OK;
+}
+
 int bsgp_plan_info(bsgp_plan p, int32_t* P, int32_t* Q, int64_t* slot_bytes,
                    int32_t* fft_waves) {
   if (!p) return fail(BSGP_ERR_ARG, "plan is NULL");
@@ -690,6 +711,7 @@
   if (!kernel_ms || !launches) return fail(BSGP_ERR_ARG, "kernel_ms / launches missing");
   if (!prm) return fail(BSGP_ERR_ARG, "params is NULL");
   if (!p) return fail(BSGP_ERR_ARG, "plan is NULL");
+  StaticGeoCall sgc(p);
   DEVICE_SCOPE(p->device);
   SolveProf prof;
   prof.kernel_ms = kernel_ms;
@@ -713,6 +735,9 @@
                       const bsgp_outputs* out, void* stream, SolveProf* prof,
                       const ResumeCtx* rs) {
   if (!p) return fail(BSGP_ERR_ARG, "plan is NULL");
+  const int static_geo_choice = p->static_geo_next;
+  p->static_geo_next = -1;
+  p->last_static_geo = 0;
   int rc = check_params(prm);
   if (rc) return rc;
   if (B < 1) return fail(BSGP_ERR_ARG, "B must be >= 1");
@@ -761,6 +786,7 @@
     a.Tc = std::max(T, std::min(nc, want));
   }
   a.fuse_col = T == 1 ? 2 : 0;
+  a.static_geo = 0;
   a.tpart = T > 1 ? p->tpart : nullptr;
   a.tctr = p->tctr;
   a.tfail = reinterpret_cast<int*>(p->tctr + (size_t)B * kTeamWords);
@@ -800,6 +826,12 @@
   const bool persist =
       prm->persistent && T == 1 && !track && (!rs || ring_rule || rs->uniform);
   if (persist) S = 1;
+  {
+    const int want = static_geo_choice >= 0 ? static_geo_choice
+                                            : (int)env_knob("BSGP_STATIC_GEO", 1, 0, 1);
+    a.static_geo = (want && persist && persist_static_geo(a, K)) ? 1 : 0;
+    p->last_static_geo = a.static_geo;
+  }
   const bool ring = prm->stop_criterion >= 2 && prm->stop_criterion <= 4;
   a.fold_setup = (persist && !ring && !rs && env_knob("BSGP_FOLD_SETUP", 1, 0, 1)) ? 1 : 0;
   if (S > 1 && p->nsub < S) {
@@ -1084,6 +1116,7 @@
                       int32_t n_state, int64_t bytes_per_image, const int32_t* index,
                       const bsgp_outputs* out, void* stream) {
   if (!p) return fail(BSGP_ERR_ARG, "plan is NULL");
+  StaticGeoCall sgc(p);
   int rc = check_params(prm);
   if (rc) return rc;
   if (!state_dev || n_state < 1) return fail(BSGP_ERR_ARG, "state_dev missing");
diff --git a/beta-sgp_amd/csrc/bsgp_device.hpp b/beta-sgp_amd/csrc/bsgp_device.hpp
--- a/beta-sgp_amd/csrc/bsgp_device.hpp
+++ b/beta-sgp_amd/csrc/bsgp_device.hpp
@@ -66,8 +66,49 @@
   size_t tf_stride;
 };
 
-__device__ __forceinline__ const cd* tf_of(const Geo& G, int img, int transpose) {
+template <class GT = Geo>
+__device__ __forceinline__ const cd* tf_of(const GT& G, int img, int transpose) {
   return (transpose ? G.tfAT : G.tfA) + (size_t)img * G.tf_stride;
+}
+
+template <int N, int OFF>
+struct SPlan {
+  static constexpr int n = N;
+  static constexpr int lds_tw = OFF;
+};
+template <int H_, int W_, int P_, int Q_>
+struct SGeo {
+  static constexpr int H = H_, W = W_, P = P_, Q = Q_;
+  static constexpr int Qh = Q_ / 2 + 1;
+  static constexpr int nfw = kWaves, nfc = kWaves, coop = 0;
+  static constexpr int maxlen = P_ > Q_ ? P_ : Q_;
+  static constexpr int lpad = (maxlen + 1 > 2 * Qh ? maxlen + 1 : 2 * Qh) | 1;
+  static constexpr int sld = H_ + (H_ & 1);
+  static constexpr int tw2 = 0, twmix = -1;
+  static constexpr int lds_fft_bytes = nfw * 2 * lpad * (int)sizeof(cd);
+  static constexpr int lds_tw_p =
+      lds_fft_bytes + kWaves * kMaxRed * (int)sizeof(double) + kSharedBytes;
+  static constexpr int lds_tw_q = P_ == Q_ ? lds_tw_p : lds_tw_p + P_ * (int)sizeof(cd);
+  static constexpr int lds_bytes = lds_tw_q + Q_ * (int)sizeof(cd);
+  static constexpr SPlan<P_, lds_tw_p> fp{};
+  static constexpr SPlan<Q_, lds_tw_q> fq{};
+  const cd* tfA;
+  const cd* tfAT;
+  size_t tf_stride;
+};
+template <class GT>
+struct IsStaticGeo : std::false_type {};
+template <int H_, int W_, int P_, int Q_>
+struct IsStaticGeo<SGeo<H_, W_, P_, Q_>> : std::true_type {};
+using SGeo256 = SGeo<256, 256, 270, 270>;
+static_assert(SGeo256::Qh == 136 && SGeo256::sld == 256 && SGeo256::lpad == 273, "geometry");
+
+template <bool COMP = true, int N, int OFF, class Sync>
+__device__ __forceinline__ cd* fft_any(cd* a, cd* b, const SPlan<N, OFF>&, bool inv, int lane,
+                                       int nlanes, Sync sync) {
+  extern __shared__ __attribute__((aligned(16))) char bsgp_dyn_lds[];
+  const cd* t = reinterpret_cast<const cd*>(bsgp_dyn_lds + OFF);
+  return fft_run_static<N, COMP>(a, b, t, inv, lane, nlanes, sync);
 }
 
 __device__ __forceinline__ void copy_tw(const FftPlan& f) {
@@ -834,8 +875,8 @@
   __builtin_memcpy(&b, y, sizeof(T));
 }
 
-template <bool COOP>
-__device__ __forceinline__ bool row_wide(const Geo& G) {
+template <bool COOP, class GT = Geo>
+__device__ __forceinline__ bool row_wide(const GT& G) {
   return !COOP && (G.W & 1) == 0;
 }
 
@@ -1348,10 +1389,17 @@
     coop_col_conv_g(G, D, spec, tf, lds);
 }
 
+template <class GT>
+__device__ __forceinline__ bool row_two(const GT&, int r, int nrows) {
+  if constexpr (IsStaticGeo<GT>::value) {
+    if constexpr ((GT::H & 1) == 0) return true;
+  }
+  return (r + 1) < nrows;
+}
 template <int JCH = kJCH, bool PF = false, bool COMP = true, bool COOP = false,
           bool PIPE = false, int PHS = -1, unsigned POL = 0, class LD, class MK,
-          class LD2 = NoWide>
-__device__ __forceinline__ void row_fwd2(const Geo& G, const Part& D, int nrows, int ncols,
+          class LD2 = NoWide, class GT = Geo>
+__device__ __forceinline__ void row_fwd2(const GT& G, const Part& D, int nrows, int ncols,
                                          int ldim, cd* spec, cd* lds, LD&& ld, MK&& mk,
                                          LD2&& ld2 = LD2{}) {
   if constexpr (COOP) {
@@ -1376,10 +1424,10 @@
     cd* b = a + G.lpad;
     int r = 2 * (D.gw0 + w);
     V v0[JCH], v1[JCH];
-    if (PF && r < nrows) load(r, (r + 1) < nrows, 0, v0, v1);
+    if (PF && r < nrows) load(r, row_two(G, r, nrows), 0, v0, v1);
     PH_SUB_T(tph);
     for (; r < nrows; r += 2 * D.gws) {
-      const bool two = (r + 1) < nrows;
+      const bool two = row_two(G, r, nrows);
       auto put = [&](int j0, const V (&w0)[JCH], const V (&w1)[JCH]) __attribute__((always_inline)) {
 #pragma unroll
         for (int u = 0; u < JCH; ++u) {
@@ -1415,7 +1463,7 @@
         }
       }
       const int rn = r + 2 * D.gws;
-      if (PF && rn < nrows) load(rn, (rn + 1) < nrows, 0, v0, v1);
+      if (PF && rn < nrows) load(rn, row_two(G, rn, nrows), 0, v0, v1);
       wave_sync();
       PH_SUB(PHS, tph);
       cd* Z = fft_any<COMP>(a, b, G.fq, false, lane, 64, WaveSync());
@@ -1447,8 +1495,8 @@
                                                   [](int, int, double v) { return v; });
 }
 
-template <unsigned POL = 0>
-__device__ __forceinline__ void gather_pair(const Geo& G, const cd* spec, int ld, int r, bool two,
+template <unsigned POL = 0, class GT = Geo>
+__device__ __forceinline__ void gather_pair(const GT& G, const cd* spec, int ld, int r, bool two,
                                             cd* a, int lane) {
   constexpr bool NT = (POL & kNtSR) != 0;
   for (int k0 = lane; k0 < G.Qh; k0 += 64 * kGCH) {
@@ -1474,8 +1522,8 @@
 
 typedef __attribute__((address_space(3))) void lds_void_t;
 typedef __attribute__((address_space(1))) void gbl_void_t;
-template <unsigned POL = 0>
-__device__ __forceinline__ void stage_pair(const Geo& G, const cd* spec, int ld, int r, bool two,
+template <unsigned POL = 0, class GT = Geo>
+__device__ __forceinline__ void stage_pair(const GT& G, const cd* spec, int ld, int r, bool two,
                                            cd* F, int lane) {
   constexpr int kAux = (POL & kNtSR) ? 2 : 0;
   for (int k0 = 0; k0 < G.Qh; k0 += 32) {
@@ -1486,7 +1534,8 @@
     }
   }
 }
-__device__ __forceinline__ void unpack_pair(const Geo& G, const cd* F, bool two, cd* a, int lane) {
+template <class GT = Geo>
+__device__ __forceinline__ void unpack_pair(const GT& G, const cd* F, bool two, cd* a, int lane) {
   for (int k = lane; k < G.Qh; k += 64) {
     const cd A = F[2 * k];
     const cd B = two ? F[2 * k + 1] : cmk(0.0, 0.0);
@@ -1497,8 +1546,8 @@
 
 template <bool PRE, int JCH = kJCH, bool COMP = true, bool COOP = false,
           bool PIPE = false, int PHS = -1, unsigned POL = 0, class LD, class USE,
-          class LD2 = NoWide>
-__device__ __forceinline__ void row_inv2(const Geo& G, const Part& D, const cd* spec, cd* lds,
+          class LD2 = NoWide, class GT = Geo>
+__device__ __forceinline__ void row_inv2(const GT& G, const Part& D, const cd* spec, cd* lds,
                                          LD&& ld, USE&& use, LD2&& ld2 = LD2{}) {
   if constexpr (COOP) {
     coop_row_inv(G, D, spec, lds, ld, use);
@@ -1521,9 +1570,9 @@
     cd* other = in + G.lpad;
     int r = 2 * (D.gw0 + w);
     PH_SUB_T(tph);
-    if (r < G.H) gather_pair<POL>(G, spec, G.sld, r, (r + 1) < G.H, in, lane);
+    if (r < G.H) gather_pair<POL>(G, spec, G.sld, r, row_two(G, r, G.H), in, lane);
     for (; r < G.H; r += 2 * D.gws) {
-      const bool two = (r + 1) < G.H;
+      const bool two = row_two(G, r, G.H);
       V v0[JCH], v1[JCH];
       if (PRE) load(r, two, 0, v0, v1);
       wave_sync();
@@ -1532,7 +1581,7 @@
       PH_SUB(PHS + 1, tph);
       cd* F = (Z == in) ? other : in;
       const int rn = r + 2 * D.gws;
-      const bool next = rn < G.H, two_n = (rn + 1) < G.H;
+      const bool next = rn < G.H, two_n = row_two(G, rn, G.H);
       if (next) stage_pair<POL>(G, spec, G.sld, rn, two_n, F, lane);
       auto eat = [&](int j0, const V (&w0)[JCH], const V (&w1)[JCH]) __attribute__((always_inline)) {
 #pragma unroll
@@ -1634,8 +1683,8 @@
   }
 }
 
-template <int JCH = kJCH, bool COMP = true, unsigned POL = 0, class LD, class CP>
-__device__ __forceinline__ void row_inv_fwd2(const Geo& G, const Part& D, cd* spec, cd* lds,
+template <int JCH = kJCH, bool COMP = true, unsigned POL = 0, class LD, class CP, class GT = Geo>
+__device__ __forceinline__ void row_inv_fwd2(const GT& G, const Part& D, cd* spec, cd* lds,
                                              LD&& ld, CP&& cp) {
   using V = decltype(ld(0, 0));
   const int w = threadIdx.x >> 6, lane = threadIdx.x & 63;
@@ -1644,7 +1693,7 @@
     cd* a = lds + w * 2 * G.lpad;
     cd* b = a + G.lpad;
     for (int r = 2 * (D.gw0 + w); r < G.H; r += 2 * D.gws) {
-      const bool two = (r + 1) < G.H;
+      const bool two = row_two(G, r, G.H);
       gather_pair<POL>(G, spec, G.sld, r, two, a, lane);
       V v0[JCH], v1[JCH];
       load_rows<JCH>(ld, r, two, 0, lane, G.W, v0, v1);
@@ -1679,8 +1728,8 @@
   }
 }
 
-template <bool COOP = false, unsigned POL = 0>
-__device__ __forceinline__ void col_conv(const Geo& G, const Part& D, cd* spec, const cd* tf,
+template <bool COOP = false, unsigned POL = 0, class GT = Geo>
+__device__ __forceinline__ void col_conv(const GT& G, const Part& D, cd* spec, const cd* tf,
                                          cd* lds) {
   constexpr bool NT = (POL & kNtSC) != 0;
   if constexpr (COOP) {
diff --git a/beta-sgp_amd/csrc/bsgp_internal.hpp b/beta-sgp_amd/csrc/bsgp_internal.hpp
--- a/beta-sgp_amd/csrc/bsgp_internal.hpp
+++ b/beta-sgp_amd/csrc/bsgp_internal.hpp
@@ -49,6 +49,7 @@
   int T;
   int Tc;
   int fuse_col;
+  int static_geo;
   double* tpart;
   unsigned int* tctr;
   int* tfail;
@@ -157,6 +158,7 @@
 hipError_t launch_persist(const SolveArgs& a, int K, size_t lds, hipStream_t s, unsigned* queue,
                           unsigned* done, int grid);
 hipError_t persist_resident_per_cu(const SolveArgs& a, int K, size_t lds, int* per_cu);
+bool persist_static_geo(const SolveArgs& a, int K);
 hipError_t persist_phase_prof(unsigned long long* out, int n, int reset);
 void persist_kernels_all(std::vector<const void*>& f);
 
diff --git a/beta-sgp_amd/csrc/bsgp_kernels.hpp b/beta-sgp_amd/csrc/bsgp_kernels.hpp
--- a/beta-sgp_amd/csrc/bsgp_kernels.hpp
+++ b/beta-sgp_amd/csrc/bsgp_kernels.hpp
@@ -26,6 +26,9 @@
 #endif
 #ifndef BSGP_STREAM_NT
 #define BSGP_STREAM_NT 0
+#endif
+#ifndef BSGP_STATIC_GEO
+#define BSGP_STATIC_GEO 0
 #endif
 constexpr int kLsLanes = 32;
 #ifndef BSGP_ACC_SERIES
@@ -243,6 +246,38 @@
     st.bar_base = (int)(t.base + (unsigned int)t.nb);
 }
 __device__ __forceinline__ bool leader(const Team& t) { return t.m == 0 && threadIdx.x == 0; }
+
+template <class GT>
+__device__ __forceinline__ decltype(auto) geo_of(const SolveArgs& A) {
+  if constexpr (IsStaticGeo<GT>::value) {
+    return GT{A.g.tfA, A.g.tfAT, A.g.tf_stride};
+  } else {
+    return (A.g);
+  }
+}
+template <class GT>
+__device__ __forceinline__ Team team_of(const SolveArgs& A, int img, const ImgState& st) {
+  if constexpr (IsStaticGeo<GT>::value) {
+    Team t{};
+    t.T = 1;
+    t.G = 1;
+    return t;
+  } else {
+    return make_team(A, img, st);
+  }
+}
+template <class GT>
+__device__ __forceinline__ size_t lds_fft_bytes_of(const SolveArgs& A) {
+  if constexpr (IsStaticGeo<GT>::value) {
+    return (size_t)GT::lds_fft_bytes;
+  } else {
+    return A.lds_fft_bytes;
+  }
+}
+#define BSGP_LDS_VIEWS_G(A, GT)                                                     \
+  extern __shared__ __attribute__((aligned(16))) char smem[];                      \
+  cd* lds = reinterpret_cast<cd*>(smem + geo_of<GT>(A).tw2);                       \
+  double* red = reinterpret_cast<double*>(smem + geo_of<GT>(A).tw2 + lds_fft_bytes_of<GT>(A))
 
 #define BSGP_LDS_VIEWS(A)                                                           \
   extern __shared__ __attribute__((aligned(16))) char smem[];                      \
@@ -753,14 +788,14 @@
   return project_df_fn(sumf, flux, 0.0, 1.0, 1e-11, 0, 0, A.prm.max_projs);
 }
 
-template <bool COOP, class V, bool LL = true, unsigned POL = 0>
+template <bool COOP, class V, bool LL = true, unsigned POL = 0, class GT = Geo>
 __device__ __forceinline__ void dir_phase(const SolveArgs& A, int img) {
   constexpr bool kO16 = (POL & kNtO16) != 0, kO8 = (POL & kNtO8) != 0;
-  BSGP_LDS_VIEWS(A);
+  BSGP_LDS_VIEWS_G(A, GT);
   ImgState& st = A.st[img];
   PH_T(tk0);
-  Team tm = make_team(A, img, st);
-  const Geo& G = A.g;
+  Team tm = team_of<GT>(A, img, st);
+  decltype(auto) G = geo_of<GT>(A);
   const Part Pt = make_part(tm, G.nfw, G.W);
   const bsgp_params& P = A.prm;
   const int N = G.H * G.W;
@@ -877,14 +912,14 @@
 }
 
 template <int K, int MODE, bool ADAPT, bool COOP, class V, bool SB = false, bool PRED = false,
-          unsigned POL = 0>
+          unsigned POL = 0, class GT = Geo>
 __device__ __forceinline__ void ls_phase(const SolveArgs& A, int img) {
   constexpr bool kO8 = (POL & kNtO8) != 0, kW = (POL & kNtW) != 0;
-  BSGP_LDS_VIEWS(A);
+  BSGP_LDS_VIEWS_G(A, GT);
   ImgState& st = A.st[img];
   PH_T(tk0);
-  Team tm = make_team(A, img, st);
-  const Geo& G = A.g;
+  Team tm = team_of<GT>(A, img, st);
+  decltype(auto) G = geo_of<GT>(A);
   const Part Pt = make_part(tm, G.nfw, G.W);
   const bsgp_params& P = A.prm;
   const int N = G.H * G.W;
@@ -1114,7 +1149,7 @@
       }
     });
     if (series) {
-      team_sum_max<N1>(t1, umax, red, tm, 25);
+      team_sum_max<N1>(t1, umax, red, tm, 38);
       rho = umax;
     } else {
       team_sum<N1>(t1, red, tm);
@@ -1402,14 +1437,14 @@
 }
 
 
-template <bool COOP, class V, unsigned POL = 0>
+template <bool COOP, class V, unsigned POL = 0, class GT = Geo>
 __device__ __forceinline__ void bb_phase(const SolveArgs& A, int img) {
   constexpr bool kO16 = (POL & kNtO16) != 0, kO8 = (POL & kNtO8) != 0, kW = (POL & kNtW) != 0;
-  BSGP_LDS_VIEWS(A);
+  BSGP_LDS_VIEWS_G(A, GT);
   ImgState& st = A.st[img];
   PH_T(tk0);
-  Team tm = make_team(A, img, st);
-  const Geo& G = A.g;
+  Team tm = team_of<GT>(A, img, st);
+  decltype(auto) G = geo_of<GT>(A);
   const Part Pt = make_part(tm, G.nfw, G.W);
   const bsgp_params& P = A.prm;
   const int N = G.H * G.W;
@@ -1588,37 +1623,53 @@
 __device__ __attribute__((noinline)) void persist_setup(ArgRef r, int img) {
   setup_phase<COOP, V>(args_of(r), __builtin_amdgcn_readfirstlane(img));
 }
-template <bool COOP, class V, unsigned POL>
+template <bool COOP, class V, unsigned POL, class GT = Geo>
 __device__ __attribute__((noinline)) void persist_dir(ArgRef r, int img) {
-  dir_phase<COOP, V, false, POL>(args_of(r), __builtin_amdgcn_readfirstlane(img));
-}
-template <bool COOP, unsigned POL>
+  dir_phase<COOP, V, false, POL, GT>(args_of(r), __builtin_amdgcn_readfirstlane(img));
+}
+template <bool COOP, unsigned POL, class GT = Geo>
 __device__ __attribute__((noinline)) void persist_col_a(ArgRef r, int img) {
   const SolveArgs& A = args_of(r);
   img = __builtin_amdgcn_readfirstlane(img);
-  BSGP_LDS_VIEWS(A);
+  BSGP_LDS_VIEWS_G(A, GT);
   (void)red;
   Team tm{};
   tm.T = 1;
   const Bufs<double> Bd = slot_bufs<double>(A, img, 0);
   PH_T(tc0);
-  col_conv<COOP, POL>(A.g, make_part(tm, COOP ? A.g.nfc : A.g.nfw, A.g.W), Bd.spec,
-                      tf_of(A.g, img, 0), lds);
+  decltype(auto) G = geo_of<GT>(A);
+  col_conv<COOP, POL>(G, make_part(tm, COOP ? G.nfc : G.nfw, G.W), Bd.spec, tf_of(G, img, 0), lds);
   PH_ADD(3, tc0);
 }
-template <int K, int MODE, bool ADAPT, bool COOP, class V, bool SB, unsigned POL>
+template <int K, int MODE, bool ADAPT, bool COOP, class V, bool SB, unsigned POL, class GT = Geo>
 __device__ __attribute__((noinline)) void persist_ls(ArgRef r, int img) {
-  ls_phase<K, MODE, ADAPT, COOP, V, SB, true, POL>(args_of(r),
-                                                   __builtin_amdgcn_readfirstlane(img));
-}
-template <bool COOP, class V, unsigned POL>
+  ls_phase<K, MODE, ADAPT, COOP, V, SB, true, POL, GT>(args_of(r),
+                                                       __builtin_amdgcn_readfirstlane(img));
+}
+template <bool COOP, class V, unsigned POL, class GT = Geo>
 __device__ __attribute__((noinline)) void persist_bb(ArgRef r, int img) {
-  bb_phase<COOP, V, POL>(args_of(r), __builtin_amdgcn_readfirstlane(img));
+  bb_phase<COOP, V, POL, GT>(args_of(r), __builtin_amdgcn_readfirstlane(img));
 }
 
 constexpr unsigned kDoneStop = 0x40000000u;
 __device__ __forceinline__ unsigned ld_sc1_u32(const unsigned* p) {
   return __hip_atomic_load((gu32*)p, __ATOMIC_RELAXED, __HIP_MEMORY_SCOPE_AGENT);
+}
+
+template <class V, bool ON>
+__host__ __device__ constexpr bool static_geo_kernel(bool coop, int K, int mode, bool adapt) {
+  return ON && !coop && K == 2 && (mode == 3 || mode == 4) && !adapt &&
+         std::is_same<V, double>::value;
+}
+inline bool static_geo_plan(const SolveArgs& a) {
+  using S = SGeo256;
+  const Geo& g = a.g;
+  return g.H == S::H && g.W == S::W && g.P == S::P && g.Q == S::Q && g.Qh == S::Qh &&
+         g.nfw == S::nfw && g.coop == 0 && g.lpad == S::lpad && g.sld == S::sld &&
+         g.tw2 == S::tw2 && g.twmix == S::twmix && g.fp.n == S::P && g.fq.n == S::Q &&
+         g.fp.lds_tw == S::lds_tw_p && g.fq.lds_tw == S::lds_tw_q &&
+         a.lds_fft_bytes == (size_t)S::lds_fft_bytes && a.T == 1 &&
+         a.storage == BSGP_STORAGE_F64;
 }
 
 template <bool COOP, int K, int MODE, bool ADAPT, class V, bool SB = false>
@@ -1630,6 +1681,7 @@
   __shared__ int s_img;
   __shared__ unsigned s_k;
   constexpr unsigned kPol = ADAPT ? 0u : (unsigned)(BSGP_STREAM_NT);
+  constexpr bool kStatic = static_geo_kernel<V, (BSGP_STATIC_GEO != 0)>(COOP, K, MODE, ADAPT);
   const int tid = threadIdx.x;
   const Geo& G = A.g;
   load_tw_lds(G);
@@ -1716,6 +1768,15 @@
     const ArgRef ar = kernarg_ref();
     if (fs && k == 1) {
       persist_setup<COOP, V>(ar, img);
+    } else if (kStatic && A.static_geo) {
+      if constexpr (kStatic) {
+        persist_dir<COOP, V, kPol, SGeo256>(ar, img);
+        __syncthreads();
+        persist_col_a<COOP, kPol, SGeo256>(ar, img);
+        persist_ls<K, MODE, ADAPT, COOP, V, SB, kPol, SGeo256>(ar, img);
+        __syncthreads();
+        persist_bb<COOP, V, kPol, SGeo256>(ar, img);
+      }
     } else {
       persist_dir<COOP, V, kPol>(ar, img);
       __syncthreads();
diff --git a/beta-sgp_amd/csrc/bsgp_persist.hip b/beta-sgp_amd/csrc/bsgp_persist.hip
--- a/beta-sgp_amd/csrc/bsgp_persist.hip
+++ b/beta-sgp_amd/csrc/bsgp_persist.hip
@@ -7,6 +7,9 @@
 #endif
 #ifndef BSGP_STREAM_NT
 #define BSGP_STREAM_NT 21
+#endif
+#ifndef BSGP_STATIC_GEO
+#define BSGP_STATIC_GEO 1
 #endif
 #include "bsgp_kernels.hpp"
 
@@ -24,6 +27,14 @@
     return bsgp_app_launch_persist(&a, K, lds, s, queue, done, grid);
   if (a.storage == BSGP_STORAGE_F32) return launch_persist_f32(a, K, lds, s, queue, done, grid);
   return launch_persist_t<double>(a, K, lds, s, queue, done, grid);
+}
+
+bool persist_static_geo(const SolveArgs& a, int K) {
+  if (a.g.coop || app_static_plan(a.g, a.storage) || a.storage != BSGP_STORAGE_F64) return false;
+  bool adapt = false;
+  const int mode = ls_mode(a, &adapt);
+  return static_geo_kernel<double, (BSGP_STATIC_GEO != 0)>(false, K >= 2 ? 2 : K, mode, adapt) &&
+         static_geo_plan(a);
 }
 
 hipError_t persist_resident_per_cu(const SolveArgs& a, int K, size_t lds, int* per_cu) {
diff --git a/beta-sgp_amd/sgp.py b/beta-sgp_amd/sgp.py
--- a/beta-sgp_amd/sgp.py
+++ b/beta-sgp_amd/sgp.py
@@ -2,6 +2,7 @@
 import logging
 import math
 import os
+import threading
 
 import numpy as np
 
@@ -444,7 +445,7 @@
                  lr_exp_param=0.1, schedule_lr=False, ls_spec=None, ls_series=None,
                  streams=None, team=None, proj_cache=None, gn_compact=None,
                  device_out=False, profile=False, storage="f64", gn_f32=None, save=False,
-                 errflag=False, obj=None, persistent=None, return_state=False):
+                 errflag=False, obj=None, persistent=None, return_state=False, static_geo=None):
     torch = _B.torch
     if save or errflag:
         raise ValueError("save / errflag are single-image options: use sgp / sgp_betaDiv")
@@ -507,12 +508,23 @@
         if len(psf) != Bn:
             raise ValueError("one PSF per image: psf must be [B, kh, kw]")
         plan = _B.per_image_plan(H, W, psf, mode, storage=storage)
-        out = plan.solve(gns, bkgs, prm, flux=fl, x0=x0, beta0=b0, profile=profile)
+        out = plan.set_static_geo(static_geo).solve(gns, bkgs, prm, flux=fl, x0=x0, beta0=b0,
+                                                    profile=profile)
+        _last.static_geo = plan.static_geo_used()
     else:
         with _B.lease_plan(H, W, psf, mode, storage=storage) as plan:
-            out = plan.solve(gns, bkgs, prm, flux=fl, x0=x0, beta0=b0, profile=profile)
+            out = plan.set_static_geo(static_geo).solve(gns, bkgs, prm, flux=fl, x0=x0, beta0=b0,
+                                                        profile=profile)
+            _last.static_geo = plan.static_geo_used()
             state = _B.SolverState(plan.save_state(Bn), psf) if return_state else None
     return _finish_batch(out, state, device_out)
+
+
+_last = threading.local()
+
+
+def last_static_geo():
+    return bool(getattr(_last, "static_geo", False))
 
 
 def _finish_batch(out, state, device_out):
@@ -543,7 +555,7 @@
     return _params(code, **d, **kw)
 
 
-_RESUME_TUNING =("streams", "persistent", "proj_cache", "ls_spec", "team")
+_RESUME_TUNING =("streams", "persistent", "proj_cache", "ls_spec", "team", "static_geo")
 
 
 def sgp_resume(state, MAXIT, images=None, device_out=False, return_state=False, **tuning):
@@ -557,6 +569,7 @@
     prm = state.params()
     prm.MAXIT = int(MAXIT)
     prm.team = int(h["T"][0])
+    static_geo = tuning.pop("static_geo", None)
     for k, v in tuning.items():
         if v is not None:
             setattr(prm, k, int(v))
@@ -573,7 +586,8 @@
         index = torch.from_numpy((idx % len(state)).astype(np.int32)).to("cuda")
     storage = int(h["storage"][0])
     with _B.lease_plan(H, W, state.psf, int(h["conv_mode"][0]), storage=storage) as plan:
-        out = plan.resume(dev.records, prm, index=index)
+        out = plan.set_static_geo(static_geo).resume(dev.records, prm, index=index)
+        _last.static_geo = plan.static_geo_used()
         new = (_B.SolverState(plan.save_state(out["iters"].numel()), state.psf)
                if return_state else None)
     return _finish_batch(out, new, device_out)
diff --git a/include/bsgp.h b/include/bsgp.h
--- a/include/bsgp.h
+++ b/include/bsgp.h
@@ -207,6 +207,9 @@
 
 int bsgp_device_synchronize(void);
 const char* bsgp_last_error(void);
+int bsgp_plan_set_static_geo(bsgp_plan plan, int32_t mode);
+int bsgp_plan_static_geo(bsgp_plan plan, int32_t* used);
+
 int32_t bsgp_abi_version(void);
 
 #ifdef __cplusplus
```

New measurement: 309,800 image-iterations/s (median of 6 runs). +2.3%, better.
